# GemsLab/H2GCN

Hardware: AMD Instinct MI355X
Metric: aggregated edges/sec (1+2-hop SpMM) (higher is better)
Workload: dtype f32

## Files before the change

h2gcn_amd/_capi.py:

```python
from __future__ import annotations

import ctypes as C
import os
from pathlib import Path

ABI_VERSION = 5
MAX_HOPS = 8

OK = 0
ERR_INVALID_ARGUMENT = -1
ERR_HIP = -2
ERR_OUT_OF_MEMORY = -3
ERR_BAD_INDEX = -4
ERR_NO_TRANSPOSE = -5
ERR_INTERNAL = -6
ERR_EXCHANGE_TIMEOUT = -7

METRICS_MAX_SETS = 4
XCHG_BLOB_BYTES = 192
XCHG_COPY_ENGINE = 0
XCHG_COPY_KERNEL = 1

DTYPE_F32 = 0
DTYPE_BF16 = 1

PLAN_BUILD_TRANSPOSE = 0x1
PLAN_SKIP_VALIDATION = 0x2
PLAN_HOST_TRANSPOSE = 0x4
PLAN_KEEP_PERMUTATION = 0x8
PLAN_SYMMETRIC_PATTERN = 0x10

EXPORTED_SYMBOLS = (
    "h2gcn_abi_version",
    "h2gcn_last_error",
    "h2gcn_device_count",
    "h2gcn_plan_create",
    "h2gcn_plan_destroy",
    "h2gcn_plan_info",
    "h2gcn_plan_set_values",
    "h2gcn_plan_transpose_sharing",
    "h2gcn_plan_device_bytes",
    "h2gcn_spmm_hops_f32",
    "h2gcn_spmm_hops_T_f32",
    "h2gcn_plan_schedule",
    "h2gcn_plan_segment_classes",
    "h2gcn_spmm_workspace_bytes",
    "h2gcn_spmm_hops_opts_f32",
    "h2gcn_spmm_hops_T_opts_f32",
    "h2gcn_spmm_hops_bf16",
    "h2gcn_spmm_hops_T_bf16",
    "h2gcn_sddmm_hops_f32",
    "h2gcn_sddmm_hops_bf16",
    "h2gcn_row_softmax_hops_f32",
    "h2gcn_row_softmax_backward_hops_f32",
    "h2gcn_edge_scores_hops_f32",
    "h2gcn_edge_scores_backward_hops_f32",
    "h2gcn_spmm_hops_values_f32",
    "h2gcn_spmm_hops_T_values_f32",
    "h2gcn_ring_scratch_bytes",
    "h2gcn_ring_count",
    "h2gcn_ring_fill",
    "h2gcn_ring_count_rows",
    "h2gcn_ring_fill_rows",
    "h2gcn_hop_normalize",
    "h2gcn_hop_normalize_rows",
    "h2gcn_dropout_dense_small_rows",
    "h2gcn_dropout_dense_workspace_bytes",
    "h2gcn_dropout_dense_f32",
    "h2gcn_dropout_dense_backward_f32",
    "h2gcn_dropout_dense_bf16",
    "h2gcn_dropout_dense_backward_bf16",
    "h2gcn_dropout_dense_rows_f32",
    "h2gcn_dropout_dense_rows_bf16",
    "h2gcn_dropout_dense_backward_rows_f32",
    "h2gcn_dropout_dense_backward_rows_bf16",
    "h2gcn_masked_metrics_workspace_bytes",
    "h2gcn_masked_metrics_f32",
    "h2gcn_masked_ce_backward_f32",
    "h2gcn_adam_keras_f32",
    "h2gcn_adam_keras_l2_f32",
    "h2gcn_l2_penalty_workspace_bytes",
    "h2gcn_l2_penalty_f32",
    "h2gcn_xchg_create",
    "h2gcn_xchg_export",
    "h2gcn_xchg_connect",
    "h2gcn_xchg_allgather_begin",
    "h2gcn_xchg_allgather_post",
    "h2gcn_xchg_allgather_pull",
    "h2gcn_xchg_allgather_pull_rows",
    "h2gcn_xchg_allgather_end",
    "h2gcn_xchg_reduce_scatter_begin",
    "h2gcn_xchg_reduce_scatter_end",
    "h2gcn_xchg_reset_dependencies",
    "h2gcn_xchg_status",
    "h2gcn_xchg_destroy",
)


class PlanOpts(C.Structure):
    _fields_ = [
        ("struct_size", C.c_uint32),
        ("flags", C.c_uint32),
        ("long_row_threshold", C.c_int32),
        ("rows_per_wave", C.c_int32),
        ("variant", C.c_int32),
        ("slice_cols", C.c_int32),
        ("reserved", C.c_int32 * 2),
    ]


LAUNCH_RELU = 0x1
LAUNCH_ACCUMULATE = 0x2


class LaunchOpts(C.Structure):
    _fields_ = [
        ("struct_size", C.c_uint32),
        ("flags", C.c_uint32),
        ("workspace", C.c_void_p),
        ("workspace_bytes", C.c_size_t),
        ("bias", C.c_void_p),
    ]


class H2GCNError(RuntimeError):

    def __init__(self, status: int, message: str):
        super().__init__(f"libh2gcn_hip: {message} (status {status})")
        self.status = status


def library_path() -> Path:
    override = os.environ.get("H2GCN_HIP_LIBRARY")
    if override:
        return Path(override)
    return Path(__file__).resolve().parent / "csrc" / "libh2gcn_hip.so"


_LIB = None


def lib() -> C.CDLL:
    global _LIB
    if _LIB is not None:
        return _LIB
    path = library_path()
    if not path.exists():
        raise RuntimeError(
            f"{path} not found: build it with `python -c 'import __graft_entry__ as g; g.build()'` "
            "or `make -C h2gcn_amd/csrc`.  h2gcn_amd has no CPU fallback."
        )
    L = C.CDLL(str(path))
    L.h2gcn_abi_version.restype = C.c_int
    L.h2gcn_abi_version.argtypes = []
    L.h2gcn_last_error.restype = C.c_char_p
    L.h2gcn_last_error.argtypes = []
    L.h2gcn_device_count.restype = C.c_int
    L.h2gcn_device_count.argtypes = []
    L.h2gcn_plan_create.restype = C.c_int
    L.h2gcn_plan_create.argtypes = [
        C.c_int, C.c_int64, C.c_int64,
        C.POINTER(C.c_void_p), C.POINTER(C.c_void_p), C.POINTER(C.c_void_p),
        C.POINTER(PlanOpts), C.c_void_p, C.POINTER(C.c_void_p),
    ]
    L.h2gcn_plan_destroy.restype = None
    L.h2gcn_plan_destroy.argtypes = [C.c_void_p]
    L.h2gcn_plan_set_values.restype = C.c_int
    L.h2gcn_plan_set_values.argtypes = [C.c_void_p, C.c_int, C.c_void_p, C.c_void_p]
    L.h2gcn_plan_info.restype = C.c_int
    L.h2gcn_plan_info.argtypes = [
        C.c_void_p, C.c_int, C.POINTER(C.c_int64), C.POINTER(C.c_int64), C.POINTER(C.c_int64),
        C.POINTER(C.c_int64), C.POINTER(C.c_int32),
    ]
    L.h2gcn_spmm_hops_f32.restype = C.c_int
    L.h2gcn_spmm_hops_f32.argtypes = [
        C.c_void_p, C.c_uint32, C.c_void_p, C.c_int64, C.c_int32, C.c_void_p, C.c_int64, C.c_int64, C.c_void_p,
    ]
    L.h2gcn_spmm_hops_T_f32.restype = C.c_int
    L.h2gcn_spmm_hops_T_f32.argtypes = [
        C.c_void_p, C.c_uint32, C.c_void_p, C.c_int64, C.c_int64, C.c_int32, C.c_void_p, C.c_int64, C.c_void_p,
    ]
    L.h2gcn_plan_schedule.restype = C.c_int
    L.h2gcn_plan_schedule.argtypes = [C.c_void_p, C.c_uint32, C.c_int, C.c_int64, C.c_int32] + [C.POINTER(C.c_int32)] * 4
    if hasattr(L, "h2gcn_plan_segment_classes"):
        L.h2gcn_plan_segment_classes.restype = C.c_int
        L.h2gcn_plan_segment_classes.argtypes = [C.c_void_p, C.c_uint32, C.c_int, C.c_int64, C.c_int32] + [C.POINTER(C.c_int64)] * 3
    if hasattr(L, "h2gcn_plan_transpose_sharing"):
        L.h2gcn_plan_transpose_sharing.restype = C.c_int
        L.h2gcn_plan_transpose_sharing.argtypes = [C.c_void_p, C.c_int]
        L.h2gcn_plan_device_bytes.restype = C.c_size_t
        L.h2gcn_plan_device_bytes.argtypes = [C.c_void_p]
    L.h2gcn_spmm_workspace_bytes.restype = C.c_size_t
    L.h2gcn_spmm_workspace_bytes.argtypes = [C.c_void_p, C.c_uint32, C.c_int, C.c_void_p, C.c_int64, C.c_int64, C.c_int32]
    L.h2gcn_spmm_hops_opts_f32.restype = C.c_int
    L.h2gcn_spmm_hops_opts_f32.argtypes = [
        C.c_void_p, C.c_uint32, C.c_void_p, C.c_int64, C.c_int32, C.c_void_p, C.c_int64, C.c_int64,
        C.POINTER(LaunchOpts), C.c_void_p,
    ]
    L.h2gcn_spmm_hops_T_opts_f32.restype = C.c_int
    L.h2gcn_spmm_hops_T_opts_f32.argtypes = [
        C.c_void_p, C.c_uint32, C.c_void_p, C.c_int64, C.c_int64, C.c_int32, C.c_void_p, C.c_int64,
        C.POINTER(LaunchOpts), C.c_void_p,
    ]
    if hasattr(L, "h2gcn_spmm_hops_bf16"):
        L.h2gcn_spmm_hops_bf16.restype = C.c_int
        L.h2gcn_spmm_hops_bf16.argtypes = [
            C.c_void_p, C.c_uint32, C.c_void_p, C.c_int64, C.c_int32, C.c_int, C.c_void_p, C.c_int64, C.c_int64,
            C.POINTER(LaunchOpts), C.c_void_p,
        ]
        L.h2gcn_spmm_hops_T_bf16.restype = C.c_int
        L.h2gcn_spmm_hops_T_bf16.argtypes = [
            C.c_void_p, C.c_uint32, C.c_void_p, C.c_int64, C.c_int64, C.c_int32, C.c_int, C.c_void_p, C.c_int64,
            C.POINTER(LaunchOpts), C.c_void_p,
        ]
    if hasattr(L, "h2gcn_sddmm_hops_f32"):
        sddmm_args = [C.c_void_p, C.c_uint32, C.c_void_p, C.c_int64, C.c_int64, C.c_void_p, C.c_int64, C.c_int32,
                      C.POINTER(C.c_void_p), C.c_void_p]
        L.h2gcn_sddmm_hops_f32.restype = C.c_int
        L.h2gcn_sddmm_hops_f32.argtypes = sddmm_args
        L.h2gcn_sddmm_hops_bf16.restype = C.c_int
        L.h2gcn_sddmm_hops_bf16.argtypes = list(sddmm_args)
    if hasattr(L, "h2gcn_row_softmax_hops_f32"):
        L.h2gcn_row_softmax_hops_f32.restype = C.c_int
        L.h2gcn_row_softmax_hops_f32.argtypes = [C.c_void_p, C.c_uint32, C.POINTER(C.c_void_p), C.POINTER(C.c_void_p), C.c_void_p]
        L.h2gcn_row_softmax_backward_hops_f32.restype = C.c_int
        L.h2gcn_row_softmax_backward_hops_f32.argtypes = [C.c_void_p, C.c_uint32, C.POINTER(C.c_void_p), C.POINTER(C.c_void_p),
                                                          C.POINTER(C.c_void_p), C.c_void_p]
    if hasattr(L, "h2gcn_edge_scores_hops_f32"):
        node_args = [C.c_void_p, C.c_uint32, C.c_void_p, C.c_int64, C.c_void_p, C.c_int64, C.c_float, C.POINTER(C.c_void_p)]
        L.h2gcn_edge_scores_hops_f32.restype = C.c_int
        L.h2gcn_edge_scores_hops_f32.argtypes = node_args + [C.c_void_p]
        L.h2gcn_edge_scores_backward_hops_f32.restype = C.c_int
        L.h2gcn_edge_scores_backward_hops_f32.argtypes = node_args + [C.c_void_p, C.c_int64, C.c_void_p, C.c_int64, C.c_void_p]
    if hasattr(L, "h2gcn_spmm_hops_values_f32"):
        values_args = [C.c_void_p, C.c_uint32, C.POINTER(C.c_void_p), C.POINTER(C.c_int64), C.POINTER(C.c_int64), C.c_int32]
        L.h2gcn_spmm_hops_values_f32.restype = C.c_int
        L.h2gcn_spmm_hops_values_f32.argtypes = values_args + [C.c_void_p, C.c_int64, C.c_int32, C.c_void_p, C.c_int64, C.c_int64, C.c_void_p]
        L.h2gcn_spmm_hops_T_values_f32.restype = C.c_int
        L.h2gcn_spmm_hops_T_values_f32.argtypes = values_args + [C.c_void_p, C.c_int64, C.c_int64, C.c_int32, C.c_void_p, C.c_int64, C.c_void_p]
    L.h2gcn_ring_scratch_bytes.restype = C.c_size_t
    L.h2gcn_ring_scratch_bytes.argtypes = [C.c_int64]
    ring_common = [C.c_int64, C.c_void_p, C.c_void_p, C.c_void_p, C.c_void_p,
                   C.c_int, C.POINTER(C.c_void_p), C.POINTER(C.c_void_p), C.c_int,
                   C.c_int, C.POINTER(C.c_void_p), C.POINTER(C.c_void_p), C.c_int]
    L.h2gcn_ring_count.restype = C.c_int
    L.h2gcn_ring_count.argtypes = ring_common + [C.c_void_p, C.POINTER(C.c_int64), C.c_void_p, C.c_size_t, C.c_void_p]
    L.h2gcn_ring_fill.restype = C.c_int
    L.h2gcn_ring_fill.argtypes = ring_common + [C.c_void_p, C.c_void_p, C.c_void_p, C.c_size_t, C.c_void_p]
    ring_rows = [C.c_int64, C.c_int64, C.c_int64] + ring_common[1:]
    L.h2gcn_ring_count_rows.restype = C.c_int
    L.h2gcn_ring_count_rows.argtypes = ring_rows + [C.c_void_p, C.POINTER(C.c_int64), C.c_void_p, C.c_size_t, C.c_void_p]
    L.h2gcn_ring_fill_rows.restype = C.c_int
    L.h2gcn_ring_fill_rows.argtypes = ring_rows + [C.c_void_p, C.c_void_p, C.c_void_p, C.c_size_t, C.c_void_p]
    L.h2gcn_hop_normalize_rows.restype = C.c_int
    L.h2gcn_hop_normalize_rows.argtypes = [C.c_int64, C.c_void_p, C.c_void_p, C.c_int, C.c_void_p, C.c_int64, C.c_void_p, C.c_void_p, C.c_void_p]
    L.h2gcn_hop_normalize.restype = C.c_int
    L.h2gcn_hop_normalize.argtypes = [C.c_int64, C.c_void_p, C.c_void_p, C.c_int, C.c_void_p, C.c_int64, C.c_void_p, C.c_void_p]
    if hasattr(L, "h2gcn_dropout_dense_small_rows"):
        L.h2gcn_dropout_dense_small_rows.restype = C.c_int64
        L.h2gcn_dropout_dense_small_rows.argtypes = [C.c_int64]
    L.h2gcn_dropout_dense_workspace_bytes.restype = C.c_size_t
    L.h2gcn_dropout_dense_workspace_bytes.argtypes = [C.c_int64, C.c_int32, C.c_int32]
    L.h2gcn_dropout_dense_f32.restype = C.c_int
    L.h2gcn_dropout_dense_f32.argtypes = [C.c_void_p, C.c_int64, C.c_int64, C.c_int32, C.c_void_p, C.c_int32, C.c_void_p, C.c_float,
                                          C.c_uint64, C.c_void_p, C.c_void_p, C.c_int64, C.c_void_p, C.c_size_t, C.c_void_p]
    L.h2gcn_dropout_dense_backward_f32.restype = C.c_int
    L.h2gcn_dropout_dense_backward_f32.argtypes = [C.c_void_p, C.c_int64, C.c_int64, C.c_int32, C.c_void_p, C.c_int32, C.c_void_p, C.c_int64,
                                                   C.c_float, C.c_uint64, C.c_void_p, C.c_void_p, C.c_int64, C.c_void_p, C.c_void_p,
                                                   C.c_size_t, C.c_void_p]
    if hasattr(L, "h2gcn_dropout_dense_bf16"):
        L.h2gcn_dropout_dense_bf16.restype = C.c_int
        L.h2gcn_dropout_dense_bf16.argtypes = list(L.h2gcn_dropout_dense_f32.argtypes)
        L.h2gcn_dropout_dense_backward_bf16.restype = C.c_int
        L.h2gcn_dropout_dense_backward_bf16.argtypes = [C.c_void_p, C.c_int64, C.c_int64, C.c_int32, C.c_void_p, C.c_int32, C.c_void_p, C.c_int64,
                                                        C.c_float, C.c_uint64, C.c_void_p, C.c_int, C.c_void_p, C.c_int64, C.c_void_p, C.c_void_p,
                                                        C.c_size_t, C.c_void_p]
    if hasattr(L, "h2gcn_dropout_dense_rows_f32"):
        rows_args = [C.c_void_p, C.c_int64]
        L.h2gcn_dropout_dense_rows_f32.restype = C.c_int
        L.h2gcn_dropout_dense_rows_f32.argtypes = list(L.h2gcn_dropout_dense_f32.argtypes) + rows_args
        L.h2gcn_dropout_dense_rows_bf16.restype = C.c_int
        L.h2gcn_dropout_dense_rows_bf16.argtypes = list(L.h2gcn_dropout_dense_f32.argtypes) + rows_args
        L.h2gcn_dropout_dense_backward_rows_f32.restype = C.c_int
        L.h2gcn_dropout_dense_backward_rows_f32.argtypes = list(L.h2gcn_dropout_dense_backward_f32.argtypes) + rows_args
        L.h2gcn_dropout_dense_backward_rows_bf16.restype = C.c_int
        L.h2gcn_dropout_dense_backward_rows_bf16.argtypes = list(L.h2gcn_dropout_dense_backward_bf16.argtypes) + rows_args
    L.h2gcn_masked_metrics_workspace_bytes.restype = C.c_size_t
    L.h2gcn_masked_metrics_workspace_bytes.argtypes = [C.c_int64]
    L.h2gcn_masked_metrics_f32.restype = C.c_int
    L.h2gcn_masked_metrics_f32.argtypes = [C.c_void_p, C.c_int64, C.c_int64, C.c_int32, C.c_int32, C.POINTER(C.c_void_p), C.POINTER(C.c_int64),
                                           C.POINTER(C.c_void_p), C.c_void_p, C.c_void_p, C.c_void_p, C.c_size_t, C.c_void_p]
    L.h2gcn_masked_ce_backward_f32.restype = C.c_int
    L.h2gcn_masked_ce_backward_f32.argtypes = [C.c_void_p, C.c_int64, C.c_int64, C.c_int32, C.c_void_p, C.c_int64, C.c_void_p, C.c_void_p,
                                               C.c_void_p, C.c_int64, C.c_void_p]
    L.h2gcn_adam_keras_f32.restype = C.c_int
    L.h2gcn_adam_keras_f32.argtypes = [C.c_int32, C.POINTER(C.c_void_p), C.POINTER(C.c_void_p), C.POINTER(C.c_void_p), C.POINTER(C.c_void_p),
                                       C.POINTER(C.c_int64), C.c_float, C.c_float, C.c_float, C.c_float, C.c_void_p, C.c_int64, C.c_void_p]
    if hasattr(L, "h2gcn_adam_keras_l2_f32"):
        L.h2gcn_adam_keras_l2_f32.restype = C.c_int
        L.h2gcn_adam_keras_l2_f32.argtypes = [C.c_int32, C.POINTER(C.c_void_p), C.POINTER(C.c_void_p), C.POINTER(C.c_void_p), C.POINTER(C.c_void_p),
                                              C.POINTER(C.c_int64), C.POINTER(C.c_float), C.c_float, C.c_float, C.c_float, C.c_float, C.c_void_p,
                                              C.c_int64, C.c_void_p]
        L.h2gcn_l2_penalty_workspace_bytes.restype = C.c_size_t
        L.h2gcn_l2_penalty_workspace_bytes.argtypes = []
        L.h2gcn_l2_penalty_f32.restype = C.c_int
        L.h2gcn_l2_penalty_f32.argtypes = [C.c_int32, C.POINTER(C.c_void_p), C.POINTER(C.c_int64), C.POINTER(C.c_float), C.c_void_p, C.c_void_p,
                                           C.c_size_t, C.c_void_p]
    L.h2gcn_xchg_create.restype = C.c_int
    L.h2gcn_xchg_create.argtypes = [C.c_int, C.c_int, C.c_int, C.c_size_t, C.c_int, C.c_int, C.POINTER(C.c_void_p)]
    L.h2gcn_xchg_export.restype = C.c_int
    L.h2gcn_xchg_export.argtypes = [C.c_void_p, C.c_void_p]
    L.h2gcn_xchg_connect.restype = C.c_int
    L.h2gcn_xchg_connect.argtypes = [C.c_void_p, C.c_void_p]
    L.h2gcn_xchg_allgather_begin.restype = C.c_int
    L.h2gcn_xchg_allgather_begin.argtypes = [
        C.c_void_p, C.c_int, C.c_void_p, C.c_int64, C.c_int64, C.c_int64, C.c_int32, C.c_void_p, C.c_void_p,
    ]
    L.h2gcn_xchg_allgather_post.restype = C.c_int
    L.h2gcn_xchg_allgather_post.argtypes = L.h2gcn_xchg_allgather_begin.argtypes
    L.h2gcn_xchg_allgather_pull.restype = C.c_int
    L.h2gcn_xchg_allgather_pull.argtypes = [C.c_void_p, C.c_int, C.c_int64, C.c_int32, C.c_void_p]
    if hasattr(L, "h2gcn_xchg_allgather_pull_rows"):
        L.h2gcn_xchg_allgather_pull_rows.restype = C.c_int
        L.h2gcn_xchg_allgather_pull_rows.argtypes = [C.c_void_p, C.c_int, C.c_int64, C.c_int32, C.c_void_p, C.POINTER(C.c_void_p), C.POINTER(C.c_int64)]
    L.h2gcn_xchg_allgather_end.restype = C.c_int
    L.h2gcn_xchg_allgather_end.argtypes = [C.c_void_p, C.c_int, C.c_void_p]
    L.h2gcn_xchg_reduce_scatter_begin.restype = C.c_int
    L.h2gcn_xchg_reduce_scatter_begin.argtypes = [C.c_void_p, C.c_int, C.c_void_p, C.c_int64, C.c_int32, C.c_void_p, C.c_void_p]
    L.h2gcn_xchg_reduce_scatter_end.restype = C.c_int
    L.h2gcn_xchg_reduce_scatter_end.argtypes = [C.c_void_p, C.c_int, C.c_void_p]
    L.h2gcn_xchg_reset_dependencies.restype = C.c_int
    L.h2gcn_xchg_reset_dependencies.argtypes = [C.c_void_p]
    L.h2gcn_xchg_status.restype = C.c_int
    L.h2gcn_xchg_status.argtypes = [C.c_void_p]
    L.h2gcn_xchg_destroy.restype = None
    L.h2gcn_xchg_destroy.argtypes = [C.c_void_p]
    got = L.h2gcn_abi_version()
    if got != ABI_VERSION and not (os.environ.get("H2GCN_HIP_LIBRARY") and got in (3, 4)):
        raise RuntimeError(f"{path}: ABI version {got}, this front end expects {ABI_VERSION}")
    _LIB = L
    return L


def has(symbol: str) -> bool:
# ... 8 lines not shown
```

h2gcn_amd/csrc/h2gcn_capi.hip:

```cpp
#include <hip/hip_runtime.h>

#include <algorithm>
#include <cstdarg>
#include <cstdlib>
#include <cstdio>
#include <cstring>
#include <deque>
#include <map>
#include <mutex>
#include <memory>
#include <new>
#include <string>
#include <vector>

#include "h2gcn_hip.h"
#include "spmm_kernels.hip.h"

#include "capi_internal.h"

namespace h2gcn {

thread_local std::string g_last_error;

int fail(h2gcn_status st, const char* fmt, ...) {
    char buf[512];
    va_list ap;
    va_start(ap, fmt);
    vsnprintf(buf, sizeof(buf), fmt, ap);
    va_end(ap);
    g_last_error = buf;
    return (int)st;
}

}

namespace {

using h2gcn::fail;
using h2gcn::g_last_error;

struct DeviceBuf {
    void* p = nullptr;
    ~DeviceBuf() {
        if (p) (void)hipFree(p);
    }
    DeviceBuf() = default;
    DeviceBuf(DeviceBuf&& o) noexcept : p(o.p) { o.p = nullptr; }
    DeviceBuf(const DeviceBuf&) = delete;
    DeviceBuf& operator=(const DeviceBuf&) = delete;
};

struct HopOperand {
    const int64_t* rowptr = nullptr;
    const int32_t* colidx = nullptr;
    const float* vals = nullptr;
    int64_t nnz = 0;
    std::vector<int64_t> long_rows;
    std::vector<uint8_t> len8;
    int64_t n_short = 0, nnz_short = 0;
    int64_t nnz_long = 0;
    const uint32_t* perm = nullptr;
};

struct LongList {
    DeviceBuf dev;
    int n = 0;
    LongList() = default;
    LongList(LongList&&) noexcept = default;
};

struct ClassLists {
    DeviceBuf short_dev, med_dev;
    int64_t n_short = 0, nnz_short = 0, n_med = 0;
    bool built = false;
    ClassLists() = default;
    ClassLists(ClassLists&&) noexcept = default;
};

}

struct h2gcn_plan {
    int n_hops = 0;
    int64_t n_rows = 0, n_cols = 0;
    int long_threshold = 256;
    int rows_per_wave = 4;
    int variant = 0;
    int slice_cols = 0;
    bool has_transpose = false;
    int device = 0;
    std::vector<HopOperand> fwd;
    std::vector<HopOperand> adj;
    std::deque<DeviceBuf> owned;
    std::vector<int> sharing;
    size_t transpose_bytes = 0;
    mutable std::mutex mu;
    mutable std::map<uint64_t, LongList> long_cache;
    mutable std::map<uint64_t, ClassLists> class_cache;
    int short_max = -1;
    double short_min_frac = 0.05;
};

namespace h2gcn {
__global__ void check_colidx_kernel(const int32_t* __restrict__ colidx, int64_t nnz, int64_t n_cols, int* flag) {
    int bad = 0;
    for (int64_t i = (int64_t)blockIdx.x * blockDim.x + threadIdx.x; i < nnz; i += (int64_t)gridDim.x * blockDim.x) {
        const int32_t c = colidx[i];
        bad |= (c < 0) | ((int64_t)c >= n_cols);
    }
    if (bad) atomicOr(flag, 1);
}

extern template void launch_in_tile_short_rows<32, false, float, float>(const LaunchParams&, const Schedule&, dim3, hipStream_t);
extern template void launch_in_tile_short_rows<16, false, float, float>(const LaunchParams&, const Schedule&, dim3, hipStream_t);
extern template void launch_in_tile_short_rows<32, true, float, float>(const LaunchParams&, const Schedule&, dim3, hipStream_t);
extern template void launch_in_tile_short_rows<16, true, float, float>(const LaunchParams&, const Schedule&, dim3, hipStream_t);
extern template void launch_spmm<false, bf16, float>(const LaunchParams&, const Schedule&, dim3, hipStream_t);
extern template void launch_spmm<false, bf16, bf16>(const LaunchParams&, const Schedule&, dim3, hipStream_t);
extern template void launch_spmm<true, bf16, float>(const LaunchParams&, const Schedule&, dim3, hipStream_t);
extern template void launch_spmm<true, bf16, bf16>(const LaunchParams&, const Schedule&, dim3, hipStream_t);

int transpose_csr_device(int64_t n_rows, int64_t n_cols, int64_t nnz, const int64_t* rowptr, const int32_t* colidx,
                         const float* vals, int64_t** t_rowptr_out, int32_t** t_colidx_out, float** t_vals_out,
                         uint32_t** perm_out_keep, hipStream_t stream, std::string* err);
void permute_values(const uint32_t* perm, const float* vals, int64_t nnz, float* t_vals, hipStream_t stream);
}

namespace {

using h2gcn::HopCsr;
using h2gcn::LaunchParams;
using h2gcn::Schedule;

int transpose_csr_host(int64_t n_rows, int64_t n_cols, const std::vector<int64_t>& rowptr,
                       const std::vector<int32_t>& colidx, const std::vector<float>& vals,
                       std::vector<int64_t>& t_rowptr, std::vector<int32_t>& t_colidx, std::vector<float>& t_vals) {
    const int64_t nnz = rowptr[n_rows];
    t_rowptr.assign(n_cols + 1, 0);
    t_colidx.resize(nnz);
    t_vals.resize(nnz);
    for (int64_t i = 0; i < nnz; ++i) t_rowptr[colidx[i] + 1]++;
    for (int64_t c = 0; c < n_cols; ++c) t_rowptr[c + 1] += t_rowptr[c];
    std::vector<int64_t> cursor(t_rowptr.begin(), t_rowptr.end() - 1);
    for (int64_t r = 0; r < n_rows; ++r) {
        for (int64_t i = rowptr[r]; i < rowptr[r + 1]; ++i) {
            const int64_t dst = cursor[colidx[i]]++;
            t_colidx[dst] = (int32_t)r;
            t_vals[dst] = vals[i];
        }
    }
    return 0;
}

void collect_long_rows(const std::vector<int64_t>& rowptr, int64_t n_rows, int threshold, std::vector<int64_t>& out) {
    out.clear();
    for (int64_t r = 0; r < n_rows; ++r)
        if (rowptr[r + 1] - rowptr[r] >= threshold) out.push_back(r);
}

void collect_segment_lengths(const std::vector<int64_t>& rowptr, int64_t n_rows, int short_max, int long_threshold, HopOperand& op) {
    op.len8.resize((size_t)n_rows);
    op.n_short = op.nnz_short = op.nnz_long = 0;
    for (int64_t r = 0; r < n_rows; ++r) {
        const int64_t len = rowptr[r + 1] - rowptr[r];
        op.len8[(size_t)r] = (uint8_t)(len > 255 ? 255 : len);
        if (len <= short_max) {
            ++op.n_short;
            op.nnz_short += len;
        } else if (len >= long_threshold) {
            op.nnz_long += len;
        }
    }
}

thread_local bool t_stream_capturing = false;

struct CaptureScope {
    explicit CaptureScope(hipStream_t stream) {
        hipStreamCaptureStatus cs = hipStreamCaptureStatusNone;
        t_stream_capturing = hipStreamIsCapturing(stream, &cs) == hipSuccess && cs != hipStreamCaptureStatusNone;
        if (!t_stream_capturing) (void)hipGetLastError();
    }
    ~CaptureScope() { t_stream_capturing = false; }
};

int refuse_build_while_capturing(const char* what) {
    return fail(H2GCN_ERR_INVALID_ARGUMENT, "the stream is being captured and this is the first launch of this hop selection: its %s "
                "has to be built first (device allocation + upload).  Run the same launch once outside the capture (a warm-up step)", what);
}

int get_class_lists(const h2gcn_plan* plan, bool adjoint, int k, uint32_t mask, bool build, const ClassLists** out) {
    *out = nullptr;
    const std::vector<HopOperand>& ops = adjoint ? plan->adj : plan->fwd;
    const int64_t n_rows = adjoint ? plan->n_cols : plan->n_rows;
    if (plan->short_max < 0 || n_rows > 0x7fffffffLL) return H2GCN_OK;
    const uint64_t key = adjoint ? ((uint64_t)mask | (1ull << 32)) : ((uint64_t)k | (1ull << 40));
    const int sm = plan->short_max;
    std::lock_guard<std::mutex> lock(plan->mu);
    auto it = plan->class_cache.find(key);
    std::vector<const uint8_t*> sel;
    std::vector<uint8_t> any_long;
    auto prepare_adjoint = [&]() {
        any_long.assign((size_t)n_rows, 0);
        for (int h = 0; h < plan->n_hops; ++h)
            if (mask & (1u << h)) {
                sel.push_back(ops[h].len8.data());
                for (int64_t r : ops[h].long_rows) any_long[(size_t)r] = 1;
            }
    };
    if (it == plan->class_cache.end()) {
        ClassLists fresh;
        if (!adjoint) {
            fresh.n_short = ops[k].n_short;
            fresh.nnz_short = ops[k].nnz_short;
            fresh.n_med = n_rows - ops[k].n_short - (int64_t)ops[k].long_rows.size();
        } else {
            prepare_adjoint();
            for (int64_t r = 0; r < n_rows; ++r) {
                bool all = true;
                int64_t z = 0;
                for (const uint8_t* l : sel) { all = all && l[r] <= sm; z += l[r]; }
                if (all) { ++fresh.n_short; fresh.nnz_short += z; }
                else if (!any_long[(size_t)r]) ++fresh.n_med;
            }
        }
        it = plan->class_cache.emplace(key, std::move(fresh)).first;
    }
    ClassLists& cl = it->second;
    if (build && !cl.built) {
        if (t_stream_capturing) return refuse_build_while_capturing("per-class row lists");
        std::vector<int32_t> h_short, h_med;
        h_short.reserve((size_t)cl.n_short);
        h_med.reserve((size_t)cl.n_med);
        if (!adjoint) {
            const std::vector<uint8_t>& len = ops[k].len8;
            const std::vector<int64_t>& longs = ops[k].long_rows;
            size_t li = 0;
            for (int64_t r = 0; r < n_rows; ++r) {
                while (li < longs.size() && longs[li] < r) ++li;
                const bool is_long = li < longs.size() && longs[li] == r;
                if (len[(size_t)r] <= sm) h_short.push_back((int32_t)r);
                else if (!is_long) h_med.push_back((int32_t)r);
            }
        } else {
            if (sel.empty()) prepare_adjoint();
            for (int64_t r = 0; r < n_rows; ++r) {
                bool all = true;
                for (const uint8_t* l : sel) all = all && l[r] <= sm;
                if (all) h_short.push_back((int32_t)r);
                else if (!any_long[(size_t)r]) h_med.push_back((int32_t)r);
            }
        }
        DeviceBuf d_short, d_med;
        if (!h_short.empty()) {
            H2GCN_HIP_TRY(hipMalloc(&d_short.p, h_short.size() * sizeof(int32_t)));
            H2GCN_HIP_TRY(hipMemcpy(d_short.p, h_short.data(), h_short.size() * sizeof(int32_t), hipMemcpyHostToDevice));
        }
        if (!h_med.empty()) {
            H2GCN_HIP_TRY(hipMalloc(&d_med.p, h_med.size() * sizeof(int32_t)));
            H2GCN_HIP_TRY(hipMemcpy(d_med.p, h_med.data(), h_med.size() * sizeof(int32_t), hipMemcpyHostToDevice));
        }
// ... 63 lines not shown
        if (d % w != 0) continue;
        const double slice_bytes = (double)n_src_rows * w * 4.0;
        if (w > 64 && avg_segment_nnz >= 16.0 && slice_bytes > 768.0 * 1024 * 1024 && d % (w / 2) == 0) continue;
        return w;
    }
    if (rows_line_aligned && d % 4 == 0 && avg_segment_nnz >= 16.0 && (double)n_src_rows * d * 4.0 >= 512.0 * 1024 * 1024) {
        return 64;
    }
    if (d > 256) {
        const bool beyond = avg_segment_nnz >= 16.0 && (double)n_src_rows * 256 * 4.0 > 768.0 * 1024 * 1024;
        return beyond ? 128 : 256;
    }
    int w = 64;
    while (w < d) w *= 2;
    return w;
}

struct LaunchShape {
    bool adjoint;
    int n_sel;
    int64_t nnz_sel;
    int64_t n_out, n_src;
    double avg;
    int64_t ld_src;
    int d;
    bool src_line_aligned;
    const int32_t* short_list[H2GCN_MAX_HOPS];
    int64_t short_count[H2GCN_MAX_HOPS];
    const int32_t* med_list[H2GCN_MAX_HOPS];
    int64_t med_count[H2GCN_MAX_HOPS];
    int n_short_lists;
    double short_frac;
    double short_nnz_frac;
};

LaunchShape shape_of(const h2gcn_plan* plan, uint32_t mask, bool adjoint, const void* src = nullptr, int64_t ld_src = 0,
                     int64_t ld_src_hop = 0, int d = 0) {
    LaunchShape sh;
    memset(&sh, 0, sizeof(sh));
    sh.adjoint = adjoint;
    const std::vector<HopOperand>& ops = adjoint ? plan->adj : plan->fwd;
    for (int k = 0; k < plan->n_hops; ++k)
        if (mask & (1u << k)) { sh.nnz_sel += ops[k].nnz; ++sh.n_sel; }
    sh.n_out = adjoint ? plan->n_cols : plan->n_rows;
    sh.n_src = adjoint ? plan->n_rows : plan->n_cols;
    sh.avg = (sh.n_out > 0 && sh.n_sel > 0) ? (double)sh.nnz_sel / ((double)sh.n_out * sh.n_sel) : 0.0;
    sh.ld_src = ld_src;
    sh.d = d;
    sh.src_line_aligned = (reinterpret_cast<uintptr_t>(src) & 127u) == 0 && (ld_src * 4) % 128 == 0 &&
                          (!adjoint || sh.n_sel <= 1 || (ld_src_hop * 4) % 128 == 0);
    return sh;
}

int fill_short(const h2gcn_plan* plan, uint32_t mask, bool adjoint, LaunchShape& sh, bool build_lists = false);

int scratch_slice_cols(const h2gcn_plan* plan, const LaunchShape& sh) {
    if (plan->variant == 4) return 0;
    const int d = sh.d;
    if (sh.n_out == 0 || sh.n_src == 0 || sh.n_sel == 0) return 0;
    if (d <= 64) return 0;
    const double src_bytes = (double)sh.n_src * d * 4.0 * (sh.adjoint ? sh.n_sel : 1);
    if (src_bytes < 512.0 * 1024 * 1024) return 0;
    if ((double)sh.nnz_sel < 32.0 * (double)sh.n_src) return 0;
    if (!sh.adjoint && (sh.ld_src * 4) % 1024 == 0 && d % 64 == 0 && d >= 128) {
        const int w = pick_slice_cols(d, sh.n_src, plan->slice_cols, sh.avg);
        return (w == 64 || w == 128) && d % w == 0 && w < d ? w : 0;
    }
    if ((!sh.src_line_aligned || d % 4 != 0) && d > (sh.adjoint ? 256 : 128) && sh.avg >= 16.0 && (plan->slice_cols == 0 || plan->slice_cols == 64)) {
        return 64;
    }
    return 0;
}

size_t scratch_bytes(const LaunchShape& sh, int rs) {
    if (rs <= 0) return 0;
    const size_t n_slices = (size_t)((sh.d + rs - 1) / rs);
    return (size_t)sh.n_src * n_slices * (size_t)rs * 4 * (size_t)(sh.adjoint ? sh.n_sel : 1);
}

int decide(const h2gcn_plan* plan, uint32_t mask, LaunchShape& sh, int scratch, bool gen, Schedule& sc) {
    const int st = fill_short(plan, mask, sh.adjoint, sh);
    if (st != H2GCN_OK) return st;
    const int d = sh.d;
    const bool exact_ok = d >= 4;
    const int forced_slice = scratch > 0 ? scratch : plan->slice_cols;
    const int variant = plan->variant == 4 ? 0 : plan->variant;
    sc.pipe = (variant == 2 || (variant == 0 && sh.avg < 16.0)) && plan->rows_per_wave * sh.n_sel <= 32;
    sc.scalar128 = exact_ok && variant == 1 && d == 128 && forced_slice == 0;
    sc.slice = (exact_ok && !sc.scalar128) ? pick_slice_cols(d, sh.n_src, forced_slice, sh.avg, scratch > 0 || sh.src_line_aligned) : 0;
    sc.exact = sc.slice > 0 || sc.scalar128;
    sc.gen = gen;
    const bool grouped_ok = sc.exact && !sc.scalar128 && !gen && (sc.slice == 64 || sc.slice == 128);
    sc.shortrow = grouped_ok && (variant == 5 || (variant == 0 && sh.avg < 16.0 && sh.n_out >= 4 * kWavesToFill));
    sc.lists = grouped_ok && !sc.shortrow && sh.short_frac > 0.0 && (variant == 6 || (variant == 0 && sh.short_frac >= plan->short_min_frac));
    sc.pipe = sc.pipe && sc.exact && !sc.shortrow && !sc.lists && !gen;
    const bool beyond = (double)sh.n_src * d * 4.0 >= 512.0 * 1024 * 1024;
    sc.fb4 = beyond && (sc.shortrow || (sc.lists && sh.short_nnz_frac > 0.5));
    sc.off32 = false;
    return H2GCN_OK;
}

int launch(LaunchParams& p, const h2gcn_plan* plan, uint32_t mask, LaunchShape& sh, const Schedule& sc, bool adjoint,
           bool src_bf16, bool out_bf16, hipStream_t stream) {
    using namespace h2gcn;
    p.slice_cols = sc.exact ? (sc.slice > 0 ? sc.slice : 128) : p.d;
    p.n_slices = sc.exact ? (p.d + p.slice_cols - 1) / p.slice_cols : 1;
    if (p.src_slice_stride == 0) p.src_slice_stride = p.slice_cols;
    p.short_max = -1;
    p.short_groups = p.med_groups = 0;
    if (sc.lists) {
        int st = fill_short(plan, mask, adjoint, sh, true);
        if (st != H2GCN_OK) return st;
        int64_t n_listed = 0, n_med = 0, longest = 0;
        for (int s = 0; s < sh.n_short_lists; ++s) {
            n_listed += sh.short_count[s];
            n_med += sh.med_count[s];
            longest = std::max(longest, sh.short_count[s]);
        }
        static const int env_mpw = getenv("H2GCN_MED_PER_WAVE") ? atoi(getenv("H2GCN_MED_PER_WAVE")) : 0;
        static const int env_spw = getenv("H2GCN_SHORT_PER_WAVE") ? atoi(getenv("H2GCN_SHORT_PER_WAVE")) : 0;
        static const int env_major = getenv("H2GCN_SHORT_HOP_MAJOR") ? atoi(getenv("H2GCN_SHORT_HOP_MAJOR")) : -1;
        const int mpw_max = adjoint ? std::max(1, std::min(4, kWave / p.n_sel)) : 8;
        p.med_per_wave = (int)std::max<int64_t>(1, std::min<int64_t>(n_med / kWavesToFill, mpw_max));
        if (env_mpw >= 1 && env_mpw * p.n_sel <= kWave) p.med_per_wave = env_mpw;
        p.short_per_wave = 4;
        while (p.short_per_wave < 64 && n_listed / (2 * p.short_per_wave) >= kWavesToFill) p.short_per_wave *= 2;
        if (env_spw >= 4 && env_spw <= 64 && env_spw % 4 == 0) p.short_per_wave = env_spw;
        p.short_hop_major = env_major >= 0 ? env_major : 0;
        int64_t sblocks = 0, mblocks = 0;
        const int64_t s_per_block = (int64_t)kWavesPerBlock * p.short_per_wave;
        for (int s = 0; s < sh.n_short_lists; ++s) {
            p.short_list[s] = sh.short_list[s];
            p.short_count[s] = sh.short_count[s];
            sblocks += (sh.short_count[s] + s_per_block - 1) / s_per_block;
            p.short_end[s] = sblocks;
            p.med_list[s] = sh.med_list[s];
            p.med_count[s] = sh.med_count[s];
            const int64_t per_block = (int64_t)kWavesPerBlock * p.med_per_wave;
            mblocks += (sh.med_count[s] + per_block - 1) / per_block;
            p.med_end[s] = mblocks;
        }
        if (!adjoint && !p.short_hop_major) sblocks = (longest + s_per_block - 1) / s_per_block * sh.n_short_lists;
        p.short_groups = (sblocks + kNumXcd - 1) / kNumXcd;
        p.med_groups = (mblocks + kNumXcd - 1) / kNumXcd;
        p.short_max = plan->short_max;
        p.blocks_per_slice = (int64_t)p.n_long + (p.short_groups + p.med_groups) * kNumXcd;
    } else {
        p.blocks_per_slice = (int64_t)p.n_long + p.tiles_per_xcd * kNumXcd;
    }
    const int64_t n_blocks = p.blocks_per_slice * p.n_slices;
    if (n_blocks <= 0) return H2GCN_OK;
    if (n_blocks > 0x7fffffffLL) return fail(H2GCN_ERR_INVALID_ARGUMENT, "grid too large (%lld blocks)", (long long)n_blocks);
    const dim3 grid((unsigned)n_blocks);
    if (!src_bf16 && adjoint) launch_spmm<true, float, float>(p, sc, grid, stream);
    else if (!src_bf16) launch_spmm<false, float, float>(p, sc, grid, stream);
    else if (out_bf16 && adjoint) launch_spmm<true, bf16, bf16>(p, sc, grid, stream);
    else if (out_bf16) launch_spmm<false, bf16, bf16>(p, sc, grid, stream);
    else if (adjoint) launch_spmm<true, bf16, float>(p, sc, grid, stream);
    else launch_spmm<false, bf16, float>(p, sc, grid, stream);
    H2GCN_HIP_TRY(hipGetLastError());
    return H2GCN_OK;
}

void use_scratch(LaunchParams& p, const LaunchShape& sh, int rs, int64_t ld_src_hop, void* workspace, hipStream_t stream,
                 bool* off32) {
    const int n_hop = sh.adjoint ? sh.n_sel : 1;
    const int n_slices = (sh.d + rs - 1) / rs;
    const bool vec4 = sh.d % 4 == 0;
    const int64_t total = sh.n_src * (int64_t)n_slices * n_hop * (rs / (vec4 ? 4 : 1));
    const unsigned blocks = (unsigned)std::min<int64_t>((total + 255) / 256, 256 * 64);
    if (vec4)
        hipLaunchKernelGGL(h2gcn::repack_slice_major_kernel<true>, dim3(blocks), dim3(256), 0, stream, (const float*)p.src, sh.ld_src,
                           ld_src_hop, n_hop, sh.n_src, sh.d, n_slices, rs, (float*)workspace);
    else
        hipLaunchKernelGGL(h2gcn::repack_slice_major_kernel<false>, dim3(blocks), dim3(256), 0, stream, (const float*)p.src, sh.ld_src,
                           ld_src_hop, n_hop, sh.n_src, sh.d, n_slices, rs, (float*)workspace);
    p.src = workspace;
    p.ld_src = rs;
    p.d_src = (sh.d + 3) & ~3;
    p.src_slice_stride = sh.n_src * (int64_t)rs * n_hop;
    for (int s = 0; s < p.n_sel; ++s) p.src_hop_off[s] = sh.adjoint ? (int64_t)s * sh.n_src * rs : 0;
    *off32 = (double)sh.n_src * (double)n_slices * rs * n_hop * 4.0 < 4294967296.0;
}

int check_device(const h2gcn_plan* plan) {
    int cur = -1;
    H2GCN_HIP_TRY(hipGetDevice(&cur));
    if (cur != plan->device)
        return fail(H2GCN_ERR_INVALID_ARGUMENT, "plan lives on device %d but the current HIP device is %d", plan->device, cur);
    return H2GCN_OK;
}

int resolve_mask(const h2gcn_plan* plan, uint32_t hop_mask, uint32_t* out) {
    const uint32_t all = plan->n_hops >= 32 ? 0xffffffffu : ((1u << plan->n_hops) - 1u);
    if (hop_mask == 0) hop_mask = all;
    if (hop_mask & ~all) return fail(H2GCN_ERR_INVALID_ARGUMENT, "hop_mask 0x%x selects hops beyond the plan's %d", hop_mask, plan->n_hops);
    *out = hop_mask;
    return H2GCN_OK;
}

int share_symmetric(h2gcn_plan* plan, bool keep_perm, hipStream_t stream) {
    using h2gcn::MirrorStatus;
    const int H = plan->n_hops;
    const int64_t n = plan->n_rows;
    std::vector<MirrorStatus> h_status((size_t)H, MirrorStatus{~0ull, 0u, 0u});
    DeviceBuf d_status;
    H2GCN_HIP_TRY(hipMalloc(&d_status.p, (size_t)H * sizeof(MirrorStatus)));
    H2GCN_HIP_TRY(hipMemcpyAsync(d_status.p, h_status.data(), (size_t)H * sizeof(MirrorStatus), hipMemcpyHostToDevice, stream));
    std::vector<DeviceBuf> t_vals((size_t)H), partner((size_t)H);
    for (int k = 0; k < H; ++k) {
        const HopOperand& f = plan->fwd[k];
        if (f.nnz == 0) continue;
        H2GCN_HIP_TRY(hipMalloc(&t_vals[k].p, (size_t)f.nnz * sizeof(float)));
        if (keep_perm) H2GCN_HIP_TRY(hipMalloc(&partner[k].p, (size_t)f.nnz * sizeof(uint32_t)));
        H2GCN_HIP_TRY(h2gcn::mirror_pass(n, f.nnz, f.rowptr, f.colidx, f.vals, (uint32_t*)partner[k].p, (float*)t_vals[k].p,
                                         (MirrorStatus*)d_status.p + k, stream));
    }
    H2GCN_HIP_TRY(hipMemcpyAsync(h_status.data(), d_status.p, (size_t)H * sizeof(MirrorStatus), hipMemcpyDeviceToHost, stream));
    H2GCN_HIP_TRY(hipStreamSynchronize(stream));
    for (int k = 0; k < H; ++k) {
        const MirrorStatus& ms = h_status[k];
        if (ms.flags & h2gcn::kMirrorRange)
            return fail(H2GCN_ERR_BAD_INDEX, "hop %d: a column index lies outside [0, %lld)", k, (long long)n);
        if (ms.flags & h2gcn::kMirrorUnsorted)
            return fail(H2GCN_ERR_BAD_INDEX, "hop %d: the column ids of a row are not strictly ascending (H2GCN_PLAN_SYMMETRIC_PATTERN "
                        "searches rows by column and relies on the documented order)", k);
        if (ms.missing_key != ~0ull) {
            const long long r = (long long)(ms.missing_key >> 32), c = (long long)(ms.missing_key & 0xffffffffull);
            return fail(H2GCN_ERR_BAD_INDEX, "hop %d: entry (%lld, %lld) has no mirror entry (%lld, %lld): pattern not symmetric", k, r, c, c, r);
        }
    }
    plan->adj.resize(H);
    for (int k = 0; k < H; ++k) {
        const HopOperand& f = plan->fwd[k];
        HopOperand& a = plan->adj[k];
        a = f;
        a.perm = nullptr;
        const bool own_vals = f.nnz > 0 && (keep_perm || (h_status[k].flags & h2gcn::kMirrorValuesDiffer));
        plan->sharing[k] = own_vals ? 1 : 2;
        if (own_vals) {
            a.vals = (const float*)t_vals[k].p;
            plan->owned.emplace_back(std::move(t_vals[k]));
            plan->transpose_bytes += (size_t)f.nnz * sizeof(float);
        }
        if (keep_perm && f.nnz > 0) {
            a.perm = (const uint32_t*)partner[k].p;
            plan->owned.emplace_back(std::move(partner[k]));
            plan->transpose_bytes += (size_t)f.nnz * sizeof(uint32_t);
        }
    }
    return H2GCN_OK;
}

}

extern "C" {

int h2gcn_abi_version(void) { return H2GCN_ABI_VERSION; }

const char* h2gcn_last_error(void) { return g_last_error.c_str(); }

int h2gcn_device_count(void) {
    int n = 0;
    hipError_t e = hipGetDeviceCount(&n);
    if (e != hipSuccess) return fail(H2GCN_ERR_HIP, "hipGetDeviceCount failed: %s", hipGetErrorString(e));
    return n;
}

int h2gcn_plan_create(int n_hops, int64_t n_rows, int64_t n_cols, const int64_t* const* rowptr_dev,
                      const int32_t* const* colidx_dev, const float* const* vals_dev,
                      const h2gcn_plan_opts* opts, void* stream_v, h2gcn_plan_t** out_plan) {
    try {
        if (!out_plan) return fail(H2GCN_ERR_INVALID_ARGUMENT, "out_plan is NULL");
        *out_plan = nullptr;
        if (n_hops < 1 || n_hops > H2GCN_MAX_HOPS)
            return fail(H2GCN_ERR_INVALID_ARGUMENT, "n_hops = %d, supported 1..%d", n_hops, H2GCN_MAX_HOPS);
        if (n_rows < 0 || n_cols < 0 || n_cols > 0x7fffffffLL)
            return fail(H2GCN_ERR_INVALID_ARGUMENT, "bad shape %lld x %lld (column ids are int32)", (long long)n_rows, (long long)n_cols);
        if (n_rows >= (1LL << 58)) return fail(H2GCN_ERR_INVALID_ARGUMENT, "n_rows too large");
        if (!rowptr_dev || !colidx_dev || !vals_dev) return fail(H2GCN_ERR_INVALID_ARGUMENT, "NULL operand table");
        h2gcn_plan_opts o;
        memset(&o, 0, sizeof(o));
        if (opts) {
            if (opts->struct_size < 8 || opts->struct_size > sizeof(o))
                return fail(H2GCN_ERR_INVALID_ARGUMENT, "opts->struct_size = %u", opts->struct_size);
            memcpy(&o, opts, opts->struct_size);
        }
        if (o.slice_cols != 0 && o.slice_cols != 64 && o.slice_cols != 128 && o.slice_cols != 256)
            return fail(H2GCN_ERR_INVALID_ARGUMENT, "slice_cols = %d, supported 0 (auto), 64, 128, 256", o.slice_cols);
        if (o.long_row_threshold < 0 || o.rows_per_wave < 0 || o.rows_per_wave > h2gcn::kMaxRowsPerWave)
            return fail(H2GCN_ERR_INVALID_ARGUMENT, "bad tunable (long_row_threshold %d, rows_per_wave %d, max %d)",
                        o.long_row_threshold, o.rows_per_wave, h2gcn::kMaxRowsPerWave);
        const bool symmetric = (o.flags & H2GCN_PLAN_SYMMETRIC_PATTERN) != 0;
        if (symmetric && !(o.flags & H2GCN_PLAN_BUILD_TRANSPOSE))
            return fail(H2GCN_ERR_INVALID_ARGUMENT, "H2GCN_PLAN_SYMMETRIC_PATTERN modifies H2GCN_PLAN_BUILD_TRANSPOSE, which is not set");
        if (symmetric && (o.flags & H2GCN_PLAN_HOST_TRANSPOSE))
            return fail(H2GCN_ERR_INVALID_ARGUMENT, "H2GCN_PLAN_SYMMETRIC_PATTERN builds no transpose: it cannot be combined with H2GCN_PLAN_HOST_TRANSPOSE");
        if (symmetric && n_rows != n_cols)
            return fail(H2GCN_ERR_INVALID_ARGUMENT, "H2GCN_PLAN_SYMMETRIC_PATTERN needs square operands, got %lld x %lld", (long long)n_rows, (long long)n_cols);
        hipStream_t stream = (hipStream_t)stream_v;

        std::unique_ptr<h2gcn_plan> plan(new h2gcn_plan());
        plan->n_hops = n_hops;
        plan->n_rows = n_rows;
        plan->n_cols = n_cols;
        if (o.long_row_threshold > 0) plan->long_threshold = o.long_row_threshold;
        if (o.rows_per_wave > 0) plan->rows_per_wave = o.rows_per_wave;
        else if (const char* e = getenv("H2GCN_ROWS_PER_WAVE")) plan->rows_per_wave = std::max(1, std::min(atoi(e), h2gcn::kMaxRowsPerWave));
        else {
            plan->rows_per_wave = (int)std::max<int64_t>(1, std::min<int64_t>(n_rows / kWavesToFill, 4));
        }
        while ((plan->rows_per_wave + 1) * n_hops > h2gcn::kWave && plan->rows_per_wave > 1) plan->rows_per_wave--;
        plan->variant = o.variant;
        if (o.variant == 0) if (const char* e = getenv("H2GCN_VARIANT")) plan->variant = atoi(e);
        plan->slice_cols = o.slice_cols;
        if (o.slice_cols == 0) if (const char* e = getenv("H2GCN_SLICE_COLS")) plan->slice_cols = atoi(e);
        plan->short_max = std::min(h2gcn::kShortMax, plan->long_threshold - 1);
        if (const char* e = getenv("H2GCN_SHORT_MIN_FRAC")) plan->short_min_frac = atof(e);
        H2GCN_HIP_TRY(hipGetDevice(&plan->device));
        plan->fwd.resize(n_hops);

        DeviceBuf flag;
        H2GCN_HIP_TRY(hipMalloc(&flag.p, sizeof(int)));
        H2GCN_HIP_TRY(hipMemsetAsync(flag.p, 0, sizeof(int), stream));

        std::vector<std::vector<int64_t>> h_rowptr(n_hops);
        for (int k = 0; k < n_hops; ++k) {
            if (!rowptr_dev[k]) return fail(H2GCN_ERR_INVALID_ARGUMENT, "hop %d: rowptr is NULL", k);
            h_rowptr[k].resize(n_rows + 1);
            H2GCN_HIP_TRY(hipMemcpyAsync(h_rowptr[k].data(), rowptr_dev[k], (n_rows + 1) * sizeof(int64_t), hipMemcpyDeviceToHost, stream));
        }
        H2GCN_HIP_TRY(hipStreamSynchronize(stream));
        for (int k = 0; k < n_hops; ++k) {
            int st = check_rowptr(h_rowptr[k], n_rows, k);
            if (st != H2GCN_OK) return st;
            HopOperand& op = plan->fwd[k];
            op.rowptr = rowptr_dev[k];
            op.colidx = colidx_dev[k];
            op.vals = vals_dev[k];
            op.nnz = h_rowptr[k][n_rows];
            if (op.nnz > 0 && (!op.colidx || !op.vals)) return fail(H2GCN_ERR_INVALID_ARGUMENT, "hop %d: colidx/vals is NULL", k);
            if (symmetric && op.nnz >= (1LL << 32))
                return fail(H2GCN_ERR_INVALID_ARGUMENT, "hop %d: H2GCN_PLAN_SYMMETRIC_PATTERN supports < 2^32 nonzeros per hop", k);
            collect_long_rows(h_rowptr[k], n_rows, plan->long_threshold, op.long_rows);
            collect_segment_lengths(h_rowptr[k], n_rows, plan->short_max, plan->long_threshold, op);
            if (!(o.flags & H2GCN_PLAN_SKIP_VALIDATION) && op.nnz > 0) {
                const int64_t want = (op.nnz + 255) / 256;
                const unsigned blocks = (unsigned)std::min<int64_t>(want, 4096);
                hipLaunchKernelGGL(h2gcn::check_colidx_kernel, dim3(blocks), dim3(256), 0, stream, op.colidx, op.nnz, n_cols, (int*)flag.p);
                H2GCN_HIP_TRY(hipGetLastError());
            }
        }
        int h_flag = 0;
        H2GCN_HIP_TRY(hipMemcpyAsync(&h_flag, flag.p, sizeof(int), hipMemcpyDeviceToHost, stream));
        H2GCN_HIP_TRY(hipStreamSynchronize(stream));
        if (h_flag) return fail(H2GCN_ERR_BAD_INDEX, "a column index lies outside [0, %lld)", (long long)n_cols);

        plan->sharing.assign(n_hops, 0);
        if (symmetric) {
            int st = share_symmetric(plan.get(), (o.flags & H2GCN_PLAN_KEEP_PERMUTATION) != 0, stream);
            if (st != H2GCN_OK) return st;
            plan->has_transpose = true;
        } else if (o.flags & H2GCN_PLAN_BUILD_TRANSPOSE) {
            if (n_rows > 0x7fffffffLL) return fail(H2GCN_ERR_INVALID_ARGUMENT, "transpose needs n_rows < 2^31");
            plan->adj.resize(n_hops);
            for (int k = 0; k < n_hops; ++k) {
                const int64_t nnz = plan->fwd[k].nnz;
                int64_t* t_rp = nullptr;
                int32_t* t_ci = nullptr;
                float* t_va = nullptr;
                uint32_t* t_perm = nullptr;
                const bool keep_perm = (o.flags & H2GCN_PLAN_KEEP_PERMUTATION) != 0;
                if (keep_perm && (o.flags & H2GCN_PLAN_HOST_TRANSPOSE))
                    return fail(H2GCN_ERR_INVALID_ARGUMENT, "H2GCN_PLAN_KEEP_PERMUTATION needs the device transposition");
                std::vector<int64_t> t_rowptr(n_cols + 1);
                std::string terr;
                int st = (o.flags & H2GCN_PLAN_HOST_TRANSPOSE)
                             ? -1
                             : h2gcn::transpose_csr_device(n_rows, n_cols, nnz, rowptr_dev[k], colidx_dev[k], vals_dev[k],
                                                           &t_rp, &t_ci, &t_va, keep_perm ? &t_perm : nullptr, stream, &terr);
                if (st != 0 && keep_perm && st != -3)
                    return fail(H2GCN_ERR_INVALID_ARGUMENT, "H2GCN_PLAN_KEEP_PERMUTATION: %s", terr.c_str());
                if (st == 0) {
                    plan->owned.emplace_back(); plan->owned.back().p = t_rp;
                    plan->owned.emplace_back(); plan->owned.back().p = t_ci;
                    plan->owned.emplace_back(); plan->owned.back().p = t_va;
                    plan->owned.emplace_back(); plan->owned.back().p = t_perm;
                    plan->transpose_bytes += (size_t)(n_cols + 1) * sizeof(int64_t) + (size_t)nnz * (t_perm ? 12 : 8);
                    H2GCN_HIP_TRY(hipMemcpy(t_rowptr.data(), t_rp, (n_cols + 1) * sizeof(int64_t), hipMemcpyDeviceToHost));
                } else if (st == -3) {
                    return fail(H2GCN_ERR_OUT_OF_MEMORY, "transposition of hop %d: %s", k, terr.c_str());
                } else {
                    std::vector<int32_t> h_col(nnz);
                    std::vector<float> h_val(nnz);
                    if (nnz > 0) {
                        H2GCN_HIP_TRY(hipMemcpy(h_col.data(), colidx_dev[k], nnz * sizeof(int32_t), hipMemcpyDeviceToHost));
                        H2GCN_HIP_TRY(hipMemcpy(h_val.data(), vals_dev[k], nnz * sizeof(float), hipMemcpyDeviceToHost));
                    }
                    std::vector<int32_t> t_col;
                    std::vector<float> t_val;
                    transpose_csr_host(n_rows, n_cols, h_rowptr[k], h_col, h_val, t_rowptr, t_col, t_val);
                    plan->owned.emplace_back();
                    DeviceBuf& d_rp = plan->owned.back();
                    H2GCN_HIP_TRY(hipMalloc(&d_rp.p, (n_cols + 1) * sizeof(int64_t)));
                    H2GCN_HIP_TRY(hipMemcpy(d_rp.p, t_rowptr.data(), (n_cols + 1) * sizeof(int64_t), hipMemcpyHostToDevice));
                    plan->owned.emplace_back();
                    DeviceBuf& d_ci = plan->owned.back();
                    plan->owned.emplace_back();
                    DeviceBuf& d_va = plan->owned.back();
                    if (nnz > 0) {
                        H2GCN_HIP_TRY(hipMalloc(&d_ci.p, nnz * sizeof(int32_t)));
                        H2GCN_HIP_TRY(hipMemcpy(d_ci.p, t_col.data(), nnz * sizeof(int32_t), hipMemcpyHostToDevice));
                        H2GCN_HIP_TRY(hipMalloc(&d_va.p, nnz * sizeof(float)));
                        H2GCN_HIP_TRY(hipMemcpy(d_va.p, t_val.data(), nnz * sizeof(float), hipMemcpyHostToDevice));
                    }
                    plan->transpose_bytes += (size_t)(n_cols + 1) * sizeof(int64_t) + (size_t)nnz * 8;
                    t_rp = (int64_t*)d_rp.p;
                    t_ci = (int32_t*)d_ci.p;
                    t_va = (float*)d_va.p;
                }
                HopOperand& op = plan->adj[k];
                op.rowptr = t_rp;
                op.colidx = t_ci;
                op.vals = t_va;
                op.nnz = nnz;
                op.perm = t_perm;
                collect_long_rows(t_rowptr, n_cols, plan->long_threshold, op.long_rows);
                collect_segment_lengths(t_rowptr, n_cols, plan->short_max, plan->long_threshold, op);
            }
            plan->has_transpose = true;
        }
        {
            const uint32_t all = n_hops >= 32 ? 0xffffffffu : ((1u << n_hops) - 1u);
            const int64_t* unused_p = nullptr;
            int unused_n = 0;
            int st = get_long_list(plan.get(), false, all, &unused_p, &unused_n);
            if (st == H2GCN_OK && plan->has_transpose) st = get_long_list(plan.get(), true, all, &unused_p, &unused_n);
            if (st != H2GCN_OK) return st;
            auto mixed = [&](const LaunchShape& sh_) {
                return plan->variant == 6 || (plan->variant == 0 && sh_.short_frac >= plan->short_min_frac &&
                                              (sh_.avg >= 16.0 || sh_.n_out < 4 * kWavesToFill));
            };
            LaunchShape sh_f = shape_of(plan.get(), all, false);
            if ((st = fill_short(plan.get(), all, false, sh_f)) != H2GCN_OK) return st;
            if (mixed(sh_f) && (st = fill_short(plan.get(), all, false, sh_f, true)) != H2GCN_OK) return st;
            if (plan->has_transpose) {
                LaunchShape sh_a = shape_of(plan.get(), all, true);
                if ((st = fill_short(plan.get(), all, true, sh_a)) != H2GCN_OK) return st;
                if (mixed(sh_a) && (st = fill_short(plan.get(), all, true, sh_a, true)) != H2GCN_OK) return st;
            }
        }
        *out_plan = plan.release();
        return H2GCN_OK;
    } catch (const std::bad_alloc&) {
        return fail(H2GCN_ERR_OUT_OF_MEMORY, "host allocation failed in plan_create");
    } catch (...) {
        return fail(H2GCN_ERR_INTERNAL, "unexpected exception in plan_create");
    }
}

void h2gcn_plan_destroy(h2gcn_plan_t* plan) { delete plan; }

int h2gcn_plan_set_values(h2gcn_plan_t* plan, int hop, const float* vals_dev, void* stream_v) {
    if (!plan) return fail(H2GCN_ERR_INVALID_ARGUMENT, "plan is NULL");
    if (hop < 0 || hop >= plan->n_hops) return fail(H2GCN_ERR_INVALID_ARGUMENT, "hop %d outside 0..%d", hop, plan->n_hops - 1);
    HopOperand& f = plan->fwd[hop];
    if (f.nnz > 0 && !vals_dev) return fail(H2GCN_ERR_INVALID_ARGUMENT, "vals is NULL");
    int st = check_device(plan);
    if (st != H2GCN_OK) return st;
    if (plan->has_transpose) {
        HopOperand& a = plan->adj[hop];
        if (a.nnz > 0 && !a.perm)
            return fail(H2GCN_ERR_INVALID_ARGUMENT, "plan has transposed operands but was created without H2GCN_PLAN_KEEP_PERMUTATION");
        h2gcn::permute_values(a.perm, vals_dev, a.nnz, const_cast<float*>(a.vals), (hipStream_t)stream_v);
        H2GCN_HIP_TRY(hipGetLastError());
    }
    f.vals = vals_dev;
    return H2GCN_OK;
}

int h2gcn_plan_info(const h2gcn_plan_t* plan, int hop, int64_t* n_rows, int64_t* n_cols, int64_t* nnz,
                    int64_t* n_long_segments, int32_t* has_transpose) {
    if (!plan) return fail(H2GCN_ERR_INVALID_ARGUMENT, "plan is NULL");
    if (hop < 0 || hop >= plan->n_hops) return fail(H2GCN_ERR_INVALID_ARGUMENT, "hop %d outside 0..%d", hop, plan->n_hops - 1);
    if (n_rows) *n_rows = plan->n_rows;
    if (n_cols) *n_cols = plan->n_cols;
    if (nnz) *nnz = plan->fwd[hop].nnz;
    if (n_long_segments) *n_long_segments = (int64_t)plan->fwd[hop].long_rows.size();
    if (has_transpose) *has_transpose = plan->has_transpose ? 1 : 0;
    return H2GCN_OK;
}

int h2gcn_plan_transpose_sharing(const h2gcn_plan_t* plan, int hop) {
    if (!plan) return fail(H2GCN_ERR_INVALID_ARGUMENT, "plan is NULL");
    if (hop < 0 || hop >= plan->n_hops) return fail(H2GCN_ERR_INVALID_ARGUMENT, "hop %d outside 0..%d", hop, plan->n_hops - 1);
    return plan->sharing[(size_t)hop];
}

size_t h2gcn_plan_device_bytes(const h2gcn_plan_t* plan) {
    if (!plan) return 0;
    std::lock_guard<std::mutex> lock(plan->mu);
    size_t bytes = plan->transpose_bytes;
    for (const auto& kv : plan->long_cache) bytes += (size_t)kv.second.n * sizeof(int64_t);
    for (const auto& kv : plan->class_cache)
        if (kv.second.built) bytes += (size_t)(kv.second.n_short + kv.second.n_med) * sizeof(int32_t);
    return bytes;
}

namespace {
int fill_short(const h2gcn_plan* plan, uint32_t mask, bool adjoint, LaunchShape& sh, bool build_lists) {
    sh.n_short_lists = 0;
    sh.short_frac = sh.short_nnz_frac = 0.0;
    if (plan->short_max < 0 || sh.n_out <= 0 || sh.n_sel <= 0) return H2GCN_OK;
    int64_t n = 0, nnz = 0;
    const ClassLists* cl = nullptr;
    if (!adjoint) {
        int s = 0;
        for (int k = 0; k < plan->n_hops; ++k) {
            if (!(mask & (1u << k))) continue;
            int st = get_class_lists(plan, false, k, 0, build_lists, &cl);
            if (st != H2GCN_OK) return st;
            if (!cl) return H2GCN_OK;
            sh.short_list[s] = (const int32_t*)cl->short_dev.p;
            sh.short_count[s] = cl->n_short;
            sh.med_list[s] = (const int32_t*)cl->med_dev.p;
            sh.med_count[s] = cl->n_med;
            n += cl->n_short;
            nnz += cl->nnz_short;
            ++s;
        }
        sh.n_short_lists = s;
        sh.short_frac = (double)n / ((double)sh.n_out * sh.n_sel);
    } else {
        if (sh.n_sel > h2gcn::kShortSumHops) return H2GCN_OK;
        int st = get_class_lists(plan, true, 0, mask, build_lists, &cl);
        if (st != H2GCN_OK) return st;
        if (!cl) return H2GCN_OK;
        sh.short_list[0] = (const int32_t*)cl->short_dev.p;
        sh.short_count[0] = cl->n_short;
        sh.med_list[0] = (const int32_t*)cl->med_dev.p;
        sh.med_count[0] = cl->n_med;
        n = cl->n_short;
        nnz = cl->nnz_short;
        sh.n_short_lists = 1;
        sh.short_frac = (double)n / (double)sh.n_out;
    }
    if (n == 0) sh.n_short_lists = 0;
    sh.short_nnz_frac = sh.nnz_sel > 0 ? (double)nnz / (double)sh.nnz_sel : (n > 0 ? 1.0 : 0.0);
    return H2GCN_OK;
}

int report_schedule(const h2gcn_plan* plan, uint32_t hop_mask, int adjoint, int64_t ld_src, int32_t d, uint32_t* mask,
                    LaunchShape& sh, int& scratch, Schedule& sc) {
    if (!plan) return fail(H2GCN_ERR_INVALID_ARGUMENT, "plan is NULL");
    int st = resolve_mask(plan, hop_mask, mask);
    if (st != H2GCN_OK) return st;
    if (d < 1 || ld_src < d) return fail(H2GCN_ERR_INVALID_ARGUMENT, "bad width %d / stride %lld", d, (long long)ld_src);
    if (adjoint && !plan->has_transpose) return fail(H2GCN_ERR_NO_TRANSPOSE, "plan was created without H2GCN_PLAN_BUILD_TRANSPOSE");
    sh = shape_of(plan, *mask, adjoint != 0, nullptr, ld_src, d, d);
    scratch = scratch_slice_cols(plan, sh);
    return decide(plan, *mask, sh, scratch, d % 4 != 0, sc);
}

}

int h2gcn_plan_schedule(const h2gcn_plan_t* plan, uint32_t hop_mask, int adjoint, int64_t ld_src, int32_t d,
                        int32_t* slice_cols, int32_t* n_slices, int32_t* segment_walk, int32_t* scratch_copy) {
    uint32_t mask;
    LaunchShape sh;
    int scratch;
    Schedule sc;
    const int st = report_schedule(plan, hop_mask, adjoint, ld_src, d, &mask, sh, scratch, sc);
    if (st != H2GCN_OK) return st;
    const int w = sc.exact ? (sc.slice > 0 ? sc.slice : 128) : d;
    if (slice_cols) *slice_cols = w;
    if (n_slices) *n_slices = sc.exact ? (d + w - 1) / w : 1;
    if (segment_walk) *segment_walk = sc.pipe ? 1 : (sc.shortrow ? 2 : (sc.lists ? 3 : 0));
    if (scratch_copy) *scratch_copy = scratch > 0 ? 1 : 0;
    return H2GCN_OK;
}

int h2gcn_plan_segment_classes(const h2gcn_plan_t* plan, uint32_t hop_mask, int adjoint, int64_t ld_src, int32_t d,
                               int64_t* segments, int64_t* nonzeros, int64_t* listed) {
    uint32_t mask;
    LaunchShape sh;
    int scratch;
    Schedule sc;
    const int st = report_schedule(plan, hop_mask, adjoint, ld_src, d, &mask, sh, scratch, sc);
    if (st != H2GCN_OK) return st;
    const std::vector<HopOperand>& ops = adjoint ? plan->adj : plan->fwd;
    int s = 0;
    for (int k = 0; k < plan->n_hops; ++k) {
        if (!(mask & (1u << k))) continue;
        const HopOperand& op = ops[k];
        const int64_t n_long = (int64_t)op.long_rows.size();
        if (segments) {
            segments[3 * s + 0] = op.n_short;
            segments[3 * s + 1] = sh.n_out - op.n_short - n_long;
            segments[3 * s + 2] = n_long;
        }
        if (nonzeros) {
            nonzeros[3 * s + 0] = op.nnz_short;
            nonzeros[3 * s + 1] = op.nnz - op.nnz_short - op.nnz_long;
            nonzeros[3 * s + 2] = op.nnz_long;
        }
        ++s;
    }
    if (listed) {
        *listed = 0;
        if (sc.lists)
            for (int q = 0; q < sh.n_short_lists; ++q) *listed += sh.short_count[q];
        if (sc.shortrow) *listed = -1;
    }
    return H2GCN_OK;
}

size_t h2gcn_spmm_workspace_bytes(const h2gcn_plan_t* plan, uint32_t hop_mask, int adjoint, const float* src_dev,
                                  int64_t ld_src, int64_t ld_src_hop, int32_t d) {
    if (!plan || d < 1 || ld_src < d) return 0;
    if (adjoint && !plan->has_transpose) return 0;
    uint32_t mask;
    if (resolve_mask(plan, hop_mask, &mask) != H2GCN_OK) return 0;
    const LaunchShape sh = shape_of(plan, mask, adjoint != 0, src_dev, ld_src, ld_src_hop, d);
    return scratch_bytes(sh, scratch_slice_cols(plan, sh));
}

namespace {
int read_launch_opts(const h2gcn_launch_opts* lopts, h2gcn_launch_opts* lo) {
    memset(lo, 0, sizeof(*lo));
    if (lopts) {
        if (lopts->struct_size < 8 || lopts->struct_size > sizeof(*lo))
            return fail(H2GCN_ERR_INVALID_ARGUMENT, "launch opts struct_size = %u", lopts->struct_size);
        memcpy(lo, lopts, lopts->struct_size);
    }
    if (lo->flags & ~(uint32_t)(H2GCN_LAUNCH_RELU | H2GCN_LAUNCH_ACCUMULATE)) return fail(H2GCN_ERR_INVALID_ARGUMENT, "unknown launch flags 0x%x", lo->flags);
    return H2GCN_OK;
}

int check_bf16_layout(const char* what, const void* p, int64_t ld_row, int64_t ld_hop, int32_t d) {
    if (reinterpret_cast<uintptr_t>(p) & 3u)
        return fail(H2GCN_ERR_INVALID_ARGUMENT, "bf16 %s: the base address must be 4-byte aligned", what);
    if ((ld_row & 1) || (ld_hop & 1))
        return fail(H2GCN_ERR_INVALID_ARGUMENT, "bf16 %s: row / hop strides must be even (got %lld / %lld elements)", what,
                    (long long)ld_row, (long long)ld_hop);
    if (d & 1) return fail(H2GCN_ERR_INVALID_ARGUMENT, "bf16 %s: the feature width d must be even (got %d)", what, d);
    return H2GCN_OK;
}

int check_dtype(const char* what, int dtype) {
    if (dtype != H2GCN_DTYPE_F32 && dtype != H2GCN_DTYPE_BF16)
        return fail(H2GCN_ERR_INVALID_ARGUMENT, "%s = %d: must be H2GCN_DTYPE_F32 (%d) or H2GCN_DTYPE_BF16 (%d)", what, dtype,
                    H2GCN_DTYPE_F32, H2GCN_DTYPE_BF16);
    return H2GCN_OK;
}

// ... 190 lines not shown
```

h2gcn_amd/csrc/spmm_kernels.hip.h:

```cpp
#pragma once

#include <hip/hip_runtime.h>
#include <stdint.h>

#include <type_traits>

#include "h2gcn_hip.h"

namespace h2gcn {

constexpr int kWave = 64;
constexpr int kWavesPerBlock = 4;
constexpr int kBlock = kWave * kWavesPerBlock;
constexpr int kNumXcd = 8;
constexpr int kMaxRowsPerWave = 7;
#ifndef H2GCN_MIN_WAVES
#define H2GCN_MIN_WAVES 6
#endif
constexpr int kMinWavesPerSimd = H2GCN_MIN_WAVES;
#ifndef H2GCN_SHORT_MIN_WAVES
#define H2GCN_SHORT_MIN_WAVES 4
#endif
#ifndef H2GCN_SHORT_FB4_MIN_WAVES
#define H2GCN_SHORT_FB4_MIN_WAVES 7
#endif
#ifndef H2GCN_MAIN_MAXB
#define H2GCN_MAIN_MAXB 8
#endif
#ifndef H2GCN_WIDE_MAXB
#define H2GCN_WIDE_MAXB H2GCN_MAIN_MAXB
#endif
#ifndef H2GCN_WIDE_MIN_WAVES
#define H2GCN_WIDE_MIN_WAVES H2GCN_MIN_WAVES
#endif
constexpr int kShortMax = 16;
constexpr int kShortSumHops = 4;
#ifndef H2GCN_SHORT_PREFETCH
#define H2GCN_SHORT_PREFETCH 2
#endif
#ifndef H2GCN_OFF64_HEAVY_MIN_WAVES
#define H2GCN_OFF64_HEAVY_MIN_WAVES 5
#endif
constexpr int kMaxTileCols = 256;
constexpr int kTreeParts = 4;

template <int LPR>
struct Tree {
    static constexpr int G = kWave / LPR;
    static_assert(G == 1 || G == 2 || G == 4, "lane geometries: 64 / 128 / 256 columns per slice");
    static constexpr int NP = kTreeParts / G;
};

struct HopCsr {
    const int64_t* rowptr;
    const int32_t* colidx;
    const float* vals;
};

struct LaunchParams {
    HopCsr hop[H2GCN_MAX_HOPS];
    int64_t src_hop_off[H2GCN_MAX_HOPS];
    int64_t dst_hop_off[H2GCN_MAX_HOPS];
    int n_sel;
    int d;
    int d_src;
    int64_t n_rows;
    const void* src;
    int64_t ld_src;
    int64_t src_slice_stride;
    void* dst;
    int64_t ld_dst;
    const int64_t* long_list;
    int n_long;
    int long_threshold;
    int rows_per_wave;
    int64_t n_tiles;
    int64_t tiles_per_xcd;
    int n_slices;
    int slice_cols;
    int64_t blocks_per_slice;
    const float* bias;
    int relu;
    int accumulate;
    const int32_t* short_list[H2GCN_MAX_HOPS];
    int64_t short_count[H2GCN_MAX_HOPS];
    int64_t short_end[H2GCN_MAX_HOPS];
    int64_t short_groups;
    int short_max;
    int short_per_wave;
    int short_hop_major;
    const int32_t* med_list[H2GCN_MAX_HOPS];
    int64_t med_count[H2GCN_MAX_HOPS];
    int64_t med_end[H2GCN_MAX_HOPS];
    int64_t med_groups;
    int med_per_wave;
};

template <int VEC>
struct VecT;
template <>
struct VecT<1> {
    using type = float;
};
template <>
struct VecT<2> {
    typedef float type __attribute__((ext_vector_type(2), aligned(4)));
};
template <>
struct VecT<4> {
    typedef float type __attribute__((ext_vector_type(4), aligned(4)));
};

struct bf16 {
    uint16_t bits;
};

template <typename TS, int VEC>
struct LoadT {
    using type = typename VecT<VEC>::type;
};
template <>
struct LoadT<bf16, 4> {
    typedef uint32_t type __attribute__((ext_vector_type(2), aligned(4)));
};
template <>
struct LoadT<bf16, 2> {
    using type = uint32_t;
};
template <>
struct LoadT<bf16, 1> {
    using type = uint16_t;
};

template <typename TS>
__device__ __forceinline__ const TS* src_ptr(const void* p) { return reinterpret_cast<const TS*>(p); }
template <typename TD>
__device__ __forceinline__ TD* dst_ptr(void* p) { return reinterpret_cast<TD*>(p); }

__device__ __forceinline__ float bf16_lo(uint32_t w) { return __uint_as_float(w << 16); }
__device__ __forceinline__ float bf16_hi(uint32_t w) { return __uint_as_float(w & 0xffff0000u); }
__device__ __forceinline__ uint32_t pack_bf16x2(float lo, float hi) {
    typedef __bf16 bf16x2 __attribute__((ext_vector_type(2)));
    const bf16x2 v = {(__bf16)lo, (__bf16)hi};
    return __builtin_bit_cast(uint32_t, v);
}

__device__ __forceinline__ int wave_uniform(int v) { return __builtin_amdgcn_readfirstlane(v); }

__device__ __forceinline__ int lane_gather(int v, int src_lane) {
    return __builtin_amdgcn_ds_bpermute(src_lane << 2, v);
}
__device__ __forceinline__ float lane_gather(float v, int src_lane) {
    return __int_as_float(__builtin_amdgcn_ds_bpermute(src_lane << 2, __float_as_int(v)));
}

__device__ __forceinline__ float fold_xor32(float v) {
    const unsigned u = __float_as_uint(v);
    auto r = __builtin_amdgcn_permlane32_swap(u, u, false, false);
    return __uint_as_float(r[0]) + __uint_as_float(r[1]);
}
__device__ __forceinline__ float fold_xor16(float v) {
    const unsigned u = __float_as_uint(v);
    auto r = __builtin_amdgcn_permlane16_swap(u, u, false, false);
    return __uint_as_float(r[0]) + __uint_as_float(r[1]);
}
__device__ __forceinline__ float fold_xor8(float v) {
    const int o = __builtin_amdgcn_update_dpp(0, __float_as_int(v), 0x128 , 0xf, 0xf, false);
    return v + __int_as_float(o);
}

__device__ __forceinline__ float fold_ror4(float v) {
    const int o = __builtin_amdgcn_update_dpp(0, __float_as_int(v), 0x124 , 0xf, 0xf, false);
    return v + __int_as_float(o);
}

template <int LPR>
__device__ __forceinline__ float fold_groups(float v) {
    if constexpr (LPR <= 8) v = fold_xor8(v);
    if constexpr (LPR <= 4) v = fold_ror4(v);
    if constexpr (LPR <= 16) v = fold_xor16(v);
    if constexpr (LPR <= 32) v = fold_xor32(v);
    return v;
}

template <int VEC, int LPR, int NP>
__device__ __forceinline__ void fold_tree(const float (&acc)[NP][VEC], float (&tot)[VEC]) {
    constexpr int G = kWave / LPR;
    static_assert(NP == Tree<LPR>::NP, "partials per lane");
#pragma unroll
    for (int i = 0; i < VEC; ++i) {
        if constexpr (G == 1) tot[i] = (acc[0][i] + acc[1][i]) + (acc[2][i] + acc[3][i]);
        else if constexpr (G == 2) tot[i] = fold_xor32(acc[0][i]) + fold_xor32(acc[1][i]);
        else tot[i] = fold_groups<LPR>(acc[0][i]);
    }
}

template <int VEC, int NP>
__device__ __forceinline__ void zero_acc(float (&acc)[NP][VEC]) {
#pragma unroll
    for (int k = 0; k < NP; ++k)
#pragma unroll
        for (int i = 0; i < VEC; ++i) acc[k][i] = 0.f;
}

template <typename TS, int VEC>
__device__ __forceinline__ typename LoadT<TS, VEC>::type load_vec(const void* p) {
#ifdef H2GCN_NT_GATHER
    return __builtin_nontemporal_load(reinterpret_cast<const typename LoadT<TS, VEC>::type*>(p));
#else
    return *reinterpret_cast<const typename LoadT<TS, VEC>::type*>(p);
#endif
}

template <typename TS, int VEC>
__device__ __forceinline__ typename LoadT<TS, VEC>::type zero_load() {
    if constexpr (std::is_same<TS, float>::value && VEC > 1) return (typename VecT<VEC>::type)(0.f);
    else return (typename LoadT<TS, VEC>::type)0;
}

template <typename TS, int VEC>
__device__ __forceinline__ void fma_vec(float (&acc)[VEC], float w, typename LoadT<TS, VEC>::type x) {
    if constexpr (std::is_same<TS, bf16>::value) {
        if constexpr (VEC == 1) {
            acc[0] = fmaf(w, __uint_as_float((uint32_t)x << 16), acc[0]);
        } else if constexpr (VEC == 2) {
            acc[0] = fmaf(w, bf16_lo(x), acc[0]);
            acc[1] = fmaf(w, bf16_hi(x), acc[1]);
        } else {
#pragma unroll
            for (int i = 0; i < VEC / 2; ++i) {
                acc[2 * i] = fmaf(w, bf16_lo(x[i]), acc[2 * i]);
                acc[2 * i + 1] = fmaf(w, bf16_hi(x[i]), acc[2 * i + 1]);
            }
        }
    } else if constexpr (VEC == 1) {
        acc[0] = fmaf(w, x, acc[0]);
    } else {
#pragma unroll
        for (int i = 0; i < VEC; ++i) acc[i] = fmaf(w, x[i], acc[i]);
    }
}

template <bool OFF32>
struct GatherAddr {
    const char* base;
    typename std::conditional<OFF32, uint32_t, int64_t>::type lane_off;
    typename std::conditional<OFF32, uint32_t, int64_t>::type ld_bytes;
    __device__ __forceinline__ const void* row(int col) const {
        if constexpr (OFF32) {
            return base + (uint32_t)(lane_off + (uint32_t)col * ld_bytes);
        } else {
            return base + (lane_off + (int64_t)col * ld_bytes);
        }
    }
};

template <typename TS, int VEC, int LPR, int U, bool PREDICATED, bool OFF32, int PHASE = 0, int NP>
__device__ __forceinline__ void gather_batch(int c, float v, int t, int g, const GatherAddr<OFF32>& addr, bool take,
                                             float (&acc)[NP][VEC]) {
    constexpr int G = kWave / LPR;
    typename LoadT<TS, VEC>::type x[U];
    float w[U];
#pragma unroll
    for (int u = 0; u < U; ++u) {
        int cj;
        if constexpr (G == 1) {
            cj = __builtin_amdgcn_readlane(c, t + u);
            w[u] = __int_as_float(__builtin_amdgcn_readlane(__float_as_int(v), t + u));
        } else {
            const int idx = ((t + u) * G + g) & (kWave - 1);
            cj = lane_gather(c, idx);
            w[u] = lane_gather(v, idx);
        }
        const void* p = addr.row(cj);
        if constexpr (PREDICATED) {
            if (take) {
                x[u] = load_vec<TS, VEC>(p);
            } else {
                w[u] = 0.f;
                x[u] = zero_load<TS, VEC>();
            }
        } else {
            x[u] = load_vec<TS, VEC>(p);
        }
    }
#pragma unroll
    for (int u = 0; u < U; ++u) fma_vec<TS, VEC>(acc[(PHASE + u) % NP], w[u], x[u]);
}

__device__ __forceinline__ void load_chunk(const int32_t* __restrict__ colidx, const float* __restrict__ vals,
                                           int64_t base, int64_t seg_end, int lane, int& c, float& v) {
    c = 0;
    v = 0.f;
    if (base + lane < seg_end) {
        c = __builtin_nontemporal_load(colidx + base + lane);
        v = __builtin_nontemporal_load(vals + base + lane);
    }
}

template <typename TS, int VEC, int LPR, bool MASKED, bool OFF32, int MAXB = H2GCN_MAIN_MAXB, int NP>
__device__ __forceinline__ void process_chunk(int c, float v, int n, int g, const GatherAddr<OFF32>& addr,
                                              bool lane_active, float (&acc)[NP][VEC]) {
    constexpr int G = kWave / LPR;
    const int full = n / G;
    int t = 0;
    if constexpr (MAXB >= 8)
        for (; t + 8 <= full; t += 8) gather_batch<TS, VEC, LPR, 8, MASKED, OFF32>(c, v, t, g, addr, lane_active, acc);
    if constexpr (MAXB < 8)
        for (; t + 4 <= full; t += 4) gather_batch<TS, VEC, LPR, 4, MASKED, OFF32>(c, v, t, g, addr, lane_active, acc);
    if (t + 4 <= full) {
        gather_batch<TS, VEC, LPR, 4, MASKED, OFF32>(c, v, t, g, addr, lane_active, acc);
        t += 4;
    }
    const int rem = n - full * G;
    if (t + 2 <= full) {
        gather_batch<TS, VEC, LPR, 2, MASKED, OFF32>(c, v, t, g, addr, lane_active, acc);
        t += 2;
        if (t + 1 <= full) {
            gather_batch<TS, VEC, LPR, 1, MASKED, OFF32, 2 % NP>(c, v, t, g, addr, lane_active, acc);
            if constexpr (G > 1)
                if (rem > 0) gather_batch<TS, VEC, LPR, 1, true, OFF32, 3 % NP>(c, v, full, g, addr, lane_active && g < rem, acc);
        } else {
            if constexpr (G > 1)
                if (rem > 0) gather_batch<TS, VEC, LPR, 1, true, OFF32, 2 % NP>(c, v, full, g, addr, lane_active && g < rem, acc);
        }
    } else if (t + 1 <= full) {
        gather_batch<TS, VEC, LPR, 1, MASKED, OFF32>(c, v, t, g, addr, lane_active, acc);
        if constexpr (G > 1)
            if (rem > 0) gather_batch<TS, VEC, LPR, 1, true, OFF32, 1 % NP>(c, v, full, g, addr, lane_active && g < rem, acc);
    } else {
        if constexpr (G > 1)
            if (rem > 0) gather_batch<TS, VEC, LPR, 1, true, OFF32>(c, v, full, g, addr, lane_active && g < rem, acc);
    }
}

constexpr int kRingHops = 2;
constexpr int kRingCap = 256;
constexpr int kRingBlock = 128;
constexpr int64_t kRingMaxRange = 0x7fff0000;
typedef uint32_t u32x2 __attribute__((ext_vector_type(2)));
typedef uint32_t u32x4 __attribute__((ext_vector_type(4), aligned(4)));
struct WindowChunk {
    const uint32_t* ring;
    uint32_t e_lane;
    template <int G>
    __device__ __forceinline__ void fetch(int step, int g, int& cj, float& w) const {
        static_assert(G > 1, "the one-neighbour-per-load geometry keeps v_readlane");
        const u32x2 pr = *reinterpret_cast<const u32x2*>(ring + 2 * ((e_lane + (uint32_t)(step * G)) & (kRingCap - 1)));
        cj = (int)pr[0];
        w = __uint_as_float(pr[1]);
    }
};

template <typename TS, int VEC, int LPR, int U, bool PREDICATED, bool OFF32, int PHASE = 0, int NP>
__device__ __forceinline__ void gather_batch_window(const WindowChunk& ch, int t, int g, const GatherAddr<OFF32>& addr, bool take,
                                             float (&acc)[NP][VEC]) {
    constexpr int G = kWave / LPR;
    typename LoadT<TS, VEC>::type x[U];
    float w[U];
#pragma unroll
    for (int u = 0; u < U; ++u) {
        int cj;
        ch.template fetch<G>(t + u, g, cj, w[u]);
        const void* p = addr.row(cj);
        if constexpr (PREDICATED) {
            if (take) {
                x[u] = load_vec<TS, VEC>(p);
            } else {
                w[u] = 0.f;
                x[u] = zero_load<TS, VEC>();
            }
        } else {
            x[u] = load_vec<TS, VEC>(p);
        }
    }
#pragma unroll
    for (int u = 0; u < U; ++u) fma_vec<TS, VEC>(acc[(PHASE + u) % NP], w[u], x[u]);
}

template <typename TS, int VEC, int LPR, bool MASKED, bool OFF32, int MAXB = H2GCN_MAIN_MAXB, int NP>
__device__ __forceinline__ void process_chunk_window(const WindowChunk& ch, int n, int g, const GatherAddr<OFF32>& addr,
                                              bool lane_active, float (&acc)[NP][VEC]) {
    constexpr int G = kWave / LPR;
    const int full = n / G;
    int t = 0;
    if constexpr (MAXB >= 8)
        for (; t + 8 <= full; t += 8) gather_batch_window<TS, VEC, LPR, 8, MASKED, OFF32>(ch, t, g, addr, lane_active, acc);
    if constexpr (MAXB < 8)
        for (; t + 4 <= full; t += 4) gather_batch_window<TS, VEC, LPR, 4, MASKED, OFF32>(ch, t, g, addr, lane_active, acc);
    if (t + 4 <= full) {
        gather_batch_window<TS, VEC, LPR, 4, MASKED, OFF32>(ch, t, g, addr, lane_active, acc);
        t += 4;
    }
    const int rem = n - full * G;
    if (t + 2 <= full) {
        gather_batch_window<TS, VEC, LPR, 2, MASKED, OFF32>(ch, t, g, addr, lane_active, acc);
        t += 2;
        if (t + 1 <= full) {
            gather_batch_window<TS, VEC, LPR, 1, MASKED, OFF32, 2 % NP>(ch, t, g, addr, lane_active, acc);
            if constexpr (G > 1)
                if (rem > 0) gather_batch_window<TS, VEC, LPR, 1, true, OFF32, 3 % NP>(ch, full, g, addr, lane_active && g < rem, acc);
        } else {
            if constexpr (G > 1)
                if (rem > 0) gather_batch_window<TS, VEC, LPR, 1, true, OFF32, 2 % NP>(ch, full, g, addr, lane_active && g < rem, acc);
        }
    } else if (t + 1 <= full) {
        gather_batch_window<TS, VEC, LPR, 1, MASKED, OFF32>(ch, t, g, addr, lane_active, acc);
        if constexpr (G > 1)
            if (rem > 0) gather_batch_window<TS, VEC, LPR, 1, true, OFF32, 1 % NP>(ch, full, g, addr, lane_active && g < rem, acc);
    } else {
        if constexpr (G > 1)
            if (rem > 0) gather_batch_window<TS, VEC, LPR, 1, true, OFF32>(ch, full, g, addr, lane_active && g < rem, acc);
    }
}

template <typename TS, int VEC, int LPR, bool MASKED, bool OFF32, int MAXB = H2GCN_MAIN_MAXB, int NP>
__device__ __forceinline__ void accumulate_segment(const int32_t* __restrict__ colidx,
                                                   const float* __restrict__ vals, int64_t seg_begin,
                                                   int64_t seg_end, int chunk0, int chunk_step,
                                                   const GatherAddr<OFF32>& addr, int lane, bool lane_active,
                                                   float (&acc)[NP][VEC]) {
    const int g = lane / LPR;
    for (int64_t base = seg_begin + (int64_t)chunk0 * kWave; base < seg_end; base += (int64_t)chunk_step * kWave) {
        const int64_t left = seg_end - base;
        const int n = left < kWave ? (int)left : kWave;
        int c;
        float v;
        load_chunk(colidx, vals, base, seg_end, lane, c, v);
        process_chunk<TS, VEC, LPR, MASKED, OFF32, MAXB>(c, v, n, g, addr, lane_active, acc);
    }
}

template <typename TS, int VEC, int LPR, bool OFF32, int MAXB = H2GCN_MAIN_MAXB, int NP>
__device__ __forceinline__ void accumulate_segment_prefetched(const int32_t* __restrict__ colidx,
                                                              const float* __restrict__ vals, int64_t seg_begin,
                                                              int64_t seg_end, int c, float v,
                                                              const GatherAddr<OFF32>& addr, int lane,
                                                              float (&acc)[NP][VEC]) {
    const int g = lane / LPR;
    for (int64_t base = seg_begin; base < seg_end; base += kWave) {
        const int64_t left = seg_end - base;
        const int n = left < kWave ? (int)left : kWave;
        int c_next = 0;
        float v_next = 0.f;
        if (left > kWave) load_chunk(colidx, vals, base + kWave, seg_end, lane, c_next, v_next);
        process_chunk<TS, VEC, LPR, false, OFF32, MAXB>(c, v, n, g, addr, true, acc);
        c = c_next;
        v = v_next;
    }
}

template <typename TS, int VEC, int LPR, bool OFF32>
__device__ __forceinline__ void accumulate_grouped(int c, float v, int n_mine, int n_max, int lane,
                                                   const GatherAddr<OFF32>& addr, float (&part)[kTreeParts][VEC]) {
    constexpr int U = kTreeParts;
    const int group_base = lane & ~(LPR - 1);
    for (int t = 0; t < n_max; t += U) {
        typename LoadT<TS, VEC>::type x[U];
        float w[U];
#pragma unroll
        for (int u = 0; u < U; ++u) {
            const int cj = lane_gather(c, group_base + t + u);
            w[u] = lane_gather(v, group_base + t + u);
            if (t + u < n_mine) {
                x[u] = load_vec<TS, VEC>(addr.row(cj));
            } else {
                w[u] = 0.f;
                x[u] = zero_load<TS, VEC>();
            }
        }
#pragma unroll
        for (int u = 0; u < U; ++u)
            if (t + u < n_mine) fma_vec<TS, VEC>(part[u], w[u], x[u]);
    }
}

template <int VEC>
__device__ __forceinline__ void combine_partials(const float (&part)[kTreeParts][VEC], float (&acc)[VEC]) {
#pragma unroll
    for (int i = 0; i < VEC; ++i) acc[i] = (part[0][i] + part[1][i]) + (part[2][i] + part[3][i]);
}

__device__ __forceinline__ float relu_keep_nan(float t) { return t < 0.f ? 0.f : t; }

template <int VEC>
__device__ __forceinline__ void epilogue(float (&acc)[VEC], const float* __restrict__ bias, int relu, int col) {
    if (bias) {
#pragma unroll
        for (int i = 0; i < VEC; ++i) acc[i] += bias[col + i];
    }
    if (relu) {
#pragma unroll
        for (int i = 0; i < VEC; ++i) acc[i] = relu_keep_nan(acc[i]);
    }
}

template <typename TD>
__device__ __forceinline__ void store_one(TD* p, float t) {
    if constexpr (std::is_same<TD, bf16>::value)
        __builtin_nontemporal_store(__builtin_bit_cast(uint16_t, (__bf16)t), reinterpret_cast<uint16_t*>(p));
    else
        __builtin_nontemporal_store(t, p);
}

template <typename TD, int VEC>
__device__ __forceinline__ void store_vec(TD* p, const float (&acc)[VEC]) {
    if constexpr (std::is_same<TD, bf16>::value) {
        if constexpr (VEC == 1) {
            store_one<TD>(p, acc[0]);
        } else if constexpr (VEC == 2) {
            __builtin_nontemporal_store(pack_bf16x2(acc[0], acc[1]), reinterpret_cast<uint32_t*>(p));
        } else {
            typename LoadT<bf16, VEC>::type o;
#pragma unroll
            for (int i = 0; i < VEC / 2; ++i) o[i] = pack_bf16x2(acc[2 * i], acc[2 * i + 1]);
            __builtin_nontemporal_store(o, reinterpret_cast<typename LoadT<bf16, VEC>::type*>(p));
        }
    } else if constexpr (VEC == 1) {
        __builtin_nontemporal_store(acc[0], p);
    } else {
        typename VecT<VEC>::type o;
#pragma unroll
        for (int i = 0; i < VEC; ++i) o[i] = acc[i];
#if defined(H2GCN_AB_NO_STORES)
        if (acc[0] == 1.2345678e30f)
            __builtin_nontemporal_store(o, reinterpret_cast<typename VecT<VEC>::type*>(p));
#elif defined(H2GCN_PLAIN_STORES)
        *reinterpret_cast<typename VecT<VEC>::type*>(p) = o;
#else
        __builtin_nontemporal_store(o, reinterpret_cast<typename VecT<VEC>::type*>(p));
#endif
    }
}

template <typename TD, int VEC, bool GEN, typename P>
__device__ __forceinline__ void store_out(const P& p, TD* row, int col0, int ecol, float (&tot)[VEC]) {
    constexpr bool kF32 = std::is_same<TD, float>::value;
    if (col0 + VEC <= p.d) {
        if constexpr (GEN) {
            if (kF32 && p.accumulate) {
                if constexpr (VEC == 1) {
                    tot[0] += reinterpret_cast<const float*>(row)[col0];
                } else {
                    const typename VecT<VEC>::type old = *reinterpret_cast<const typename VecT<VEC>::type*>(reinterpret_cast<const float*>(row) + col0);
#pragma unroll
                    for (int i = 0; i < VEC; ++i) tot[i] += old[i];
                }
            }
            epilogue<VEC>(tot, p.bias, p.relu, col0);
        }
        store_vec<TD, VEC>(row + col0, tot);
        return;
    }
    if constexpr (GEN) {
        if (col0 < p.d) {
#pragma unroll
            for (int i = 0; i < VEC; ++i) {
                const int c = ecol + i;
                if (c >= col0 && c < p.d) {
                    float t = tot[i];
                    if (kF32 && p.accumulate) t += reinterpret_cast<const float*>(row)[c];
                    if (p.bias) t += p.bias[c];
                    if (p.relu) t = relu_keep_nan(t);
                    store_one<TD>(row + c, t);
                }
            }
        }
    }
}

template <typename TS, typename TD, int VEC, int LPR, bool SUM, bool OFF32, bool EPI, int PD>
__device__ __forceinline__ void short_list_blocks(const LaunchParams& p, int64_t sblock, int lane, int wave, int64_t lane_off0,
                                                  int64_t src_col_begin, int lcol, int ecol,
                                                  uint64_t (&s_seg)[kWavesPerBlock][kShortSumHops][kWave],
                                                  int32_t (&s_row)[kWavesPerBlock][kWave]) {
    using off_t = typename std::conditional<OFF32, uint32_t, int64_t>::type;
    constexpr int G = kWave / LPR;
    constexpr uint64_t kBeginMask = (1ull << 58) - 1;
    const int li = lane % LPR, g = lane / LPR;
    const int n_sel = p.n_sel;
    int hop = 0;
    int64_t local = sblock;
// ... 154 lines not shown
    constexpr int NP = Tree<LPR>::NP;
    constexpr int kBias = VEC;
    const int li = lane % LPR, g = lane / LPR;
    const int n_sel = p.n_sel;
    const off_t lane_off0 = (off_t)lane_off0_;
    auto seg_bound = [&](int l) -> int64_t {
        return ((int64_t)__builtin_amdgcn_readlane(rp_hi, l) << 32) | (uint32_t)__builtin_amdgcn_readlane(rp_lo, l);
    };
    {
        constexpr int G = kWave / LPR;
        const int short_max = min(LPR, p.long_threshold - 1);
        const int n_blocks = (rows_here + G - 1) / G;
        const GatherAddr<OFF32> addr0{nullptr, lane_off0, (off_t)(p.ld_src * sizeof(TS))};
        auto row_wave_wide = [&](int r, int s_first, int s_last) {
            float acc[NP][VEC];
            zero_acc<VEC, NP>(acc);
            if constexpr (SUM) {
                for (int s = s_first; s < s_last; ++s) {
                    const int l0 = s * (rpw + 1) + r;
                    if (seg_bound(l0 + 1) - seg_bound(l0) >= p.long_threshold) return;
                }
            }
            for (int s = s_first; s < s_last; ++s) {
                const int l0 = s * (rpw + 1) + r;
                const int64_t sb = seg_bound(l0), se = seg_bound(l0 + 1);
                if (!SUM && se - sb >= p.long_threshold) continue;
                const HopCsr& h = p.hop[s];
                GatherAddr<OFF32> addr = addr0;
                addr.base = reinterpret_cast<const char*>(src_ptr<TS>(p.src) + p.src_hop_off[s] + src_col_begin - kBias);
                accumulate_segment<TS, VEC, LPR, false, OFF32, FB>(h.colidx, h.vals, sb, se, 0, 1, addr, lane, true, acc);
                if constexpr (!SUM) {
                    float tot[VEC];
                    fold_tree<VEC, LPR, NP>(acc, tot);
                    if (g == 0) store_out<TD, VEC, EPI>(p, dst_ptr<TD>(p.dst) + (row0 + r) * p.ld_dst + p.dst_hop_off[s], lcol, ecol, tot);
                    zero_acc<VEC, NP>(acc);
                }
            }
            if constexpr (SUM) {
                float tot[VEC];
                fold_tree<VEC, LPR, NP>(acc, tot);
                if (g == 0) store_out<TD, VEC, EPI>(p, dst_ptr<TD>(p.dst) + (row0 + r) * p.ld_dst, lcol, ecol, tot);
            }
        };
        auto my_segment = [&](int s, int blk, int64_t& begin, int& len) {
            const int r = blk * G + g;
            const int l0 = s * (rpw + 1) + min(r, rpw - 1);
            const int64_t sb = ((int64_t)lane_gather(rp_hi, l0) << 32) | (uint32_t)lane_gather(rp_lo, l0);
            const int64_t se = ((int64_t)lane_gather(rp_hi, l0 + 1) << 32) | (uint32_t)lane_gather(rp_lo, l0 + 1);
            begin = sb;
            const int64_t n = se - sb;
            len = r < rows_here ? (int)(n > 0x7fffffff ? 0x7fffffff : n) : -1;
        };
        if constexpr (!SUM) {
            const int n_rounds = n_sel * n_blocks;
            int64_t begin_n = 0;
            int len_n = -1, c_n = 0;
            float v_n = 0.f;
            bool short_n = false;
            auto fetch = [&](int i) {
                const int s_ = i / n_blocks, blk_ = i - s_ * n_blocks;
                my_segment(s_, blk_, begin_n, len_n);
                short_n = __builtin_amdgcn_ballot_w64(len_n > short_max) == 0;
                c_n = 0;
                v_n = 0.f;
                if (short_n && li < len_n) {
                    c_n = __builtin_nontemporal_load(p.hop[s_].colidx + begin_n + li);
                    v_n = __builtin_nontemporal_load(p.hop[s_].vals + begin_n + li);
                }
            };
            if (n_rounds > 0) fetch(0);
            for (int i = 0; i < n_rounds; ++i) {
                const int s = i / n_blocks, blk = i - s * n_blocks;
                const int len = len_n, c = c_n;
                const float v = v_n;
                const bool is_short = short_n;
                if (i + 1 < n_rounds) fetch(i + 1);
                if (is_short) {
                    int n_max = 0;
#pragma unroll
                    for (int gg = 0; gg < G; ++gg) n_max = max(n_max, __builtin_amdgcn_readlane(len, gg * LPR));
                    float part[kTreeParts][VEC];
                    zero_acc<VEC, kTreeParts>(part);
                    GatherAddr<OFF32> addr = addr0;
                    addr.base = reinterpret_cast<const char*>(src_ptr<TS>(p.src) + p.src_hop_off[s] + src_col_begin - kBias);
                    accumulate_grouped<TS, VEC, LPR, OFF32>(c, v, len, n_max, lane, addr, part);
                    float tot[VEC];
                    combine_partials<VEC>(part, tot);
                    if (len >= 0) store_out<TD, VEC, EPI>(p, dst_ptr<TD>(p.dst) + (row0 + blk * G + g) * p.ld_dst + p.dst_hop_off[s], lcol, ecol, tot);
                } else {
                    for (int gg = 0; gg < G && blk * G + gg < rows_here; ++gg) row_wave_wide(blk * G + gg, s, s + 1);
                }
            }
        } else {
            auto block_short = [&](int blk_) {
                bool ok = true;
                for (int s_ = 0; s_ < n_sel; ++s_) {
                    int64_t b_;
                    int l_;
                    my_segment(s_, blk_, b_, l_);
                    ok = ok && __builtin_amdgcn_ballot_w64(l_ > short_max) == 0;
                }
                return ok;
            };
            int64_t begin_n = 0;
            int len_n = -1, c_n = 0;
            float v_n = 0.f;
            auto fetch = [&](int blk_, int s_, bool short_blk) {
                my_segment(s_, blk_, begin_n, len_n);
                c_n = 0;
                v_n = 0.f;
                if (short_blk && li < len_n) {
                    c_n = __builtin_nontemporal_load(p.hop[s_].colidx + begin_n + li);
                    v_n = __builtin_nontemporal_load(p.hop[s_].vals + begin_n + li);
                }
            };
            bool cur_short = n_blocks > 0 && block_short(0);
            if (n_blocks > 0) fetch(0, 0, cur_short);
            for (int blk = 0; blk < n_blocks; ++blk) {
                const bool nxt_short = blk + 1 < n_blocks && block_short(blk + 1);
                if (cur_short) {
                    float part[kTreeParts][VEC];
                    zero_acc<VEC, kTreeParts>(part);
                    bool valid = false;
                    for (int s = 0; s < n_sel; ++s) {
                        const int len = len_n, c = c_n;
                        const float v = v_n;
                        valid = len >= 0;
                        if (s + 1 < n_sel) fetch(blk, s + 1, true);
                        else if (blk + 1 < n_blocks) fetch(blk + 1, 0, nxt_short);
                        int n_max = 0;
#pragma unroll
                        for (int gg = 0; gg < G; ++gg) n_max = max(n_max, __builtin_amdgcn_readlane(len, gg * LPR));
                        GatherAddr<OFF32> addr = addr0;
                        addr.base = reinterpret_cast<const char*>(src_ptr<TS>(p.src) + p.src_hop_off[s] + src_col_begin - kBias);
                        accumulate_grouped<TS, VEC, LPR, OFF32>(c, v, len, n_max, lane, addr, part);
                    }
                    float tot[VEC];
                    combine_partials<VEC>(part, tot);
                    if (valid) store_out<TD, VEC, EPI>(p, dst_ptr<TD>(p.dst) + (row0 + blk * G + g) * p.ld_dst, lcol, ecol, tot);
                } else {
                    if (blk + 1 < n_blocks) fetch(blk + 1, 0, nxt_short);
                    for (int gg = 0; gg < G && blk * G + gg < rows_here; ++gg) row_wave_wide(blk * G + gg, 0, n_sel);
                }
                cur_short = nxt_short;
            }
        }
        return;
    }
}

template <typename T>
__device__ __forceinline__ T pick(int s, T of_hop0, T of_hop1) { return s ? of_hop1 : of_hop0; }

template <typename TS, typename TD, int VEC, int LPR, bool SUM, bool OFF32, bool EPI, int MAXB>
__device__ __forceinline__ void window_tile_walk(const LaunchParams& p, int lane, int rpw, int64_t row0, int rows_here, int64_t rp,
                                                 int64_t lane_off0, int64_t src_col_begin, int lcol, int ecol,
                                                 uint32_t (&ring)[kRingHops][2 * kRingCap]) {
    using off_t = typename std::conditional<OFF32, uint32_t, int64_t>::type;
    constexpr int NP = Tree<LPR>::NP;
    static_assert(kRingBlock == 4 * (kWave / 2) && kRingCap >= 2 * kRingBlock && kWave + 31 < kRingBlock, "ring safety (see above)");
    static_assert(kRingHops == 2, "hop state is selected with pick(s, hop 0's, hop 1's)");
    const int g = lane / LPR;
    const int n_sel = p.n_sel;
    const int half = lane >> 5, l4 = 4 * (lane & 31);
    auto misalign = [](const void* a) __attribute__((always_inline)) { return (int)((reinterpret_cast<uintptr_t>(a) >> 2) & 31); };
    const int32_t *col0 = nullptr, *col1 = nullptr;
    const float *val0 = nullptr, *val1 = nullptr;
    int len0 = 0, len1 = 0, mmin0 = 0, mmin1 = 0, mmax0 = 0, mmax1 = 0, blk0 = 0, blk1 = 0;
    int rel = 0;
    auto init_hop = [&](int s, const int32_t*& col, const float*& val, int& len, int& mmin, int& mmax) __attribute__((always_inline)) {
        const int l0 = s * (rpw + 1);
        const int rp_lo = (int)(rp & 0xffffffff), rp_hi = (int)(rp >> 32);
        const int64_t org = ((int64_t)__builtin_amdgcn_readlane(rp_hi, l0) << 32) | (uint32_t)__builtin_amdgcn_readlane(rp_lo, l0);
        if (lane >= l0) rel = (int)(rp - org);
        len = __builtin_amdgcn_readlane(rel, l0 + rows_here);
        col = p.hop[s].colidx + org;
        val = p.hop[s].vals + org;
        const int mc = misalign(col), mv = misalign(val);
        mmin = min(mc, mv);
        mmax = max(mc, mv);
    };
    init_hop(0, col0, val0, len0, mmin0, mmax0);
    if (n_sel > 1) init_hop(1, col1, val1, len1, mmin1, mmax1);
    auto bound = [&](int l) __attribute__((always_inline)) { return __builtin_amdgcn_readlane(rel, l); };
    auto lane_array = [&](int s) __attribute__((always_inline)) {
        return reinterpret_cast<const uint32_t*>(pick<const void*>(half, pick(s, col0, col1), pick(s, val0, val1)));
    };
    auto block_load = [&](int s, int blk) __attribute__((always_inline)) {
        const uint32_t* a = lane_array(s);
        const int hi = pick(s, len0, len1);
        const int x0 = blk * kRingBlock - misalign(a) + l4;
        u32x4 st = {0u, 0u, 0u, 0u};
        if (x0 >= 0 && x0 + 4 <= hi) {
            st = __builtin_nontemporal_load(reinterpret_cast<const u32x4*>(a + x0));
        } else {
#pragma unroll
            for (int i = 0; i < 4; ++i)
                if (x0 + i >= 0 && x0 + i < hi) st[i] = __builtin_nontemporal_load(a + (x0 + i));
        }
        return st;
    };
    auto block_commit = [&](int s, int blk, const u32x4& st) __attribute__((always_inline)) {
        const int x0 = blk * kRingBlock - misalign(lane_array(s)) + l4;
        uint32_t* slots = ring[s];
#pragma unroll
        for (int i = 0; i < 4; ++i) slots[2 * ((uint32_t)(x0 + i) & (kRingCap - 1)) + half] = st[i];
        __builtin_amdgcn_fence(__ATOMIC_RELEASE, "wavefront");
        __builtin_amdgcn_wave_barrier();
        __builtin_amdgcn_fence(__ATOMIC_ACQUIRE, "wavefront");
    };
    auto blk_of = [&](int s) __attribute__((always_inline)) { return pick(s, blk0, blk1); };
    auto set_blk = [&](int s, int b) __attribute__((always_inline)) {
        if (s) blk1 = b;
        else blk0 = b;
    };
    auto avail = [&](int s, int blk) __attribute__((always_inline)) { return blk * kRingBlock - pick(s, mmax0, mmax1); };

    const int n_seg = rows_here * n_sel;
    uint32_t skip = 0;
    for (int q = 0; q < n_seg; ++q) {
        const int r = q / n_sel, s_ = q - r * n_sel;
        const int l0 = s_ * (rpw + 1) + r;
        if (bound(l0 + 1) - bound(l0) >= p.long_threshold) skip |= SUM ? (((1u << n_sel) - 1u) << (r * n_sel)) : (1u << q);
    }
    float acc[NP][VEC];
    zero_acc<VEC, NP>(acc);
    for (int q = 0; q < n_seg; ++q) {
        const int r = q / n_sel, s = q - r * n_sel;
        const int l0 = s * (rpw + 1) + r;
        const int sb = bound(l0), se = bound(l0 + 1);
        const bool skipped = (skip >> q) & 1u;
        if (skipped) {
            const int b = (se + pick(s, mmin0, mmin1)) / kRingBlock;
            if (b > blk_of(s)) set_blk(s, b);
        } else {
            const GatherAddr<OFF32> addr{reinterpret_cast<const char*>(src_ptr<TS>(p.src) + p.src_hop_off[s] + src_col_begin - VEC),
                                         (off_t)lane_off0, (off_t)(p.ld_src * sizeof(TS))};
            for (int base = sb; base < se; base += kWave) {
                const int n = min(se - base, kWave);
                for (int b = blk_of(s); base + n > avail(s, b); set_blk(s, ++b)) {
                    const u32x4 st = block_load(s, b);
                    block_commit(s, b, st);
                }
                int ps = s, pb = base + kWave, pe = se;
                if (pb >= se) {
                    pb = pe = 0;
                    if (q + 1 < n_seg && !((skip >> (q + 1)) & 1u)) {
                        const int r1 = (q + 1) / n_sel;
                        ps = q + 1 - r1 * n_sel;
                        pb = bound(ps * (rpw + 1) + r1);
                        pe = bound(ps * (rpw + 1) + r1 + 1);
                    }
                }
                const bool refill = pb < pe && min(pb + kWave, pe) > avail(ps, blk_of(ps));
                u32x4 st = {0u, 0u, 0u, 0u};
                if (refill) st = block_load(ps, blk_of(ps));
                process_chunk_window<TS, VEC, LPR, false, OFF32, MAXB>(WindowChunk{ring[s], (uint32_t)(base + g)}, n, g, addr, true, acc);
                if (refill) {
                    block_commit(ps, blk_of(ps), st);
                    set_blk(ps, blk_of(ps) + 1);
                }
            }
        }
        if (!SUM || s == n_sel - 1) {
            if (!skipped) {
                float tot[VEC];
                fold_tree<VEC, LPR, NP>(acc, tot);
                if (g == 0) store_out<TD, VEC, EPI>(p, dst_ptr<TD>(p.dst) + (row0 + r) * p.ld_dst + (SUM ? 0 : p.dst_hop_off[s]), lcol, ecol, tot);
            }
            zero_acc<VEC, NP>(acc);
        }
    }
}

template <int LPR, bool EXACT, bool PIPE, bool SHORT, bool EPI, bool LISTS>
constexpr bool uses_index_window() {
    return EXACT && !SHORT && !LISTS && !PIPE && !EPI && LPR == 16;
}

template <int VEC, int LPR, bool EXACT, bool SUM, bool OFF32, bool PIPE, bool SHORT, bool EPI, int FB, bool LISTS, typename TS>
constexpr int min_waves_per_simd() {
    if (!EXACT) return 2;
    if (SHORT) return FB == 4 && !SUM ? H2GCN_SHORT_FB4_MIN_WAVES : H2GCN_SHORT_MIN_WAVES;
    const bool bf16_less = std::is_same<TS, bf16>::value && VEC == 4 &&
                           (LISTS ? FB == 4 && SUM && !OFF32 : (OFF32 && EPI && LPR == 32) || (SUM && OFF32 && PIPE && LPR == 16));
    if (LISTS && FB == 4) return H2GCN_SHORT_FB4_MIN_WAVES - bf16_less;
    const bool heavy = VEC == 4 && (LISTS ? (SUM && (!OFF32 || LPR >= 32)) || (!OFF32 && LPR >= 32) : !OFF32 || (PIPE && LPR == 32));
    if (heavy) return H2GCN_OFF64_HEAVY_MIN_WAVES - bf16_less;
    return (LPR >= 32 ? H2GCN_WIDE_MIN_WAVES : kMinWavesPerSimd) - bf16_less;
}

template <int VEC, int LPR, bool EXACT, bool SUM, bool OFF32, bool PIPE = false, bool SHORT = false, bool EPI = false, int FB = 8, bool LISTS = false,
          typename TS = float, typename TD = float>
__global__ __launch_bounds__(kBlock, (min_waves_per_simd<VEC, LPR, EXACT, SUM, OFF32, PIPE, SHORT, EPI, FB, LISTS, TS>())) void spmm_hops_kernel(const LaunchParams p) {
    static_assert(!LISTS || (EXACT && !SHORT && !PIPE && (LPR == 16 || LPR == 32)), "list-driven launches exist for 64- and 128-column slices");
    static_assert(EXACT || LPR == kWave, "column-tiled path uses the whole wave per row");
    __shared__ float partial[kWavesPerBlock][kMaxTileCols];
    using off_t = typename std::conditional<OFF32, uint32_t, int64_t>::type;
    constexpr int NP = Tree<LPR>::NP;
    constexpr int kMainB = LISTS ? FB : (LPR >= 32 ? H2GCN_WIDE_MAXB : H2GCN_MAIN_MAXB);

    const int lane = threadIdx.x & (kWave - 1);
    const int wave = wave_uniform(threadIdx.x >> 6);
    const int li = lane % LPR;
    const int g = lane / LPR;
    const int n_sel = p.n_sel;

    const int64_t bid = blockIdx.x;
    const int slice = EXACT ? (int)(bid / p.blocks_per_slice) : 0;
    const int64_t b = EXACT ? bid - (int64_t)slice * p.blocks_per_slice : bid;
    const int col_begin = EXACT ? slice * (VEC * LPR) : 0;
    const int col_end = EXACT ? col_begin + VEC * LPR : p.d;
    const int64_t src_col_begin = EXACT ? (int64_t)slice * p.src_slice_stride : 0;
    const int lcol = col_begin + li * VEC;
    const int ecol = EXACT ? ((lcol + VEC <= p.d_src) ? lcol : p.d_src - VEC) : lcol;
    const off_t lane_off0 = (off_t)((ecol - col_begin + VEC) * (int)sizeof(TS));
    constexpr int kBias = EXACT ? VEC : 0;

    if (b < p.n_long) {
        const int64_t entry = p.long_list[b];
        const int64_t row = SUM ? entry : (entry >> 4);
        const int s_first = SUM ? 0 : (int)(entry & 15);
        const int s_last = SUM ? n_sel : s_first + 1;
        for (int col0 = col_begin; col0 < col_end; col0 += VEC * LPR) {
            const bool lane_active = EXACT || (col0 + li * VEC < p.d);
            float acc[NP][VEC];
            zero_acc<VEC, NP>(acc);
            for (int s = s_first; s < s_last; ++s) {
                const HopCsr& h = p.hop[s];
                const int64_t sb = h.rowptr[row], se = h.rowptr[row + 1];
                const GatherAddr<OFF32> addr{reinterpret_cast<const char*>(src_ptr<TS>(p.src) + p.src_hop_off[s] + src_col_begin + (col0 - col_begin) - kBias),
                                             EXACT ? lane_off0 : (off_t)(li * VEC * (int)sizeof(TS)), (off_t)(p.ld_src * sizeof(TS))};
                accumulate_segment<TS, VEC, LPR, !EXACT, OFF32, kMainB>(h.colidx, h.vals, sb, se, wave, kWavesPerBlock, addr, lane,
                                                            lane_active, acc);
            }
            float tot[VEC];
            fold_tree<VEC, LPR, NP>(acc, tot);
            if (g == 0) {
                const int rel = EXACT ? ecol - col_begin : li * VEC;
                if (!EXACT || lcol < p.d_src) {
#pragma unroll
                    for (int i = 0; i < VEC; ++i)
                        if (rel + i >= 0) partial[wave][rel + i] = tot[i];
                }
            }
            __syncthreads();
            const int c = threadIdx.x;
            if (c < VEC * LPR && col0 + c < p.d) {
                float t = partial[0][c];
#pragma unroll
                for (int w = 1; w < kWavesPerBlock; ++w) t += partial[w][c];
                const int64_t off = row * p.ld_dst + (SUM ? 0 : p.dst_hop_off[s_first]) + col0 + c;
                if constexpr (EPI) {
                    if constexpr (std::is_same<TD, float>::value)
                        if (p.accumulate) t += dst_ptr<float>(p.dst)[off];
                    if (p.bias) t += p.bias[col0 + c];
                    if (p.relu) t = relu_keep_nan(t);
                }
                store_one<TD>(dst_ptr<TD>(p.dst) + off, t);
            }
            if (!EXACT) __syncthreads();
        }
        return;
    }

    const int64_t tb = b - p.n_long;
    int64_t tile;
    if constexpr (LISTS) {
        __shared__ uint64_t s_seg[kWavesPerBlock][kShortSumHops][kWave];
        __shared__ int32_t s_row[kWavesPerBlock][kWave];
        const int64_t q = tb >> 3;
        const int i8 = (int)(tb & 7);
        const int64_t n_groups = p.short_groups + p.med_groups;
        const int64_t s_before = (q * p.short_groups) / n_groups;
        if (((q + 1) * p.short_groups) / n_groups > s_before)
            short_list_blocks<TS, TD, VEC, LPR, SUM, OFF32, EPI, H2GCN_SHORT_PREFETCH>(p, s_before * kNumXcd + i8, lane, wave, (int64_t)lane_off0,
                                                                               src_col_begin, lcol, ecol, s_seg, s_row);
        else
            medium_list_blocks<TS, TD, VEC, LPR, SUM, OFF32, EPI, FB>(p, (q - s_before) * kNumXcd + i8, lane, wave, (int64_t)lane_off0,
                                                              src_col_begin, lcol, ecol);
        return;
    } else {
        tile = (tb % kNumXcd) * p.tiles_per_xcd + tb / kNumXcd;
    }
    if (tile >= p.n_tiles) return;
    const int rpw = p.rows_per_wave;
    const int64_t row0 = (tile * kWavesPerBlock + wave) * rpw;
    if (row0 >= p.n_rows) return;
    const int64_t rows_here_l = p.n_rows - row0;
    const int rows_here = rows_here_l < rpw ? (int)rows_here_l : rpw;

    int64_t rp = 0;
    {
        const int hs = lane / (rpw + 1), r = lane % (rpw + 1);
        if (hs < n_sel && r <= rows_here) rp = p.hop[hs].rowptr[row0 + r];
    }
    const int rp_lo = (int)(rp & 0xffffffff), rp_hi = (int)(rp >> 32);
    auto seg_bound = [&](int l) -> int64_t {
        return ((int64_t)__builtin_amdgcn_readlane(rp_hi, l) << 32) | (uint32_t)__builtin_amdgcn_readlane(rp_lo, l);
    };

    if constexpr (SHORT && EXACT && (kWave / LPR == 2 || kWave / LPR == 4)) {
        in_tile_short_rows<TS, TD, VEC, LPR, SUM, OFF32, EPI, FB>(p, lane, rpw, row0, rows_here, rp_lo, rp_hi, (int64_t)lane_off0, src_col_begin, lcol, ecol);
        return;
    }
    if constexpr (uses_index_window<LPR, EXACT, PIPE, SHORT, EPI, LISTS>()) {
        __shared__ uint32_t ring[kWavesPerBlock][kRingHops][2 * kRingCap];
        bool fits = n_sel <= kRingHops;
#pragma unroll
        for (int s = 0; s < kRingHops; ++s)
            if (s < n_sel && seg_bound(s * (rpw + 1) + rows_here) - seg_bound(s * (rpw + 1)) > kRingMaxRange) fits = false;
        if (fits) {
            window_tile_walk<TS, TD, VEC, LPR, SUM, OFF32, EPI, kMainB>(p, lane, rpw, row0, rows_here, rp, (int64_t)lane_off0, src_col_begin, lcol, ecol,
                                                                        ring[wave]);
            return;
        }
    }
    if constexpr (PIPE && EXACT) {
        const int n_seg = rows_here * n_sel;
        uint32_t skip = 0;
        for (int q = 0; q < n_seg; ++q) {
            const int r = q / n_sel, s_ = q - r * n_sel;
            const int l0 = s_ * (rpw + 1) + r;
            if (seg_bound(l0 + 1) - seg_bound(l0) >= p.long_threshold) skip |= SUM ? (((1u << n_sel) - 1u) << (r * n_sel)) : (1u << q);
        }
        auto seg = [&](int q, int& s_, int64_t& sb, int64_t& se) {
            const int r = q / n_sel;
            s_ = q - r * n_sel;
            const int l0 = s_ * (rpw + 1) + r;
            sb = seg_bound(l0);
            se = (skip >> q) & 1u ? sb : seg_bound(l0 + 1);
        };
        int s_cur, s_nxt = 0;
        int64_t b_cur, e_cur, b_nxt = 0, e_nxt = 0;
        int c_cur, c_nxt = 0;
        float v_cur, v_nxt = 0.f;
        seg(0, s_nxt, b_nxt, e_nxt);
        load_chunk(p.hop[s_nxt].colidx, p.hop[s_nxt].vals, b_nxt, e_nxt, lane, c_nxt, v_nxt);
        float acc[NP][VEC];
        zero_acc<VEC, NP>(acc);
        for (int q = 0; q < n_seg; ++q) {
            s_cur = s_nxt; b_cur = b_nxt; e_cur = e_nxt; c_cur = c_nxt; v_cur = v_nxt;
            if (q + 1 < n_seg) {
                seg(q + 1, s_nxt, b_nxt, e_nxt);
                load_chunk(p.hop[s_nxt].colidx, p.hop[s_nxt].vals, b_nxt, e_nxt, lane, c_nxt, v_nxt);
            }
            const int r = q / n_sel;
            const int64_t row = row0 + r;
            const HopCsr& h = p.hop[s_cur];
            const GatherAddr<OFF32> addr{reinterpret_cast<const char*>(src_ptr<TS>(p.src) + p.src_hop_off[s_cur] + src_col_begin - kBias),
                                         lane_off0, (off_t)(p.ld_src * sizeof(TS))};
            accumulate_segment_prefetched<TS, VEC, LPR, OFF32>(h.colidx, h.vals, b_cur, e_cur, c_cur, v_cur, addr, lane, acc);
            const bool skipped = (skip >> q) & 1u;
            if (!SUM || s_cur == n_sel - 1) {
                if (!skipped) {
                    float tot[VEC];
                    fold_tree<VEC, LPR, NP>(acc, tot);
                    if (g == 0) store_out<TD, VEC, EPI>(p, dst_ptr<TD>(p.dst) + row * p.ld_dst + (SUM ? 0 : p.dst_hop_off[s_cur]), lcol, ecol, tot);
                }
                zero_acc<VEC, NP>(acc);
            }
        }
        return;
    }

#ifdef H2GCN_AB_STORE_BEHIND_FETCH
    if constexpr (EXACT && !SUM && !EPI) {
        float held[VEC];
        int64_t held_off = 0;
        bool held_valid = false;
        for (int r = 0; r < rows_here; ++r) {
            const int64_t row = row0 + r;
            for (int s = 0; s < n_sel; ++s) {
                const int l0 = s * (rpw + 1) + r;
                const int64_t sb = seg_bound(l0), se = seg_bound(l0 + 1);
                if (se - sb >= p.long_threshold) continue;
                const HopCsr& h = p.hop[s];
                int c;
                float v;
                load_chunk(h.colidx, h.vals, sb, se, lane, c, v);
                if (held_valid) {
                    if (g == 0) store_out<TD, VEC, EPI>(p, dst_ptr<TD>(p.dst) + held_off, lcol, ecol, held);
                    held_valid = false;
                }
                float acc[NP][VEC];
                zero_acc<VEC, NP>(acc);
                const GatherAddr<OFF32> addr{reinterpret_cast<const char*>(src_ptr<TS>(p.src) + p.src_hop_off[s] + src_col_begin - kBias), lane_off0, (off_t)(p.ld_src * sizeof(TS))};
                accumulate_segment_prefetched<TS, VEC, LPR, OFF32, kMainB>(h.colidx, h.vals, sb, se, c, v, addr, lane, acc);
                fold_tree<VEC, LPR, NP>(acc, held);
                held_off = row * p.ld_dst + p.dst_hop_off[s];
                held_valid = true;
            }
        }
        if (held_valid && g == 0) store_out<TD, VEC, EPI>(p, dst_ptr<TD>(p.dst) + held_off, lcol, ecol, held);
        return;
    }
#endif

    for (int r = 0; r < rows_here; ++r) {
        const int64_t row = row0 + r;
        if constexpr (SUM) {
            bool skip_row = false;
            for (int s = 0; s < n_sel; ++s) {
                const int l0 = s * (rpw + 1) + r;
                const int64_t len = seg_bound(l0 + 1) - seg_bound(l0);
                if (len >= p.long_threshold) skip_row = true;
            }
            if (skip_row) continue;
        }
        for (int col0 = col_begin; col0 < col_end; col0 += VEC * LPR) {
            const bool lane_active = EXACT || (col0 + li * VEC < p.d);
            float acc[NP][VEC];
            zero_acc<VEC, NP>(acc);
#ifdef H2GCN_DEFER_HOP_STORES
            float held[VEC];
            int held_s = -1;
#endif
            for (int s = 0; s < n_sel; ++s) {
                const int l0 = s * (rpw + 1) + r;
                const int64_t sb = seg_bound(l0), se = seg_bound(l0 + 1);
                if (!SUM && se - sb >= p.long_threshold) continue;
                const HopCsr& h = p.hop[s];
                const GatherAddr<OFF32> addr{reinterpret_cast<const char*>(src_ptr<TS>(p.src) + p.src_hop_off[s] + src_col_begin + (col0 - col_begin) - kBias),
                                             EXACT ? lane_off0 : (off_t)(li * VEC * (int)sizeof(TS)), (off_t)(p.ld_src * sizeof(TS))};
                accumulate_segment<TS, VEC, LPR, !EXACT, OFF32, kMainB>(h.colidx, h.vals, sb, se, 0, 1, addr, lane, lane_active, acc);
                if constexpr (!SUM) {
                    float tot[VEC];
                    fold_tree<VEC, LPR, NP>(acc, tot);
#ifdef H2GCN_DEFER_HOP_STORES
                    if (EXACT && n_sel == 2 && s == 0) {
#pragma unroll
                        for (int i = 0; i < VEC; ++i) held[i] = tot[i];
                        held_s = 0;
                    } else {
                        if (held_s >= 0 && g == 0 && lane_active)
                            store_out<TD, VEC, EPI>(p, dst_ptr<TD>(p.dst) + row * p.ld_dst + p.dst_hop_off[held_s], lcol, ecol, held);
                        held_s = -1;
                        if (g == 0 && lane_active)
                            store_out<TD, VEC, EPI>(p, dst_ptr<TD>(p.dst) + row * p.ld_dst + p.dst_hop_off[s], EXACT ? lcol : col0 + li * VEC, EXACT ? ecol : col0 + li * VEC, tot);
                    }
#else
                    if (g == 0 && lane_active)
                        store_out<TD, VEC, EPI>(p, dst_ptr<TD>(p.dst) + row * p.ld_dst + p.dst_hop_off[s], EXACT ? lcol : col0 + li * VEC, EXACT ? ecol : col0 + li * VEC, tot);
#endif
                    zero_acc<VEC, NP>(acc);
                }
            }
#ifdef H2GCN_DEFER_HOP_STORES
            if constexpr (!SUM)
                if (held_s >= 0 && g == 0 && lane_active)
                    store_out<TD, VEC, EPI>(p, dst_ptr<TD>(p.dst) + row * p.ld_dst + p.dst_hop_off[held_s], lcol, ecol, held);
#endif
            if constexpr (SUM) {
                float tot[VEC];
                fold_tree<VEC, LPR, NP>(acc, tot);
                if (g == 0 && lane_active)
                    store_out<TD, VEC, EPI>(p, dst_ptr<TD>(p.dst) + row * p.ld_dst, EXACT ? lcol : col0 + li * VEC, EXACT ? ecol : col0 + li * VEC, tot);
            }
        }
    }
}

template <bool VEC4>
__global__ void repack_slice_major_kernel(const float* __restrict__ x, int64_t ld, int64_t ld_hop, int n_hop, int64_t n_rows,
                                          int d, int n_slices, int slice_cols, float* __restrict__ w) {
    using f4 = float __attribute__((ext_vector_type(4)));
    constexpr int E = VEC4 ? 4 : 1;
    const int cu = slice_cols / E;
    const int64_t per_hop = n_rows * cu;
    const int64_t per_slice = per_hop * n_hop;
    const int64_t total = per_slice * n_slices;
    for (int64_t i = (int64_t)blockIdx.x * blockDim.x + threadIdx.x; i < total; i += (int64_t)gridDim.x * blockDim.x) {
        const int q = (int)(i / per_slice);
        const int64_t i1 = i - q * per_slice;
        const int s = (int)(i1 / per_hop);
        const int64_t i2 = i1 - s * per_hop;
        const int64_t r = i2 / cu;
        const int c = (int)(i2 - r * cu);
        const int col = q * slice_cols + c * E;
        const float* src = x + r * ld + s * ld_hop + col;
        if constexpr (VEC4) {
            f4 v = {0.f, 0.f, 0.f, 0.f};
            if (col < d) v = *reinterpret_cast<const f4*>(src);
            __builtin_nontemporal_store(v, reinterpret_cast<f4*>(w) + i);
        } else {
            __builtin_nontemporal_store(col < d ? *src : 0.f, w + i);
        }
    }
}

struct Schedule {
    bool exact;
    bool scalar128;
    bool pipe;
    bool shortrow;
    bool lists;
    bool fb4;
    bool gen;
    bool off32;
    int slice;
};


template <int VEC, int LPR, bool EXACT, bool SUM, typename TS, typename TD>
void launch_tile_walk(const LaunchParams& p, const Schedule& k, dim3 grid, hipStream_t stream) {
    const dim3 block(kBlock);
    const bool pipe = EXACT && k.pipe;
    if (k.gen && k.off32)
        hipLaunchKernelGGL((spmm_hops_kernel<VEC, LPR, EXACT, SUM, true, false, false, true, 8, false, TS, TD>), grid, block, 0, stream, p);
    else if (k.gen)
        hipLaunchKernelGGL((spmm_hops_kernel<VEC, LPR, EXACT, SUM, false, false, false, true, 8, false, TS, TD>), grid, block, 0, stream, p);
    else if (k.off32 && !pipe)
        hipLaunchKernelGGL((spmm_hops_kernel<VEC, LPR, EXACT, SUM, true, false, false, false, 8, false, TS, TD>), grid, block, 0, stream, p);
    else if (!pipe)
        hipLaunchKernelGGL((spmm_hops_kernel<VEC, LPR, EXACT, SUM, false, false, false, false, 8, false, TS, TD>), grid, block, 0, stream, p);
    else if constexpr (EXACT) {
        if (k.off32)
            hipLaunchKernelGGL((spmm_hops_kernel<VEC, LPR, EXACT, SUM, true, true, false, false, 8, false, TS, TD>), grid, block, 0, stream, p);
        else
            hipLaunchKernelGGL((spmm_hops_kernel<VEC, LPR, EXACT, SUM, false, true, false, false, 8, false, TS, TD>), grid, block, 0, stream, p);
    }
}

template <int LPR, bool SUM, typename TS, typename TD>
void launch_list_driven(const LaunchParams& p, const Schedule& k, dim3 grid, hipStream_t stream) {
    const dim3 block(kBlock);
    if (k.off32 && k.fb4)
        hipLaunchKernelGGL((spmm_hops_kernel<4, LPR, true, SUM, true, false, false, false, 4, true, TS, TD>), grid, block, 0, stream, p);
    else if (k.off32)
        hipLaunchKernelGGL((spmm_hops_kernel<4, LPR, true, SUM, true, false, false, false, 8, true, TS, TD>), grid, block, 0, stream, p);
    else if (k.fb4)
        hipLaunchKernelGGL((spmm_hops_kernel<4, LPR, true, SUM, false, false, false, false, 4, true, TS, TD>), grid, block, 0, stream, p);
    else
        hipLaunchKernelGGL((spmm_hops_kernel<4, LPR, true, SUM, false, false, false, false, 8, true, TS, TD>), grid, block, 0, stream, p);
}

template <int LPR, bool SUM, typename TS, typename TD>
void launch_in_tile_short_rows(const LaunchParams& p, const Schedule& k, dim3 grid, hipStream_t stream) {
    const dim3 block(kBlock);
    if (k.off32 && k.fb4)
        hipLaunchKernelGGL((spmm_hops_kernel<4, LPR, true, SUM, true, false, true, false, 4, false, TS, TD>), grid, block, 0, stream, p);
    else if (k.off32)
        hipLaunchKernelGGL((spmm_hops_kernel<4, LPR, true, SUM, true, false, true, false, 8, false, TS, TD>), grid, block, 0, stream, p);
    else if (k.fb4)
        hipLaunchKernelGGL((spmm_hops_kernel<4, LPR, true, SUM, false, false, true, false, 4, false, TS, TD>), grid, block, 0, stream, p);
    else
        hipLaunchKernelGGL((spmm_hops_kernel<4, LPR, true, SUM, false, false, true, false, 8, false, TS, TD>), grid, block, 0, stream, p);
}

template <bool SUM, typename TS, typename TD>
void launch_spmm(const LaunchParams& p, const Schedule& k, dim3 grid, hipStream_t stream) {
    if (k.shortrow && k.slice == 128) launch_in_tile_short_rows<32, SUM, TS, TD>(p, k, grid, stream);
    else if (k.shortrow) launch_in_tile_short_rows<16, SUM, TS, TD>(p, k, grid, stream);
    else if (k.scalar128) launch_tile_walk<2, 64, true, SUM, TS, TD>(p, k, grid, stream);
    else if (k.slice == 256) launch_tile_walk<4, 64, true, SUM, TS, TD>(p, k, grid, stream);
    else if (k.lists && k.slice == 128) launch_list_driven<32, SUM, TS, TD>(p, k, grid, stream);
    else if (k.lists) launch_list_driven<16, SUM, TS, TD>(p, k, grid, stream);
    else if (k.slice == 128) launch_tile_walk<4, 32, true, SUM, TS, TD>(p, k, grid, stream);
    else if (k.slice == 64) launch_tile_walk<4, 16, true, SUM, TS, TD>(p, k, grid, stream);
    else launch_tile_walk<1, 64, false, SUM, TS, TD>(p, k, grid, stream);
}

}
```

h2gcn_amd/hops.py:

```python
from __future__ import annotations

import ctypes as C
from typing import Iterable, Optional, Sequence

import torch

from . import _capi


def _require(cond: bool, msg: str) -> None:
    if not cond:
        raise ValueError(msg)


def _bf16_layout(name: str, t: torch.Tensor, d: int, strides) -> None:
    _require(d % 2 == 0, f"bf16 {name}: the feature width d must be even (got {d})")
    _require(t.data_ptr() % 4 == 0, f"bf16 {name}: the base address must be 4-byte aligned")
    for st in strides:
        _require(st % 2 == 0, f"bf16 {name}: row / hop strides must be even (got {tuple(strides)} elements)")


def _bf16_symbols() -> None:
    _require(_capi.has("h2gcn_spmm_hops_bf16"), f"{_capi.library_path()} predates the bf16 launches (ABI 5)")


class HopPlan:

    def __init__(self, rowptr: Sequence[torch.Tensor], colidx: Sequence[torch.Tensor],
                 vals: Sequence[torch.Tensor], n_cols: int, *, build_transpose: bool = False,
                 long_row_threshold: int = 0, rows_per_wave: int = 0, variant: int = 0,
                 slice_cols: int = 0, validate: bool = True, host_transpose: bool = False,
                 keep_permutation: bool = False, symmetric_pattern: bool = False):
        H = len(rowptr)
        _require(1 <= H <= _capi.MAX_HOPS, f"need 1..{_capi.MAX_HOPS} hop matrices, got {H}")
        _require(len(colidx) == H and len(vals) == H, "rowptr/colidx/vals lists differ in length")
        dev = rowptr[0].device
        _require(dev.type == "cuda", f"HopPlan operands must live on a GPU, got {dev} (no CPU fallback)")
        n_rows = rowptr[0].numel() - 1
        _require(n_rows >= 0, "rowptr must have n_rows+1 entries")
        for k in range(H):
            rp, ci, va = rowptr[k], colidx[k], vals[k]
            _require(rp.dtype == torch.int64 and ci.dtype == torch.int32 and va.dtype == torch.float32,
                     f"hop {k}: dtypes must be int64/int32/float32, got {rp.dtype}/{ci.dtype}/{va.dtype}")
            _require(rp.device == dev and ci.device == dev and va.device == dev, f"hop {k}: operands on different devices")
            _require(rp.dim() == 1 and rp.numel() == n_rows + 1, f"hop {k}: rowptr has {rp.numel()} entries, expected {n_rows + 1}")
            _require(ci.dim() == 1 and va.dim() == 1 and ci.numel() == va.numel(), f"hop {k}: colidx/vals sizes differ")
            _require(rp.is_contiguous() and ci.is_contiguous() and va.is_contiguous(), f"hop {k}: operands must be contiguous")
        if symmetric_pattern:
            _require(build_transpose, "symmetric_pattern=True modifies build_transpose=True, which is not set")
            _require(not host_transpose, "symmetric_pattern=True builds no transpose: it cannot be combined with host_transpose=True")
            _require(n_rows == int(n_cols), f"symmetric_pattern=True needs square operands, got {n_rows} x {int(n_cols)}")
            if not _capi.has("h2gcn_plan_transpose_sharing"):
                raise RuntimeError(f"{_capi.library_path()} predates symmetric plans (H2GCN_PLAN_SYMMETRIC_PATTERN)")
        self._tunables = dict(long_row_threshold=long_row_threshold, rows_per_wave=rows_per_wave, variant=variant, slice_cols=slice_cols)
        self.n_hops = H
        self.n_rows = int(n_rows)
        self.n_cols = int(n_cols)
        self.device = dev
        self.has_transpose = bool(build_transpose)
        self.keep_permutation = bool(keep_permutation and build_transpose)
        self.rowptr = list(rowptr)
        self.colidx = list(colidx)
        self.vals = list(vals)
        self._handle = C.c_void_p()
        self.use_workspace = True
        self.min_chunk_cols = 16

        L = _capi.lib()
        arr_t = C.c_void_p * H
        rp_a = arr_t(*[t.data_ptr() for t in self.rowptr])
        ci_a = arr_t(*[t.data_ptr() for t in self.colidx])
        va_a = arr_t(*[t.data_ptr() for t in self.vals])
        opts = _capi.PlanOpts()
        opts.struct_size = C.sizeof(_capi.PlanOpts)
        opts.flags = ((_capi.PLAN_BUILD_TRANSPOSE if build_transpose else 0) | (0 if validate else _capi.PLAN_SKIP_VALIDATION)
                      | (_capi.PLAN_HOST_TRANSPOSE if host_transpose else 0)
                      | (_capi.PLAN_KEEP_PERMUTATION if keep_permutation and build_transpose else 0)
                      | (_capi.PLAN_SYMMETRIC_PATTERN if symmetric_pattern else 0))
        opts.long_row_threshold = int(long_row_threshold)
        opts.rows_per_wave = int(rows_per_wave)
        opts.variant = int(variant)
        opts.slice_cols = int(slice_cols)
        with torch.cuda.device(dev):
            stream = torch.cuda.current_stream(dev).cuda_stream
            st = L.h2gcn_plan_create(H, self.n_rows, self.n_cols, rp_a, ci_a, va_a, C.byref(opts),
                                     C.c_void_p(stream), C.byref(self._handle))
        _capi.check(st)

    @classmethod
    def from_scipy(cls, mats: Iterable, device, **kw) -> "HopPlan":
        import numpy as np
        import scipy.sparse as sp

        rowptr, colidx, vals = [], [], []
        n_cols = None
        n_rows = None
        for m in mats:
            m = sp.csr_matrix(m)
            m.sum_duplicates()
            m.sort_indices()
            _require(n_cols in (None, m.shape[1]) and n_rows in (None, m.shape[0]), "hop matrices differ in shape")
            n_rows, n_cols = m.shape
            rowptr.append(torch.from_numpy(m.indptr.astype(np.int64)).to(device))
            colidx.append(torch.from_numpy(m.indices.astype(np.int32)).to(device))
            vals.append(torch.from_numpy(m.data.astype(np.float32)).to(device))
        _require(n_cols is not None, "empty hop list")
        return cls(rowptr, colidx, vals, n_cols, **kw)

    def set_values(self, hop: int, vals: torch.Tensor) -> None:
        _require(vals.dtype == torch.float32 and vals.device == self.device and vals.is_contiguous()
                 and vals.numel() == self.colidx[hop].numel(), "vals must be a contiguous float32 array of the hop's nnz")
        with torch.cuda.device(self.device):
            stream = torch.cuda.current_stream(self.device).cuda_stream
            _capi.check(_capi.lib().h2gcn_plan_set_values(self._handle, int(hop), C.c_void_p(vals.data_ptr()), C.c_void_p(stream)))
        self.vals[hop] = vals
        self.values_version = getattr(self, "values_version", 0) + 1

    def select_rows(self, rows, build_transpose: bool = True) -> "RowSelection":
        _require(self.device.type == "cuda", f"select_rows: the plan must live on a GPU, got {self.device} (no CPU fallback)")
        t = rows if isinstance(rows, torch.Tensor) else torch.as_tensor(rows)
        if t.dtype == torch.bool:
            _require(t.dim() == 1 and t.numel() == self.n_rows, f"select_rows: a bool mask must have shape [{self.n_rows}], got {tuple(t.shape)}")
            idx = torch.nonzero(t.to(self.device)).flatten()
            _require(idx.numel() > 0, "select_rows: empty selection")
        else:
            _require(not (t.is_floating_point() or t.is_complex()), f"select_rows: rows must be a bool mask or integer indices, got {t.dtype}")
            _require(t.dim() == 1, f"select_rows: an index tensor must be one-dimensional, got shape {tuple(t.shape)}")
            _require(t.numel() > 0, "select_rows: empty selection")
            idx = torch.sort(t.to(self.device, torch.int64)).values
            lo, hi = int(idx[0]), int(idx[-1])
            _require(lo >= 0 and hi < self.n_rows, f"select_rows: row index {lo if lo < 0 else hi} outside [0, {self.n_rows})")
            _require(not bool((idx[1:] == idx[:-1]).any()), "select_rows: duplicate row indices")
        m = int(idx.numel())
        rowptr, colidx, vals = [], [], []
        for k in range(self.n_hops):
            rp = self.rowptr[k]
            begin = rp[idx]
            lens = rp[idx + 1] - begin
            sub_rp = torch.zeros(m + 1, dtype=torch.int64, device=self.device)
            torch.cumsum(lens, 0, out=sub_rp[1:])
            nnz = int(sub_rp[-1])
            src = torch.arange(nnz, dtype=torch.int64, device=self.device) + torch.repeat_interleave(begin - sub_rp[:-1], lens, output_size=nnz)
            rowptr.append(sub_rp)
            colidx.append(self.colidx[k][src].contiguous())
            vals.append(self.vals[k][src].contiguous())
        plan = HopPlan(rowptr, colidx, vals, self.n_cols, build_transpose=build_transpose, validate=False, **self._tunables)
        return RowSelection(idx.to(torch.int32), plan, self.n_rows)

    @property
    def nnz(self) -> list:
        return [int(t.numel()) for t in self.colidx]

    def info(self, hop: int) -> dict:
        L = _capi.lib()
        n_rows, n_cols, nnz, n_long = C.c_int64(), C.c_int64(), C.c_int64(), C.c_int64()
        has_t = C.c_int32()
        _capi.check(L.h2gcn_plan_info(self._handle, hop, C.byref(n_rows), C.byref(n_cols), C.byref(nnz),
                                      C.byref(n_long), C.byref(has_t)))
        return dict(n_rows=n_rows.value, n_cols=n_cols.value, nnz=nnz.value, n_long_segments=n_long.value,
                    has_transpose=bool(has_t.value))

    @property
    def transpose_sharing(self) -> list:
        if not _capi.has("h2gcn_plan_transpose_sharing"):
            return ["none"] * self.n_hops
        L = _capi.lib()
        out = []
        for k in range(self.n_hops):
            v = L.h2gcn_plan_transpose_sharing(self._handle, k)
            _capi.check(v)
            out.append(("none", "indices", "indices+values")[v])
        return out

    def device_bytes(self) -> int:
        if not _capi.has("h2gcn_plan_device_bytes"):
            raise RuntimeError(f"{_capi.library_path()} predates h2gcn_plan_device_bytes")
        return int(_capi.lib().h2gcn_plan_device_bytes(self._handle))

    def schedule(self, d: int, ld_src: Optional[int] = None, hops=None, adjoint: bool = False) -> dict:
        L = _capi.lib()
        sc, ns, pf, cp = C.c_int32(), C.c_int32(), C.c_int32(), C.c_int32()
        ld = int(ld_src) if ld_src is not None else (self.n_selected(hops) * d if adjoint else d)
        _capi.check(L.h2gcn_plan_schedule(self._handle, self._mask(hops), 1 if adjoint else 0, ld, int(d),
                                          C.byref(sc), C.byref(ns), C.byref(pf), C.byref(cp)))
        return dict(slice_cols=sc.value, n_slices=ns.value,
                    segment_walk={0: "wave per segment", 1: "wave per segment + index prefetch",
                                  2: "lane group per segment (short rows)",
                                  3: "lane group per segment (binned short segments) + wave per segment"}[pf.value],
                    scratch_copy=bool(cp.value) and self.use_workspace)

    def segment_classes(self, d: int, ld_src: Optional[int] = None, hops=None, adjoint: bool = False) -> dict:
        L = _capi.lib()
        if not _capi.has("h2gcn_plan_segment_classes"):
            raise RuntimeError(f"{_capi.library_path()} predates h2gcn_plan_segment_classes (ABI 4)")
        h_sel = self.n_selected(hops)
        seg, nnz, listed = (C.c_int64 * (3 * h_sel))(), (C.c_int64 * (3 * h_sel))(), C.c_int64()
        ld = int(ld_src) if ld_src is not None else (h_sel * d if adjoint else d)
        _capi.check(L.h2gcn_plan_segment_classes(self._handle, self._mask(hops), 1 if adjoint else 0, ld, int(d), seg, nnz, C.byref(listed)))
        sel = self._selected(hops)
        short_walk = ("lane group per segment (binned list)" if listed.value > 0 else
                      "lane group per segment (rounds of consecutive short rows)" if listed.value < 0 else "wave per segment")
        per_hop = [dict(hop=sel[s], segments=dict(short=seg[3 * s], medium=seg[3 * s + 1], long=seg[3 * s + 2]),
                        nonzeros=dict(short=nnz[3 * s], medium=nnz[3 * s + 1], long=nnz[3 * s + 2])) for s in range(h_sel)]
        return dict(per_hop=per_hop, listed=listed.value,
                    walks=dict(short=short_walk, medium="wave per segment", long="workgroup per segment (4 waves, LDS-staged)"))

    def _mask(self, hops) -> int:
        if hops is None:
            return 0
        mask = 0
        for h in hops:
            _require(0 <= int(h) < self.n_hops, f"hop index {h} outside 0..{self.n_hops - 1}")
            mask |= 1 << int(h)
        _require(mask != 0, "empty hop selection")
        return mask

    def _selected(self, hops) -> list:
        return list(range(self.n_hops)) if hops is None else sorted({int(h) for h in hops})

    def n_selected(self, hops) -> int:
        return self.n_hops if hops is None else bin(self._mask(hops)).count("1")

    def spmm(self, x: torch.Tensor, hops=None, out: Optional[torch.Tensor] = None, bias: Optional[torch.Tensor] = None,
             relu: bool = False, out_dtype: Optional[torch.dtype] = None) -> torch.Tensor:
        _require(x.dim() == 2, f"inputs must be [n_cols, d], got shape {tuple(x.shape)}")
        _require(x.dtype in (torch.float32, torch.bfloat16), f"inputs must be float32 or bfloat16, got {x.dtype}")
        _require(x.device == self.device, f"inputs on {x.device}, plan on {self.device}")
        _require(x.shape[0] == self.n_cols, f"inputs have {x.shape[0]} rows, hop matrices have {self.n_cols} columns")
        d = int(x.shape[1])
        _require(d >= 1, "inputs need at least one column")
        bf16 = x.dtype == torch.bfloat16
        if out_dtype is None:
            out_dtype = out.dtype if out is not None else x.dtype
        _require(out_dtype in (torch.float32, torch.bfloat16), f"outputs must be float32 or bfloat16, got {out_dtype}")
        _require(bf16 or out_dtype == torch.float32, "float32 inputs give float32 outputs (float32 -> bfloat16 is not supported)")
        if x.stride(1) != 1:
            x = x.contiguous()
        h_sel = self.n_selected(hops)
        if out is None:
            out = torch.empty((self.n_rows, h_sel, d), dtype=out_dtype, device=self.device)
        else:
            _require(out.dtype == out_dtype and out.device == self.device, f"out must be {out_dtype} on the plan's device")
            _require(tuple(out.shape) == (self.n_rows, h_sel, d), f"out has shape {tuple(out.shape)}, expected {(self.n_rows, h_sel, d)}")
            _require(d == 1 or out.stride(2) == 1, "out's last dimension must be contiguous")
        if bf16:
            _bf16_symbols()
            _bf16_layout("inputs", x, d, (x.stride(0),))
            if out_dtype == torch.bfloat16:
                _bf16_layout("out", out, d, (out.stride(0), out.stride(1) if h_sel > 1 else d))
        if self.n_rows == 0:
            return out
        if bias is not None:
            _require(bias.dtype == torch.float32 and bias.device == self.device and bias.numel() == d and bias.is_contiguous(),
                     f"bias must be a contiguous float32 [{d}] tensor on the plan's device")
        L = _capi.lib()
        mask = self._mask(hops)
        with torch.cuda.device(self.device):
            stream = torch.cuda.current_stream(self.device).cuda_stream
            ws_bytes = (int(L.h2gcn_spmm_workspace_bytes(self._handle, mask, 0, C.c_void_p(x.data_ptr()), x.stride(0), 0, d))
                        if self.use_workspace and not bf16 else 0)
            ws = torch.empty(ws_bytes, dtype=torch.uint8, device=self.device) if ws_bytes else None
            opts = None
            if ws is not None or bias is not None or relu:
                opts = _capi.LaunchOpts(struct_size=C.sizeof(_capi.LaunchOpts), flags=_capi.LAUNCH_RELU if relu else 0,
                                        workspace=ws.data_ptr() if ws is not None else None, workspace_bytes=ws_bytes,
                                        bias=bias.data_ptr() if bias is not None else None)
            fn, y_dtype = ((L.h2gcn_spmm_hops_bf16, (_capi.DTYPE_BF16 if out_dtype == torch.bfloat16 else _capi.DTYPE_F32,))
                           if bf16 else (L.h2gcn_spmm_hops_opts_f32, ()))
            st = fn(self._handle, mask, C.c_void_p(x.data_ptr()), x.stride(0), d, *y_dtype,
                    C.c_void_p(out.data_ptr()), out.stride(0), out.stride(1) if h_sel > 1 else d,
                    C.byref(opts) if opts is not None else None, C.c_void_p(stream))
        _capi.check(st)
        return out

    def spmm_t(self, grad: torch.Tensor, hops=None, out: torch.Tensor = None, accumulate: bool = False,
               out_dtype: Optional[torch.dtype] = None) -> torch.Tensor:
        _require(self.has_transpose, "plan was built without build_transpose=True; backward is unavailable")
        h_sel = self.n_selected(hops)
        _require(grad.dim() == 3 and grad.shape[0] == self.n_rows and grad.shape[1] == h_sel,
                 f"grad must be [{self.n_rows}, {h_sel}, d], got {tuple(grad.shape)}")
        _require(grad.dtype in (torch.float32, torch.bfloat16) and grad.device == self.device,
                 "grad must be float32 or bfloat16 on the plan's device")
        d = int(grad.shape[2])
        bf16 = grad.dtype == torch.bfloat16
        if out_dtype is None:
            out_dtype = out.dtype if out is not None else grad.dtype
        _require(out_dtype in (torch.float32, torch.bfloat16), f"dx must be float32 or bfloat16, got {out_dtype}")
        _require(bf16 or out_dtype == torch.float32, "a float32 grad gives a float32 dx (float32 -> bfloat16 is not supported)")
        _require(not (accumulate and out_dtype == torch.bfloat16), "accumulate=True needs a float32 out (a bfloat16 dx cannot be accumulated into)")
        if grad.stride(2) != 1 or grad.stride(0) < d or (h_sel > 1 and grad.stride(1) < d):
            grad = grad.contiguous()
        if out is None:
            _require(not accumulate, "accumulate=True needs the tensor to accumulate into (out=)")
            dx = torch.empty((self.n_cols, d), dtype=out_dtype, device=self.device)
        else:
            _require(out.shape == (self.n_cols, d) and out.dtype == out_dtype and out.device == self.device
                     and (out.stride(1) == 1 or d == 1) and (out.stride(0) >= d or self.n_cols <= 1),
                     f"out must be {out_dtype} [{self.n_cols}, {d}] on the plan's device with unit column stride")
            dx = out
        if bf16:
            _bf16_symbols()
            _bf16_layout("grad", grad, d, (grad.stride(0) if self.n_rows > 0 else h_sel * d, grad.stride(1) if h_sel > 1 else d))
            if out_dtype == torch.bfloat16:
                _bf16_layout("dx", dx, d, (dx.stride(0) if self.n_cols > 1 else d,))
        if self.n_cols == 0:
            return dx
        L = _capi.lib()
        mask = self._mask(hops)
        ld_row, ld_hop = (grad.stride(0) if self.n_rows > 0 else h_sel * d), (grad.stride(1) if h_sel > 1 else d)
        with torch.cuda.device(self.device):
            stream = torch.cuda.current_stream(self.device).cuda_stream
            ws_bytes = (int(L.h2gcn_spmm_workspace_bytes(self._handle, mask, 1, C.c_void_p(grad.data_ptr()), ld_row, ld_hop, d))
                        if self.use_workspace and not bf16 else 0)
            opts = None
            if ws_bytes or accumulate:
                ws = torch.empty(ws_bytes, dtype=torch.uint8, device=self.device) if ws_bytes else None
                opts = _capi.LaunchOpts(struct_size=C.sizeof(_capi.LaunchOpts), flags=_capi.LAUNCH_ACCUMULATE if accumulate else 0,
                                        workspace=ws.data_ptr() if ws is not None else None, workspace_bytes=ws_bytes, bias=None)
            fn, dx_dtype = ((L.h2gcn_spmm_hops_T_bf16, (_capi.DTYPE_BF16 if out_dtype == torch.bfloat16 else _capi.DTYPE_F32,))
                            if bf16 else (L.h2gcn_spmm_hops_T_opts_f32, ()))
            st = fn(self._handle, mask, C.c_void_p(grad.data_ptr()), ld_row, ld_hop, d, *dx_dtype,
                    C.c_void_p(dx.data_ptr()), dx.stride(0) if self.n_cols > 1 else d,
                    C.byref(opts) if opts is not None else None, C.c_void_p(stream))
        _capi.check(st)
        return dx

# ... 258 lines not shown
```

include/h2gcn_hip.h:

```cpp
#ifndef H2GCN_HIP_H_
#define H2GCN_HIP_H_

#include <stddef.h>
#include <stdint.h>

#ifdef __cplusplus
extern "C" {
#endif

#define H2GCN_ABI_VERSION 5
#define H2GCN_MAX_HOPS 8

typedef enum h2gcn_status {
    H2GCN_OK = 0,
    H2GCN_ERR_INVALID_ARGUMENT = -1,
    H2GCN_ERR_HIP = -2,
    H2GCN_ERR_OUT_OF_MEMORY = -3,
    H2GCN_ERR_BAD_INDEX = -4,
    H2GCN_ERR_NO_TRANSPOSE = -5,
    H2GCN_ERR_INTERNAL = -6,
    H2GCN_ERR_EXCHANGE_TIMEOUT = -7
} h2gcn_status;

#define H2GCN_PLAN_BUILD_TRANSPOSE 0x1u
#define H2GCN_PLAN_SKIP_VALIDATION 0x2u
#define H2GCN_PLAN_HOST_TRANSPOSE  0x4u

#define H2GCN_PLAN_KEEP_PERMUTATION 0x8u

#define H2GCN_PLAN_SYMMETRIC_PATTERN 0x10u

typedef struct h2gcn_plan_opts {
    uint32_t struct_size;
    uint32_t flags;
    int32_t long_row_threshold;
    int32_t rows_per_wave;
    int32_t variant;
    int32_t slice_cols;
    int32_t reserved[2];
} h2gcn_plan_opts;

typedef struct h2gcn_plan h2gcn_plan_t;

int h2gcn_abi_version(void);

const char* h2gcn_last_error(void);

int h2gcn_device_count(void);

int h2gcn_plan_create(int n_hops, int64_t n_rows, int64_t n_cols,
                      const int64_t* const* rowptr_dev, const int32_t* const* colidx_dev,
                      const float* const* vals_dev, const h2gcn_plan_opts* opts, void* stream,
                      h2gcn_plan_t** out_plan);

void h2gcn_plan_destroy(h2gcn_plan_t* plan);

int h2gcn_plan_set_values(h2gcn_plan_t* plan, int hop, const float* vals_dev, void* stream);

int h2gcn_plan_info(const h2gcn_plan_t* plan, int hop, int64_t* n_rows, int64_t* n_cols, int64_t* nnz,
                    int64_t* n_long_segments, int32_t* has_transpose);

int h2gcn_plan_transpose_sharing(const h2gcn_plan_t* plan, int hop);

size_t h2gcn_plan_device_bytes(const h2gcn_plan_t* plan);

int h2gcn_plan_schedule(const h2gcn_plan_t* plan, uint32_t hop_mask, int adjoint, int64_t ld_src, int32_t d,
                        int32_t* slice_cols, int32_t* n_slices, int32_t* segment_walk, int32_t* scratch_copy);

int h2gcn_plan_segment_classes(const h2gcn_plan_t* plan, uint32_t hop_mask, int adjoint, int64_t ld_src, int32_t d,
                               int64_t* segments, int64_t* nonzeros, int64_t* listed);

int h2gcn_spmm_hops_f32(const h2gcn_plan_t* plan, uint32_t hop_mask, const float* X_dev, int64_t ldx,
                        int32_t d, float* Y_dev, int64_t ldy_row, int64_t ldy_hop, void* stream);

#define H2GCN_LAUNCH_RELU 0x1u
#define H2GCN_LAUNCH_ACCUMULATE 0x2u
typedef struct h2gcn_launch_opts {
    uint32_t struct_size;
    uint32_t flags;
    void* workspace_dev;
    size_t workspace_bytes;
    const float* bias_dev;
} h2gcn_launch_opts;
size_t h2gcn_spmm_workspace_bytes(const h2gcn_plan_t* plan, uint32_t hop_mask, int adjoint, const float* src_dev,
                                  int64_t ld_src, int64_t ld_src_hop, int32_t d);
int h2gcn_spmm_hops_opts_f32(const h2gcn_plan_t* plan, uint32_t hop_mask, const float* X_dev, int64_t ldx,
                             int32_t d, float* Y_dev, int64_t ldy_row, int64_t ldy_hop,
                             const h2gcn_launch_opts* opts, void* stream);

int h2gcn_spmm_hops_T_f32(const h2gcn_plan_t* plan, uint32_t hop_mask, const float* dY_dev, int64_t ldg_row,
                          int64_t ldg_hop, int32_t d, float* dX_dev, int64_t ldx, void* stream);
int h2gcn_spmm_hops_T_opts_f32(const h2gcn_plan_t* plan, uint32_t hop_mask, const float* dY_dev, int64_t ldg_row,
                               int64_t ldg_hop, int32_t d, float* dX_dev, int64_t ldx,
                               const h2gcn_launch_opts* opts, void* stream);

#define H2GCN_DTYPE_F32 0
#define H2GCN_DTYPE_BF16 1
int h2gcn_spmm_hops_bf16(const h2gcn_plan_t* plan, uint32_t hop_mask, const uint16_t* X_dev, int64_t ldx, int32_t d,
                         int y_dtype, void* Y_dev, int64_t ldy_row, int64_t ldy_hop, const h2gcn_launch_opts* opts, void* stream);
int h2gcn_spmm_hops_T_bf16(const h2gcn_plan_t* plan, uint32_t hop_mask, const uint16_t* dY_dev, int64_t ldg_row, int64_t ldg_hop,
                           int32_t d, int dx_dtype, void* dX_dev, int64_t ldx, const h2gcn_launch_opts* opts, void* stream);

int h2gcn_sddmm_hops_f32(const h2gcn_plan_t* plan, uint32_t hop_mask, const float* dY_dev, int64_t ldg_row, int64_t ldg_hop,
                         const float* X_dev, int64_t ldx, int32_t d, float* const* dvals_dev, void* stream);
int h2gcn_sddmm_hops_bf16(const h2gcn_plan_t* plan, uint32_t hop_mask, const uint16_t* dY_dev, int64_t ldg_row, int64_t ldg_hop,
                          const uint16_t* X_dev, int64_t ldx, int32_t d, float* const* dvals_dev, void* stream);

int h2gcn_row_softmax_hops_f32(const h2gcn_plan_t* plan, uint32_t hop_mask, const float* const* scores_dev,
                               float* const* alpha_dev, void* stream);
int h2gcn_row_softmax_backward_hops_f32(const h2gcn_plan_t* plan, uint32_t hop_mask, const float* const* alpha_dev,
                                        const float* const* dalpha_dev, float* const* dscores_dev, void* stream);

int h2gcn_edge_scores_hops_f32(const h2gcn_plan_t* plan, uint32_t hop_mask, const float* l_dev, int64_t ldl,
                               const float* r_dev, int64_t ldr, float negative_slope, float* const* scores_dev, void* stream);
int h2gcn_edge_scores_backward_hops_f32(const h2gcn_plan_t* plan, uint32_t hop_mask, const float* l_dev, int64_t ldl,
                                        const float* r_dev, int64_t ldr, float negative_slope, const float* const* dscores_dev,
                                        float* dl_dev, int64_t lddl, float* dr_dev, int64_t lddr, void* stream);

int h2gcn_spmm_hops_values_f32(const h2gcn_plan_t* plan, uint32_t hop_mask, const float* const* values_dev, const int64_t* ldv_entry,
                               const int64_t* ldv_head, int32_t n_heads, const float* X_dev, int64_t ldx, int32_t d, float* Y_dev,
                               int64_t ldy_row, int64_t ldy_hop, void* stream);
int h2gcn_spmm_hops_T_values_f32(const h2gcn_plan_t* plan, uint32_t hop_mask, const float* const* values_dev, const int64_t* ldv_entry,
                                 const int64_t* ldv_head, int32_t n_heads, const float* dY_dev, int64_t ldg_row, int64_t ldg_hop, int32_t d,
                                 float* dX_dev, int64_t ldx, void* stream);

size_t h2gcn_ring_scratch_bytes(int64_t n);
int h2gcn_ring_count(int64_t n, const int64_t* a_rowptr_dev, const int32_t* a_colidx_dev,
                     const int64_t* f_rowptr_dev, const int32_t* f_colidx_dev,
                     int n_add, const int64_t* const* add_rowptr_dev, const int32_t* const* add_colidx_dev, int add_diag,
                     int n_sub, const int64_t* const* sub_rowptr_dev, const int32_t* const* sub_colidx_dev, int sub_diag,
                     int64_t* out_rowptr_dev, int64_t* nnz_out, void* scratch_dev, size_t scratch_bytes, void* stream);
int h2gcn_ring_fill(int64_t n, const int64_t* a_rowptr_dev, const int32_t* a_colidx_dev,
                    const int64_t* f_rowptr_dev, const int32_t* f_colidx_dev,
                    int n_add, const int64_t* const* add_rowptr_dev, const int32_t* const* add_colidx_dev, int add_diag,
                    int n_sub, const int64_t* const* sub_rowptr_dev, const int32_t* const* sub_colidx_dev, int sub_diag,
                    const int64_t* out_rowptr_dev, int32_t* out_colidx_dev, void* scratch_dev, size_t scratch_bytes,
                    void* stream);
int h2gcn_ring_count_rows(int64_t n, int64_t row_begin, int64_t n_rows, const int64_t* a_rowptr_dev, const int32_t* a_colidx_dev,
                          const int64_t* f_rowptr_dev, const int32_t* f_colidx_dev,
                          int n_add, const int64_t* const* add_rowptr_dev, const int32_t* const* add_colidx_dev, int add_diag,
                          int n_sub, const int64_t* const* sub_rowptr_dev, const int32_t* const* sub_colidx_dev, int sub_diag,
                          int64_t* out_rowptr_dev, int64_t* nnz_out, void* scratch_dev, size_t scratch_bytes, void* stream);
int h2gcn_ring_fill_rows(int64_t n, int64_t row_begin, int64_t n_rows, const int64_t* a_rowptr_dev, const int32_t* a_colidx_dev,
                         const int64_t* f_rowptr_dev, const int32_t* f_colidx_dev,
                         int n_add, const int64_t* const* add_rowptr_dev, const int32_t* const* add_colidx_dev, int add_diag,
                         int n_sub, const int64_t* const* sub_rowptr_dev, const int32_t* const* sub_colidx_dev, int sub_diag,
                         const int64_t* out_rowptr_dev, int32_t* out_colidx_dev, void* scratch_dev, size_t scratch_bytes,
                         void* stream);
int h2gcn_hop_normalize(int64_t n, const int64_t* rowptr_dev, const int32_t* colidx_dev, int mode,
                        const double* s_table_dev, int64_t s_table_len, float* vals_dev, void* stream);
int h2gcn_hop_normalize_rows(int64_t n_rows, const int64_t* rowptr_dev, const int32_t* colidx_dev, int mode,
                             const double* s_table_dev, int64_t s_table_len, const int64_t* col_len_dev,
                             float* vals_dev, void* stream);

int64_t h2gcn_dropout_dense_small_rows(int64_t rows);
size_t h2gcn_dropout_dense_workspace_bytes(int64_t n_rows, int32_t k, int32_t c);
int h2gcn_dropout_dense_f32(const float* X_dev, int64_t ldx, int64_t n_rows, int32_t k, const float* W_dev, int32_t c,
                            const float* bias_dev, float keep_prob, uint64_t seed, const int64_t* step_dev,
                            float* Z_dev, int64_t ldz, void* workspace_dev, size_t workspace_bytes, void* stream);
int h2gcn_dropout_dense_backward_f32(const float* X_dev, int64_t ldx, int64_t n_rows, int32_t k, const float* W_dev, int32_t c,
                                     const float* G_dev, int64_t ldg, float keep_prob, uint64_t seed, const int64_t* step_dev,
                                     float* dX_dev, int64_t lddx, float* dW_dev, void* workspace_dev, size_t workspace_bytes,
                                     void* stream);
int h2gcn_dropout_dense_bf16(const uint16_t* X_dev, int64_t ldx, int64_t n_rows, int32_t k, const float* W_dev, int32_t c,
                             const float* bias_dev, float keep_prob, uint64_t seed, const int64_t* step_dev,
                             float* Z_dev, int64_t ldz, void* workspace_dev, size_t workspace_bytes, void* stream);
int h2gcn_dropout_dense_backward_bf16(const uint16_t* X_dev, int64_t ldx, int64_t n_rows, int32_t k, const float* W_dev, int32_t c,
                                      const float* G_dev, int64_t ldg, float keep_prob, uint64_t seed, const int64_t* step_dev,
                                      int dx_dtype, void* dX_dev, int64_t lddx, float* dW_dev, void* workspace_dev,
                                      size_t workspace_bytes, void* stream);
int h2gcn_dropout_dense_rows_f32(const float* X_dev, int64_t ldx, int64_t n_rows, int32_t k, const float* W_dev, int32_t c,
                                 const float* bias_dev, float keep_prob, uint64_t seed, const int64_t* step_dev,
                                 float* Z_dev, int64_t ldz, void* workspace_dev, size_t workspace_bytes, void* stream,
                                 const int32_t* rows_dev, int64_t n_sel);
int h2gcn_dropout_dense_rows_bf16(const uint16_t* X_dev, int64_t ldx, int64_t n_rows, int32_t k, const float* W_dev, int32_t c,
                                  const float* bias_dev, float keep_prob, uint64_t seed, const int64_t* step_dev,
                                  float* Z_dev, int64_t ldz, void* workspace_dev, size_t workspace_bytes, void* stream,
                                  const int32_t* rows_dev, int64_t n_sel);
int h2gcn_dropout_dense_backward_rows_f32(const float* X_dev, int64_t ldx, int64_t n_rows, int32_t k, const float* W_dev, int32_t c,
                                          const float* G_dev, int64_t ldg, float keep_prob, uint64_t seed, const int64_t* step_dev,
                                          float* dX_dev, int64_t lddx, float* dW_dev, void* workspace_dev, size_t workspace_bytes,
                                          void* stream, const int32_t* rows_dev, int64_t n_sel);
int h2gcn_dropout_dense_backward_rows_bf16(const uint16_t* X_dev, int64_t ldx, int64_t n_rows, int32_t k, const float* W_dev, int32_t c,
                                           const float* G_dev, int64_t ldg, float keep_prob, uint64_t seed, const int64_t* step_dev,
                                           int dx_dtype, void* dX_dev, int64_t lddx, float* dW_dev, void* workspace_dev,
                                           size_t workspace_bytes, void* stream, const int32_t* rows_dev, int64_t n_sel);

#define H2GCN_METRICS_MAX_SETS 4
size_t h2gcn_masked_metrics_workspace_bytes(int64_t n_rows);
int h2gcn_masked_metrics_f32(const float* Z_dev, int64_t ldz, int64_t n_rows, int32_t c, int32_t n_sets, const float* const* Y_dev,
                             const int64_t* ldy, const float* const* w_dev, float* loss_out_dev, float* acc_out_dev,
                             void* workspace_dev, size_t workspace_bytes, void* stream);
int h2gcn_masked_ce_backward_f32(const float* Z_dev, int64_t ldz, int64_t n_rows, int32_t c, const float* Y_dev, int64_t ldy,
                                 const float* w_dev, const float* gscale_dev, float* dZ_dev, int64_t lddz, void* stream);

#define H2GCN_ADAM_MAX_TENSORS 16
int h2gcn_adam_keras_f32(int32_t n_tensors, float* const* params_dev, const float* const* grads_dev, float* const* m_dev,
                         float* const* v_dev, const int64_t* sizes, float lr, float beta1, float beta2, float epsilon,
                         const int64_t* step_dev, int64_t step, void* stream);

int h2gcn_adam_keras_l2_f32(int32_t n_tensors, float* const* params_dev, const float* const* grads_dev, float* const* m_dev,
                            float* const* v_dev, const int64_t* sizes, const float* l2, float lr, float beta_1, float beta_2,
                            float epsilon, const int64_t* step_dev, int64_t step, void* stream);
size_t h2gcn_l2_penalty_workspace_bytes(void);
int h2gcn_l2_penalty_f32(int32_t n_tensors, const float* const* params_dev, const int64_t* sizes, const float* l2,
                         float* out_dev, void* workspace_dev, size_t workspace_bytes, void* stream);

typedef struct h2gcn_xchg h2gcn_xchg_t;

#define H2GCN_XCHG_BLOB_BYTES 192
#define H2GCN_XCHG_COPY_ENGINE 0
#define H2GCN_XCHG_COPY_KERNEL 1

int h2gcn_xchg_create(int world, int rank, int n_channels, size_t slot_bytes, int mode, int timeout_ms,
                      h2gcn_xchg_t** out);
// ... 22 lines not shown
```

Before: 13.90 billion.

## Use per-row constant edge values to skip per-edge value loads in SpMM

At plan creation, each hop's CSR is scanned to find out whether every row has a single repeated edge value (for example row-normalized adjacency). If so, one value per row is stored. The forward f32 index-window kernel then loads only column indices and applies that per-row weight, instead of streaming per-edge values and keeping them in the LDS ring. This cuts global memory traffic and halves ring shared memory, at the cost of an extra preprocessing kernel, more kernel instantiations, and invalidating the row values when plan values are later set.

```diff
diff --git a/h2gcn_amd/_capi.py b/h2gcn_amd/_capi.py
--- a/h2gcn_amd/_capi.py
+++ b/h2gcn_amd/_capi.py
@@ -39,6 +39,7 @@
     "h2gcn_plan_info",
     "h2gcn_plan_set_values",
     "h2gcn_plan_transpose_sharing",
+    "h2gcn_plan_row_constant",
     "h2gcn_plan_device_bytes",
     "h2gcn_spmm_hops_f32",
     "h2gcn_spmm_hops_T_f32",
@@ -190,6 +191,9 @@
         L.h2gcn_plan_transpose_sharing.argtypes = [C.c_void_p, C.c_int]
         L.h2gcn_plan_device_bytes.restype = C.c_size_t
         L.h2gcn_plan_device_bytes.argtypes = [C.c_void_p]
+    if hasattr(L, "h2gcn_plan_row_constant"):
+        L.h2gcn_plan_row_constant.restype = C.c_int
+        L.h2gcn_plan_row_constant.argtypes = [C.c_void_p, C.c_int]
     L.h2gcn_spmm_workspace_bytes.restype = C.c_size_t
     L.h2gcn_spmm_workspace_bytes.argtypes = [C.c_void_p, C.c_uint32, C.c_int, C.c_void_p, C.c_int64, C.c_int64, C.c_int32]
     L.h2gcn_spmm_hops_opts_f32.restype = C.c_int
diff --git a/h2gcn_amd/csrc/h2gcn_capi.hip b/h2gcn_amd/csrc/h2gcn_capi.hip
--- a/h2gcn_amd/csrc/h2gcn_capi.hip
+++ b/h2gcn_amd/csrc/h2gcn_capi.hip
@@ -93,6 +93,8 @@
     std::deque<DeviceBuf> owned;
     std::vector<int> sharing;
     size_t transpose_bytes = 0;
+    std::vector<DeviceBuf> rowval;
+    std::vector<char> row_const;
     mutable std::mutex mu;
     mutable std::map<uint64_t, LongList> long_cache;
     mutable std::map<uint64_t, ClassLists> class_cache;
@@ -106,6 +108,21 @@
     for (int64_t i = (int64_t)blockIdx.x * blockDim.x + threadIdx.x; i < nnz; i += (int64_t)gridDim.x * blockDim.x) {
         const int32_t c = colidx[i];
         bad |= (c < 0) | ((int64_t)c >= n_cols);
+    }
+    if (bad) atomicOr(flag, 1);
+}
+
+__global__ void row_values_kernel(const int64_t* __restrict__ rowptr, const float* __restrict__ vals, int64_t n_rows,
+                                  float* __restrict__ rowval, int* flag) {
+    const int lane = threadIdx.x & (kWave - 1);
+    const int64_t n_waves = ((int64_t)gridDim.x * blockDim.x) / kWave;
+    const uint32_t* v = reinterpret_cast<const uint32_t*>(vals);
+    int bad = 0;
+    for (int64_t r = ((int64_t)blockIdx.x * blockDim.x + threadIdx.x) / kWave; r < n_rows; r += n_waves) {
+        const int64_t b = rowptr[r], e = rowptr[r + 1];
+        const uint32_t first = b < e ? v[b] : 0u;
+        for (int64_t i = b + lane; i < e; i += kWave) bad |= v[i] != first;
+        if (lane == 0) reinterpret_cast<uint32_t*>(rowval)[r] = first;
     }
     if (bad) atomicOr(flag, 1);
 }
@@ -475,12 +492,20 @@
     if (n_blocks <= 0) return H2GCN_OK;
     if (n_blocks > 0x7fffffffLL) return fail(H2GCN_ERR_INVALID_ARGUMENT, "grid too large (%lld blocks)", (long long)n_blocks);
     const dim3 grid((unsigned)n_blocks);
-    if (!src_bf16 && adjoint) launch_spmm<true, float, float>(p, sc, grid, stream);
-    else if (!src_bf16) launch_spmm<false, float, float>(p, sc, grid, stream);
-    else if (out_bf16 && adjoint) launch_spmm<true, bf16, bf16>(p, sc, grid, stream);
-    else if (out_bf16) launch_spmm<false, bf16, bf16>(p, sc, grid, stream);
-    else if (adjoint) launch_spmm<true, bf16, float>(p, sc, grid, stream);
-    else launch_spmm<false, bf16, float>(p, sc, grid, stream);
+    Schedule rv = sc;
+    rv.rowval = !adjoint && !out_bf16 && sc.exact && sc.slice == 64 && !sc.scalar128 && !sc.pipe && !sc.shortrow && !sc.lists &&
+                !sc.gen && p.n_sel <= kRingHops;
+    for (int k = 0, s = 0; rv.rowval && k < plan->n_hops; ++k) {
+        if (!(mask & (1u << k))) continue;
+        if (plan->row_const[(size_t)k] && plan->rowval[(size_t)k].p) p.rowval[s++] = (const float*)plan->rowval[(size_t)k].p;
+        else rv.rowval = false;
+    }
+    if (!src_bf16 && adjoint) launch_spmm<true, float, float>(p, rv, grid, stream);
+    else if (!src_bf16) launch_spmm<false, float, float>(p, rv, grid, stream);
+    else if (out_bf16 && adjoint) launch_spmm<true, bf16, bf16>(p, rv, grid, stream);
+    else if (out_bf16) launch_spmm<false, bf16, bf16>(p, rv, grid, stream);
+    else if (adjoint) launch_spmm<true, bf16, float>(p, rv, grid, stream);
+    else launch_spmm<false, bf16, float>(p, rv, grid, stream);
     H2GCN_HIP_TRY(hipGetLastError());
     return H2GCN_OK;
 }
@@ -646,6 +671,8 @@
         DeviceBuf flag;
         H2GCN_HIP_TRY(hipMalloc(&flag.p, sizeof(int)));
         H2GCN_HIP_TRY(hipMemsetAsync(flag.p, 0, sizeof(int), stream));
+        plan->rowval.resize(n_hops);
+        plan->row_const.assign(n_hops, 0);
 
         std::vector<std::vector<int64_t>> h_rowptr(n_hops);
         for (int k = 0; k < n_hops; ++k) {
@@ -754,6 +781,30 @@
             plan->has_transpose = true;
         }
         {
+            DeviceBuf rc_flag;
+            H2GCN_HIP_TRY(hipMalloc(&rc_flag.p, (size_t)n_hops * sizeof(int)));
+            H2GCN_HIP_TRY(hipMemsetAsync(rc_flag.p, 0, (size_t)n_hops * sizeof(int), stream));
+            for (int k = 0; k < n_hops; ++k) {
+                const HopOperand& op = plan->fwd[k];
+                H2GCN_HIP_TRY(hipMalloc(&plan->rowval[k].p, (size_t)std::max<int64_t>(n_rows, 1) * sizeof(float)));
+                if (n_rows == 0) continue;
+                const unsigned blocks = (unsigned)std::min<int64_t>((n_rows + h2gcn::kWavesPerBlock - 1) / h2gcn::kWavesPerBlock, 8192);
+                hipLaunchKernelGGL(h2gcn::row_values_kernel, dim3(blocks), dim3(h2gcn::kBlock), 0, stream, op.rowptr, op.vals, n_rows,
+                                   (float*)plan->rowval[k].p, (int*)rc_flag.p + k);
+                H2GCN_HIP_TRY(hipGetLastError());
+            }
+            std::vector<int> h_rc((size_t)n_hops, 0);
+            H2GCN_HIP_TRY(hipMemcpyAsync(h_rc.data(), rc_flag.p, h_rc.size() * sizeof(int), hipMemcpyDeviceToHost, stream));
+            H2GCN_HIP_TRY(hipStreamSynchronize(stream));
+            for (int k = 0; k < n_hops; ++k) {
+                plan->row_const[k] = h_rc[k] ? 0 : 1;
+                if (!plan->row_const[k]) {
+                    (void)hipFree(plan->rowval[k].p);
+                    plan->rowval[k].p = nullptr;
+                }
+            }
+        }
+        {
             const uint32_t all = n_hops >= 32 ? 0xffffffffu : ((1u << n_hops) - 1u);
             const int64_t* unused_p = nullptr;
             int unused_n = 0;
@@ -799,6 +850,15 @@
         H2GCN_HIP_TRY(hipGetLastError());
     }
     f.vals = vals_dev;
+    plan->row_const[(size_t)hop] = 0;
+    if (plan->rowval[(size_t)hop].p) {
+        hipStreamCaptureStatus cs = hipStreamCaptureStatusNone;
+        if (hipStreamIsCapturing((hipStream_t)stream_v, &cs) != hipSuccess) (void)hipGetLastError();
+        else if (cs == hipStreamCaptureStatusNone) {
+            (void)hipFree(plan->rowval[(size_t)hop].p);
+            plan->rowval[(size_t)hop].p = nullptr;
+        }
+    }
     return H2GCN_OK;
 }
 
@@ -820,10 +880,18 @@
     return plan->sharing[(size_t)hop];
 }
 
+int h2gcn_plan_row_constant(const h2gcn_plan_t* plan, int hop) {
+    if (!plan) return fail(H2GCN_ERR_INVALID_ARGUMENT, "plan is NULL");
+    if (hop < 0 || hop >= plan->n_hops) return fail(H2GCN_ERR_INVALID_ARGUMENT, "hop %d outside 0..%d", hop, plan->n_hops - 1);
+    return plan->row_const[(size_t)hop] ? 1 : 0;
+}
+
 size_t h2gcn_plan_device_bytes(const h2gcn_plan_t* plan) {
     if (!plan) return 0;
     std::lock_guard<std::mutex> lock(plan->mu);
     size_t bytes = plan->transpose_bytes;
+    for (const DeviceBuf& rv : plan->rowval)
+        if (rv.p) bytes += (size_t)std::max<int64_t>(plan->n_rows, 1) * sizeof(float);
     for (const auto& kv : plan->long_cache) bytes += (size_t)kv.second.n * sizeof(int64_t);
     for (const auto& kv : plan->class_cache)
         if (kv.second.built) bytes += (size_t)(kv.second.n_short + kv.second.n_med) * sizeof(int32_t);
diff --git a/h2gcn_amd/csrc/spmm_kernels.hip.h b/h2gcn_amd/csrc/spmm_kernels.hip.h
--- a/h2gcn_amd/csrc/spmm_kernels.hip.h
+++ b/h2gcn_amd/csrc/spmm_kernels.hip.h
@@ -94,6 +94,7 @@
     int64_t med_end[H2GCN_MAX_HOPS];
     int64_t med_groups;
     int med_per_wave;
+    const float* rowval[H2GCN_MAX_HOPS];
 };
 
 template <int VEC>
@@ -255,9 +256,9 @@
     }
 };
 
-template <typename TS, int VEC, int LPR, int U, bool PREDICATED, bool OFF32, int PHASE = 0, int NP>
+template <typename TS, int VEC, int LPR, int U, bool PREDICATED, bool OFF32, int PHASE = 0, int NP, bool EP = false>
 __device__ __forceinline__ void gather_batch(int c, float v, int t, int g, const GatherAddr<OFF32>& addr, bool take,
-                                             float (&acc)[NP][VEC]) {
+                                             float (&acc)[NP][VEC], std::integral_constant<bool, EP> = {}) {
     constexpr int G = kWave / LPR;
     typename LoadT<TS, VEC>::type x[U];
     float w[U];
@@ -277,7 +278,7 @@
             if (take) {
                 x[u] = load_vec<TS, VEC>(p);
             } else {
-                w[u] = 0.f;
+                w[u] = EP ? -0.f : 0.f;
                 x[u] = zero_load<TS, VEC>();
             }
         } else {
@@ -298,9 +299,16 @@
     }
 }
 
-template <typename TS, int VEC, int LPR, bool MASKED, bool OFF32, int MAXB = H2GCN_MAIN_MAXB, int NP>
+__device__ __forceinline__ void load_chunk_ids(const int32_t* __restrict__ colidx, float w, int64_t base, int64_t seg_end, int lane,
+                                               int& c, float& v) {
+    c = 0;
+    v = w;
+    if (base + lane < seg_end) c = __builtin_nontemporal_load(colidx + base + lane);
+}
+
+template <typename TS, int VEC, int LPR, bool MASKED, bool OFF32, int MAXB = H2GCN_MAIN_MAXB, int NP, bool EP = false>
 __device__ __forceinline__ void process_chunk(int c, float v, int n, int g, const GatherAddr<OFF32>& addr,
-                                              bool lane_active, float (&acc)[NP][VEC]) {
+                                              bool lane_active, float (&acc)[NP][VEC], std::integral_constant<bool, EP> ep = {}) {
     constexpr int G = kWave / LPR;
     const int full = n / G;
     int t = 0;
@@ -319,18 +327,18 @@
         if (t + 1 <= full) {
             gather_batch<TS, VEC, LPR, 1, MASKED, OFF32, 2 % NP>(c, v, t, g, addr, lane_active, acc);
             if constexpr (G > 1)
-                if (rem > 0) gather_batch<TS, VEC, LPR, 1, true, OFF32, 3 % NP>(c, v, full, g, addr, lane_active && g < rem, acc);
+                if (rem > 0) gather_batch<TS, VEC, LPR, 1, true, OFF32, 3 % NP>(c, v, full, g, addr, lane_active && g < rem, acc, ep);
         } else {
             if constexpr (G > 1)
-                if (rem > 0) gather_batch<TS, VEC, LPR, 1, true, OFF32, 2 % NP>(c, v, full, g, addr, lane_active && g < rem, acc);
+                if (rem > 0) gather_batch<TS, VEC, LPR, 1, true, OFF32, 2 % NP>(c, v, full, g, addr, lane_active && g < rem, acc, ep);
         }
     } else if (t + 1 <= full) {
         gather_batch<TS, VEC, LPR, 1, MASKED, OFF32>(c, v, t, g, addr, lane_active, acc);
         if constexpr (G > 1)
-            if (rem > 0) gather_batch<TS, VEC, LPR, 1, true, OFF32, 1 % NP>(c, v, full, g, addr, lane_active && g < rem, acc);
+            if (rem > 0) gather_batch<TS, VEC, LPR, 1, true, OFF32, 1 % NP>(c, v, full, g, addr, lane_active && g < rem, acc, ep);
     } else {
         if constexpr (G > 1)
-            if (rem > 0) gather_batch<TS, VEC, LPR, 1, true, OFF32>(c, v, full, g, addr, lane_active && g < rem, acc);
+            if (rem > 0) gather_batch<TS, VEC, LPR, 1, true, OFF32>(c, v, full, g, addr, lane_active && g < rem, acc, ep);
     }
 }
 
@@ -343,6 +351,7 @@
 struct WindowChunk {
     const uint32_t* ring;
     uint32_t e_lane;
+    static constexpr bool kExactPadding = false;
     template <int G>
     __device__ __forceinline__ void fetch(int step, int g, int& cj, float& w) const {
         static_assert(G > 1, "the one-neighbour-per-load geometry keeps v_readlane");
@@ -352,8 +361,21 @@
     }
 };
 
-template <typename TS, int VEC, int LPR, int U, bool PREDICATED, bool OFF32, int PHASE = 0, int NP>
-__device__ __forceinline__ void gather_batch_window(const WindowChunk& ch, int t, int g, const GatherAddr<OFF32>& addr, bool take,
+struct WindowChunkIds {
+    const uint32_t* ring;
+    uint32_t e_lane;
+    float w;
+    static constexpr bool kExactPadding = true;
+    template <int G>
+    __device__ __forceinline__ void fetch(int step, int g, int& cj, float& wj) const {
+        static_assert(G > 1, "the one-neighbour-per-load geometry keeps v_readlane");
+        cj = (int)ring[(e_lane + (uint32_t)(step * G)) & (kRingCap - 1)];
+        wj = w;
+    }
+};
+
+template <typename TS, int VEC, int LPR, int U, bool PREDICATED, bool OFF32, int PHASE = 0, typename CH, int NP>
+__device__ __forceinline__ void gather_batch_window(const CH& ch, int t, int g, const GatherAddr<OFF32>& addr, bool take,
                                              float (&acc)[NP][VEC]) {
     constexpr int G = kWave / LPR;
     typename LoadT<TS, VEC>::type x[U];
@@ -367,7 +389,7 @@
             if (take) {
                 x[u] = load_vec<TS, VEC>(p);
             } else {
-                w[u] = 0.f;
+                w[u] = CH::kExactPadding ? -0.f : 0.f;
                 x[u] = zero_load<TS, VEC>();
             }
         } else {
@@ -378,8 +400,8 @@
     for (int u = 0; u < U; ++u) fma_vec<TS, VEC>(acc[(PHASE + u) % NP], w[u], x[u]);
 }
 
-template <typename TS, int VEC, int LPR, bool MASKED, bool OFF32, int MAXB = H2GCN_MAIN_MAXB, int NP>
-__device__ __forceinline__ void process_chunk_window(const WindowChunk& ch, int n, int g, const GatherAddr<OFF32>& addr,
+template <typename TS, int VEC, int LPR, bool MASKED, bool OFF32, int MAXB = H2GCN_MAIN_MAXB, typename CH, int NP>
+__device__ __forceinline__ void process_chunk_window(const CH& ch, int n, int g, const GatherAddr<OFF32>& addr,
                                               bool lane_active, float (&acc)[NP][VEC]) {
     constexpr int G = kWave / LPR;
     const int full = n / G;
@@ -414,20 +436,21 @@
     }
 }
 
-template <typename TS, int VEC, int LPR, bool MASKED, bool OFF32, int MAXB = H2GCN_MAIN_MAXB, int NP>
+template <typename TS, int VEC, int LPR, bool MASKED, bool OFF32, int MAXB = H2GCN_MAIN_MAXB, bool ROWVAL = false, int NP>
 __device__ __forceinline__ void accumulate_segment(const int32_t* __restrict__ colidx,
                                                    const float* __restrict__ vals, int64_t seg_begin,
                                                    int64_t seg_end, int chunk0, int chunk_step,
                                                    const GatherAddr<OFF32>& addr, int lane, bool lane_active,
-                                                   float (&acc)[NP][VEC]) {
+                                                   float (&acc)[NP][VEC], float w = 0.f) {
     const int g = lane / LPR;
     for (int64_t base = seg_begin + (int64_t)chunk0 * kWave; base < seg_end; base += (int64_t)chunk_step * kWave) {
         const int64_t left = seg_end - base;
         const int n = left < kWave ? (int)left : kWave;
         int c;
         float v;
-        load_chunk(colidx, vals, base, seg_end, lane, c, v);
-        process_chunk<TS, VEC, LPR, MASKED, OFF32, MAXB>(c, v, n, g, addr, lane_active, acc);
+        if constexpr (ROWVAL) load_chunk_ids(colidx, w, base, seg_end, lane, c, v);
+        else load_chunk(colidx, vals, base, seg_end, lane, c, v);
+        process_chunk<TS, VEC, LPR, MASKED, OFF32, MAXB>(c, v, n, g, addr, lane_active, acc, std::integral_constant<bool, ROWVAL>{});
     }
 }
 
@@ -888,12 +911,13 @@
 template <typename T>
 __device__ __forceinline__ T pick(int s, T of_hop0, T of_hop1) { return s ? of_hop1 : of_hop0; }
 
-template <typename TS, typename TD, int VEC, int LPR, bool SUM, bool OFF32, bool EPI, int MAXB>
+template <typename TS, typename TD, int VEC, int LPR, bool SUM, bool OFF32, bool EPI, int MAXB, bool ROWVAL = false>
 __device__ __forceinline__ void window_tile_walk(const LaunchParams& p, int lane, int rpw, int64_t row0, int rows_here, int64_t rp,
                                                  int64_t lane_off0, int64_t src_col_begin, int lcol, int ecol,
-                                                 uint32_t (&ring)[kRingHops][2 * kRingCap]) {
+                                                 uint32_t (&ring)[kRingHops][(ROWVAL ? 1 : 2) * kRingCap], float rv = 0.f) {
     using off_t = typename std::conditional<OFF32, uint32_t, int64_t>::type;
     constexpr int NP = Tree<LPR>::NP;
+    static_assert(!ROWVAL || !SUM, "row-constant values exist for forward operands only");
     static_assert(kRingBlock == 4 * (kWave / 2) && kRingCap >= 2 * kRingBlock && kWave + 31 < kRingBlock, "ring safety (see above)");
     static_assert(kRingHops == 2, "hop state is selected with pick(s, hop 0's, hop 1's)");
     const int g = lane / LPR;
@@ -911,8 +935,8 @@
         if (lane >= l0) rel = (int)(rp - org);
         len = __builtin_amdgcn_readlane(rel, l0 + rows_here);
         col = p.hop[s].colidx + org;
-        val = p.hop[s].vals + org;
-        const int mc = misalign(col), mv = misalign(val);
+        if constexpr (!ROWVAL) val = p.hop[s].vals + org;
+        const int mc = misalign(col), mv = ROWVAL ? mc : misalign(val);
         mmin = min(mc, mv);
         mmax = max(mc, mv);
     };
@@ -920,11 +944,12 @@
     if (n_sel > 1) init_hop(1, col1, val1, len1, mmin1, mmax1);
     auto bound = [&](int l) __attribute__((always_inline)) { return __builtin_amdgcn_readlane(rel, l); };
     auto lane_array = [&](int s) __attribute__((always_inline)) {
-        return reinterpret_cast<const uint32_t*>(pick<const void*>(half, pick(s, col0, col1), pick(s, val0, val1)));
+        if constexpr (ROWVAL) return reinterpret_cast<const uint32_t*>(pick(s, col0, col1));
+        else return reinterpret_cast<const uint32_t*>(pick<const void*>(half, pick(s, col0, col1), pick(s, val0, val1)));
     };
     auto block_load = [&](int s, int blk) __attribute__((always_inline)) {
         const uint32_t* a = lane_array(s);
-        const int hi = pick(s, len0, len1);
+        const int hi = (ROWVAL && half) ? 0 : pick(s, len0, len1);
         const int x0 = blk * kRingBlock - misalign(a) + l4;
         u32x4 st = {0u, 0u, 0u, 0u};
         if (x0 >= 0 && x0 + 4 <= hi) {
@@ -939,8 +964,15 @@
     auto block_commit = [&](int s, int blk, const u32x4& st) __attribute__((always_inline)) {
         const int x0 = blk * kRingBlock - misalign(lane_array(s)) + l4;
         uint32_t* slots = ring[s];
-#pragma unroll
-        for (int i = 0; i < 4; ++i) slots[2 * ((uint32_t)(x0 + i) & (kRingCap - 1)) + half] = st[i];
+        if constexpr (ROWVAL) {
+            if (!half) {
+#pragma unroll
+                for (int i = 0; i < 4; ++i) slots[(uint32_t)(x0 + i) & (kRingCap - 1)] = st[i];
+            }
+        } else {
+#pragma unroll
+            for (int i = 0; i < 4; ++i) slots[2 * ((uint32_t)(x0 + i) & (kRingCap - 1)) + half] = st[i];
+        }
         __builtin_amdgcn_fence(__ATOMIC_RELEASE, "wavefront");
         __builtin_amdgcn_wave_barrier();
         __builtin_amdgcn_fence(__ATOMIC_ACQUIRE, "wavefront");
@@ -972,6 +1004,8 @@
         } else {
             const GatherAddr<OFF32> addr{reinterpret_cast<const char*>(src_ptr<TS>(p.src) + p.src_hop_off[s] + src_col_begin - VEC),
                                          (off_t)lane_off0, (off_t)(p.ld_src * sizeof(TS))};
+            float w_row = 0.f;
+            if constexpr (ROWVAL) w_row = __int_as_float(__builtin_amdgcn_readlane(__float_as_int(rv), l0));
             for (int base = sb; base < se; base += kWave) {
                 const int n = min(se - base, kWave);
                 for (int b = blk_of(s); base + n > avail(s, b); set_blk(s, ++b)) {
@@ -991,7 +1025,10 @@
                 const bool refill = pb < pe && min(pb + kWave, pe) > avail(ps, blk_of(ps));
                 u32x4 st = {0u, 0u, 0u, 0u};
                 if (refill) st = block_load(ps, blk_of(ps));
-                process_chunk_window<TS, VEC, LPR, false, OFF32, MAXB>(WindowChunk{ring[s], (uint32_t)(base + g)}, n, g, addr, true, acc);
+                if constexpr (ROWVAL)
+                    process_chunk_window<TS, VEC, LPR, false, OFF32, MAXB>(WindowChunkIds{ring[s], (uint32_t)(base + g), w_row}, n, g, addr, true, acc);
+                else
+                    process_chunk_window<TS, VEC, LPR, false, OFF32, MAXB>(WindowChunk{ring[s], (uint32_t)(base + g)}, n, g, addr, true, acc);
                 if (refill) {
                     block_commit(ps, blk_of(ps), st);
                     set_blk(ps, blk_of(ps) + 1);
@@ -1027,10 +1064,11 @@
 }
 
 template <int VEC, int LPR, bool EXACT, bool SUM, bool OFF32, bool PIPE = false, bool SHORT = false, bool EPI = false, int FB = 8, bool LISTS = false,
-          typename TS = float, typename TD = float>
+          typename TS = float, typename TD = float, bool ROWVAL = false>
 __global__ __launch_bounds__(kBlock, (min_waves_per_simd<VEC, LPR, EXACT, SUM, OFF32, PIPE, SHORT, EPI, FB, LISTS, TS>())) void spmm_hops_kernel(const LaunchParams p) {
     static_assert(!LISTS || (EXACT && !SHORT && !PIPE && (LPR == 16 || LPR == 32)), "list-driven launches exist for 64- and 128-column slices");
     static_assert(EXACT || LPR == kWave, "column-tiled path uses the whole wave per row");
+    static_assert(!ROWVAL || (uses_index_window<LPR, EXACT, PIPE, SHORT, EPI, LISTS>() && !SUM), "row values: forward walk on the index window");
     __shared__ float partial[kWavesPerBlock][kMaxTileCols];
     using off_t = typename std::conditional<OFF32, uint32_t, int64_t>::type;
     constexpr int NP = Tree<LPR>::NP;
@@ -1067,8 +1105,12 @@
                 const int64_t sb = h.rowptr[row], se = h.rowptr[row + 1];
                 const GatherAddr<OFF32> addr{reinterpret_cast<const char*>(src_ptr<TS>(p.src) + p.src_hop_off[s] + src_col_begin + (col0 - col_begin) - kBias),
                                              EXACT ? lane_off0 : (off_t)(li * VEC * (int)sizeof(TS)), (off_t)(p.ld_src * sizeof(TS))};
-                accumulate_segment<TS, VEC, LPR, !EXACT, OFF32, kMainB>(h.colidx, h.vals, sb, se, wave, kWavesPerBlock, addr, lane,
-                                                            lane_active, acc);
+                if constexpr (ROWVAL)
+                    accumulate_segment<TS, VEC, LPR, !EXACT, OFF32, kMainB, true>(h.colidx, nullptr, sb, se, wave, kWavesPerBlock, addr, lane,
+                                                                              lane_active, acc, p.rowval[s][row]);
+                else
+                    accumulate_segment<TS, VEC, LPR, !EXACT, OFF32, kMainB>(h.colidx, h.vals, sb, se, wave, kWavesPerBlock, addr, lane,
+                                                                            lane_active, acc);
             }
             float tot[VEC];
             fold_tree<VEC, LPR, NP>(acc, tot);
@@ -1127,9 +1169,12 @@
     const int rows_here = rows_here_l < rpw ? (int)rows_here_l : rpw;
 
     int64_t rp = 0;
+    float rv = 0.f;
     {
         const int hs = lane / (rpw + 1), r = lane % (rpw + 1);
         if (hs < n_sel && r <= rows_here) rp = p.hop[hs].rowptr[row0 + r];
+        if constexpr (ROWVAL)
+            if (hs < n_sel && r < rows_here) rv = p.rowval[hs][row0 + r];
     }
     const int rp_lo = (int)(rp & 0xffffffff), rp_hi = (int)(rp >> 32);
     auto seg_bound = [&](int l) -> int64_t {
@@ -1141,14 +1186,14 @@
         return;
     }
     if constexpr (uses_index_window<LPR, EXACT, PIPE, SHORT, EPI, LISTS>()) {
-        __shared__ uint32_t ring[kWavesPerBlock][kRingHops][2 * kRingCap];
+        __shared__ uint32_t ring[kWavesPerBlock][kRingHops][(ROWVAL ? 1 : 2) * kRingCap];
         bool fits = n_sel <= kRingHops;
 #pragma unroll
         for (int s = 0; s < kRingHops; ++s)
             if (s < n_sel && seg_bound(s * (rpw + 1) + rows_here) - seg_bound(s * (rpw + 1)) > kRingMaxRange) fits = false;
         if (fits) {
-            window_tile_walk<TS, TD, VEC, LPR, SUM, OFF32, EPI, kMainB>(p, lane, rpw, row0, rows_here, rp, (int64_t)lane_off0, src_col_begin, lcol, ecol,
-                                                                        ring[wave]);
+            window_tile_walk<TS, TD, VEC, LPR, SUM, OFF32, EPI, kMainB, ROWVAL>(p, lane, rpw, row0, rows_here, rp, (int64_t)lane_off0, src_col_begin, lcol,
+                                                                                ecol, ring[wave], rv);
             return;
         }
     }
@@ -1259,7 +1304,11 @@
                 const HopCsr& h = p.hop[s];
                 const GatherAddr<OFF32> addr{reinterpret_cast<const char*>(src_ptr<TS>(p.src) + p.src_hop_off[s] + src_col_begin + (col0 - col_begin) - kBias),
                                              EXACT ? lane_off0 : (off_t)(li * VEC * (int)sizeof(TS)), (off_t)(p.ld_src * sizeof(TS))};
-                accumulate_segment<TS, VEC, LPR, !EXACT, OFF32, kMainB>(h.colidx, h.vals, sb, se, 0, 1, addr, lane, lane_active, acc);
+                if constexpr (ROWVAL)
+                    accumulate_segment<TS, VEC, LPR, !EXACT, OFF32, kMainB, true>(h.colidx, nullptr, sb, se, 0, 1, addr, lane, lane_active, acc,
+                                                                              __int_as_float(__builtin_amdgcn_readlane(__float_as_int(rv), l0)));
+                else
+                    accumulate_segment<TS, VEC, LPR, !EXACT, OFF32, kMainB>(h.colidx, h.vals, sb, se, 0, 1, addr, lane, lane_active, acc);
                 if constexpr (!SUM) {
                     float tot[VEC];
                     fold_tree<VEC, LPR, NP>(acc, tot);
@@ -1335,6 +1384,7 @@
     bool gen;
     bool off32;
     int slice;
+    bool rowval = false;
 };
 
 
@@ -1342,6 +1392,15 @@
 void launch_tile_walk(const LaunchParams& p, const Schedule& k, dim3 grid, hipStream_t stream) {
     const dim3 block(kBlock);
     const bool pipe = EXACT && k.pipe;
+    if constexpr (uses_index_window<LPR, EXACT, false, false, false, false>() && !SUM && std::is_same<TD, float>::value) {
+        if (k.rowval && !k.gen && !pipe) {
+            if (k.off32)
+                hipLaunchKernelGGL((spmm_hops_kernel<VEC, LPR, EXACT, SUM, true, false, false, false, 8, false, TS, TD, true>), grid, block, 0, stream, p);
+            else
+                hipLaunchKernelGGL((spmm_hops_kernel<VEC, LPR, EXACT, SUM, false, false, false, false, 8, false, TS, TD, true>), grid, block, 0, stream, p);
+            return;
+        }
+    }
     if (k.gen && k.off32)
         hipLaunchKernelGGL((spmm_hops_kernel<VEC, LPR, EXACT, SUM, true, false, false, true, 8, false, TS, TD>), grid, block, 0, stream, p);
     else if (k.gen)
diff --git a/h2gcn_amd/hops.py b/h2gcn_amd/hops.py
--- a/h2gcn_amd/hops.py
+++ b/h2gcn_amd/hops.py
@@ -172,6 +172,18 @@
             out.append(("none", "indices", "indices+values")[v])
         return out
 
+    @property
+    def row_constant(self) -> list:
+        if not _capi.has("h2gcn_plan_row_constant"):
+            return [0] * self.n_hops
+        L = _capi.lib()
+        out = []
+        for k in range(self.n_hops):
+            v = L.h2gcn_plan_row_constant(self._handle, k)
+            _capi.check(v)
+            out.append(int(v))
+        return out
+
     def device_bytes(self) -> int:
         if not _capi.has("h2gcn_plan_device_bytes"):
             raise RuntimeError(f"{_capi.library_path()} predates h2gcn_plan_device_bytes")
diff --git a/include/h2gcn_hip.h b/include/h2gcn_hip.h
--- a/include/h2gcn_hip.h
+++ b/include/h2gcn_hip.h
@@ -61,6 +61,8 @@
                     int64_t* n_long_segments, int32_t* has_transpose);
 
 int h2gcn_plan_transpose_sharing(const h2gcn_plan_t* plan, int hop);
+
+int h2gcn_plan_row_constant(const h2gcn_plan_t* plan, int hop);
 
 size_t h2gcn_plan_device_bytes(const h2gcn_plan_t* plan);
 
```

New measurement: 14.16 billion (median of 6 runs). 1.02x the previous value.
